# LitLeo/3m-asr-inference

Measured on AMD Instinct MI355X. Metric: encoder frames/sec, 18Lx32e Conformer-MoE, 206-frame utterance, higher is better.
Workload: dtype f32; 1 GPU; 18-layer 32-expert fp32 (v_mfma_f32_16x16x4_f32), batch=1x206 frames per GPU, all experts local (BASELINE.json configs[1]); layers=18, experts=32, frames=206, batch_per_gpu=1, parallelism=replicas x1, streams_per_gpu=4, hip_graph=True, kernels_per_forward=267, fold_pos_proj=True, routing=balanced, route_mode=staged, packed_rows=False, fork_embed=auto

## Files before the change

### 3m-asr-inference_amd/csrc/api.hip

```cpp
#include <string.h>

#include <vector>

#include "../../include/m3asr.h"
#include "common.h"
#include "kernels.h"

namespace m3 {

static thread_local char g_err[512] = "";

void set_error(const char* fmt, ...) {
  va_list ap;
  va_start(ap, fmt);
  vsnprintf(g_err, sizeof(g_err), fmt, ap);
  va_end(ap);
}
const char* last_error() { return g_err; }

struct MoeWorkspace {
  int32_t* mapping;
  int32_t* acc;
  int32_t* pos;
  float* slab;
// ... 152 lines not shown
  M3_REQUIRE(rows && mapping && out, "moe_combine_bf16: null pointer");
  return launch_moe_combine(rows, 1, mapping, nullptr, gate_value, nullptr, resid, alpha, ln_gamma, ln_beta, ln_eps, out,
                            S, idim, (hipStream_t)stream, out_bf16);
}
int m3_ep_send_map(const int32_t* gate_idx, const int32_t* mapping, const int32_t* acc_histogram, int S, int world, int e_loc,
                   int capacity, int32_t* map_send, void* wire, int row_bytes, m3_stream stream) {
  M3_REQUIRE(gate_idx && mapping && acc_histogram && map_send && wire, "ep_send_map: null pointer");
  return launch_ep_send_map(gate_idx, mapping, acc_histogram, S, world, e_loc, capacity, map_send, wire, row_bytes,
                            (hipStream_t)stream);
}
int m3_ep_recv_gate(const void* wire, int world, int e_loc, int capacity, int row_bytes, int32_t* gate_recv, m3_stream stream) {
  M3_REQUIRE(wire && gate_recv, "ep_recv_gate: null pointer");
  return launch_ep_recv_gate(wire, world, e_loc, capacity, row_bytes, gate_recv, (hipStream_t)stream);
}
int m3_moe_router(const float* embed, int ld_embed, int embed_dim, const float* x, int ldx, int idim, const float* w,
                  const float* bias, const float* ln_gamma, const float* ln_beta, float ln_eps, float* xn, int ld_xn,
                  float* logits, int ld_logits, int S, int num_expert, m3_stream stream) {
  M3_REQUIRE(S <= 1 || (ld_embed >= embed_dim && ldx >= idim), "moe_router: ld_embed=%d / ldx=%d shorter than the rows (%d / %d)",
             ld_embed, ldx, embed_dim, idim);
  M3_REQUIRE(S <= 1 || xn == nullptr || ld_xn >= idim, "moe_router: ld_xn=%d is shorter than a row of %d", ld_xn, idim);
  M3_REQUIRE(S <= 1 || ld_logits >= num_expert, "moe_router: ld_logits=%d is shorter than a row of %d", ld_logits, num_expert);
  M3_REQUIRE(aligned16(embed) && aligned16(x) && aligned16(xn), "moe_router: embed / x / xn must be 16-byte aligned");
  return launch_moe_router(embed, ld_embed, embed_dim, x, ldx, idim, w, bias, ln_gamma, ln_beta, ln_eps, xn, ld_xn, logits,
                           ld_logits, S, num_expert, nullptr, (hipStream_t)stream);
}
int m3_softmax_top1(const float* logits, int ld, const int32_t* len, int rows_per_batch, int S, int width,
                    int32_t* idx, float* value, m3_stream stream) {
  M3_REQUIRE(S <= 1 || ld >= width, "softmax_topk: ld=%d is shorter than a row of %d", ld, width);
  return launch_softmax_top1(logits, ld, len, rows_per_batch, S, width, idx, value, (hipStream_t)stream);
}
int m3_moe_gate_index(const float* logits, const int32_t* row_len, int rows_per_batch, int S, int num_expert, int32_t* gate_idx,
                      float* gate_value, int32_t* mapping, int32_t* acc_histogram, int32_t* pos, m3_stream stream) {
  M3_REQUIRE(logits && gate_idx && gate_value && mapping && acc_histogram, "moe_gate_index: null pointer");
  M3_REQUIRE(aligned16(logits), "moe_gate_index: logits must be 16-byte aligned");
  return launch_moe_gate_index(logits, num_expert, row_len, rows_per_batch, S, gate_idx, gate_value, mapping, acc_histogram, pos,
                               (hipStream_t)stream);
}
int m3_moe_route(const float* x, int ldx, int idim, const float* wx, const float* wsum, const float* bias, const float* eall,
                 int ld_e, float ln_eps, const int32_t* row_len, int rows_per_batch, int S, int num_expert, int32_t* gate_idx,
                 float* gate_value, int32_t* mapping, int32_t* acc_histogram, int32_t* pos, m3_stream stream) {
  M3_REQUIRE(x && wx && wsum && gate_idx && gate_value && mapping && acc_histogram, "moe_route: null pointer");
  M3_REQUIRE(idim > 0, "moe_route: idim=%d", idim);
  M3_REQUIRE(S <= 1 || ldx >= idim, "moe_route: ldx=%d is shorter than a row of %d", ldx, idim);
  M3_REQUIRE(eall == nullptr || S <= 1 || ld_e >= num_expert, "moe_route: ld_e=%d is shorter than a row of %d", ld_e, num_expert);
  M3_REQUIRE(aligned16(x) && aligned16(wx), "moe_route: x / wx must be 16-byte aligned");
  return launch_moe_route(x, ldx, idim, wx, wsum, bias, eall, ld_e, ln_eps, row_len, rows_per_batch, S, num_expert, gate_idx,
                          gate_value, mapping, acc_histogram, pos, (hipStream_t)stream);
}
size_t m3_moe_route_expert_workspace_size(int S, int num_expert, int idim, int hidden_units) {
  if (!expert_ffn_f32_self_routing(S, num_expert) || idim <= 0 || hidden_units <= 0 || hidden_units % kExpertSlice) return 0;
  return align_up(expert_ffn_slab_bytes(S, idim, hidden_units), 256);
}
int m3_moe_route_expert_ffn(const float* x, int ldx, const float* logits, const int32_t* row_len, int rows_per_batch,
                            const float* w1, const float* b1, const float* w2, int w2_sliced, const float* b2, int S,
                            int num_expert, int idim, int hidden_units, const float* norm_gamma, const float* norm_beta,
                            float norm_eps, int use_gate_value, const float* resid, float alpha, const float* ln_gamma,
                            const float* ln_beta, float ln_eps, int32_t* gate_idx, float* gate_value, int32_t* mapping,
                            int32_t* acc_histogram, int32_t* pos, float* y, void* workspace, size_t workspace_bytes,
                            m3_stream stream) {
  M3_REQUIRE(x && w1 && b1 && w2 && y, "moe_route_expert_ffn: null pointer");
  M3_REQUIRE((norm_gamma == nullptr) == (norm_beta == nullptr) && (ln_gamma == nullptr) == (ln_beta == nullptr),
             "moe_route_expert_ffn: a LayerNorm needs both gamma and beta");
  M3_REQUIRE(idim > 0 && hidden_units > 0, "moe_route_expert_ffn: bad sizes D=%d F=%d", idim, hidden_units);
  M3_REQUIRE(S <= 1 || ldx >= idim, "moe_route_expert_ffn: ldx=%d is shorter than a row of %d", ldx, idim);
  M3_REQUIRE(aligned16(x) && aligned16(logits), "moe_route_expert_ffn: x / logits must be 16-byte aligned");
  const size_t need = m3_moe_route_expert_workspace_size(S, num_expert, idim, hidden_units);
  M3_REQUIRE(need == 0 || (workspace != nullptr && workspace_bytes >= need), "moe_route_expert_ffn: workspace %zu bytes < required %zu",
             workspace_bytes, need);
  float* slab = (float*)workspace;
  int rc = launch_expert_route_ffn_f32(x, ldx, logits, row_len, rows_per_batch, S, num_expert, idim, hidden_units, w1, b1, w2, w2_sliced,
                                       b2, slab, gate_idx, gate_value, mapping, acc_histogram, pos, (hipStream_t)stream, norm_gamma,
                                       norm_beta, norm_eps);
  if (rc) return rc;
  return launch_moe_combine(slab, hidden_units / kExpertSlice, nullptr, gate_idx, use_gate_value ? gate_value : nullptr, nullptr, resid,
                            alpha, ln_gamma, ln_beta, ln_eps, y, S, idim, (hipStream_t)stream);
}

static int attention_operands(const void* qkv, int ldq, const void* p, int ldp, const void* out, int ldo, int B, int T, int H, int dk) {
  M3_REQUIRE(B * T <= 1 || (ldq >= 3 * H * dk && ldo >= H * dk), "attention: ldq=%d / ldo=%d shorter than the rows (%d / %d)", ldq, ldo, 3 * H * dk, H * dk);
  M3_REQUIRE(T <= 1 || ldp >= H * dk, "attention: ldp=%d is shorter than a row of %d", ldp, H * dk);
  M3_REQUIRE(aligned16(qkv) && aligned16(p) && aligned16(out), "attention: qkv / p / out must be 16-byte aligned");
  return 0;
}

static int linear_params(const m3_linear_desc* d, GemmParams* out) {
  M3_REQUIRE(d != nullptr, "linear: null descriptor");
  GemmParams p;
  p.A = d->a; p.lda = d->lda;
  p.A2 = d->a2; p.lda2 = d->lda2; p.K1 = d->k1;
  p.mode = d->a2 ? GEMM_A_CONCAT2 : GEMM_A_PLAIN;
  p.W = (const float*)d->w; p.bias = d->bias; p.Y = d->y; p.ldy = d->ldy;
  M3_REQUIRE(d->weight_dtype == M3_F32 || d->weight_dtype == M3_BF16, "linear: weight_dtype %d", d->weight_dtype);
  p.w_bf16 = d->weight_dtype == M3_BF16;
  p.M = d->M; p.N = d->N; p.K = d->K;
  p.ln_gamma = d->ln_gamma; p.ln_beta = d->ln_beta; p.ln_eps = d->ln_eps;
  p.ln_wsum = d->ln_wsum; p.ln_wbeta = d->ln_wbeta;
  p.row_len = d->len; p.rows_per_batch = d->rows_per_batch; p.mask_in = d->mask_in; p.mask_out = d->mask_out;
  p.act = d->act; p.alpha = d->alpha; p.resid = d->resid; p.ldr = d->ldr;
  M3_REQUIRE((d->a_dtype == M3_F32 || d->a_dtype == M3_BF16) && (d->y_dtype == M3_F32 || d->y_dtype == M3_BF16),
             "linear: a_dtype / y_dtype must be f32 or bf16");
  if (d->a_dtype == M3_BF16 || d->y_dtype == M3_BF16 || d->y_copy_bf16)
    M3_REQUIRE(p.w_bf16 && p.mode == GEMM_A_PLAIN && !p.ln_gamma, "linear: bf16 activations need bf16 weights, plain A, no affine LayerNorm");
  p.a_bf16 = d->a_dtype == M3_BF16; p.y_bf16 = d->y_dtype == M3_BF16;
  p.Yb = d->y_copy_bf16; p.ldyb = d->ld_copy; p.Yb_stats = d->y_copy_stats;
  p.ln_stats = d->ln_stats; p.ln_stat_parts = d->ln_stat_parts;
  {
    const int n_out = d->act == M3_ACT_GLU ? d->N / 2 : d->N;
    const int k1 = d->a2 ? d->k1 : d->K, a_mult = p.a_bf16 ? 8 : 4;
    const bool rows = d->M > 1;
    M3_REQUIRE(d->lda % a_mult == 0 && (!rows || d->lda >= k1), "linear: lda=%d must be a multiple of %d and >= %d", d->lda, a_mult, k1);
    if (d->a2) M3_REQUIRE(d->lda2 % 4 == 0 && (!rows || d->lda2 >= d->K - k1), "linear: lda2=%d must be a multiple of 4 and >= %d", d->lda2, d->K - k1);
    M3_REQUIRE(!rows || d->ldy >= n_out, "linear: ldy=%d is shorter than an output row of %d", d->ldy, n_out);
    if (p.y_bf16) M3_REQUIRE(d->ldy % 4 == 0, "linear: ldy=%d must be a multiple of 4 for a bf16 y", d->ldy);
    if (d->resid) M3_REQUIRE(!rows || d->ldr >= n_out, "linear: ldr=%d is shorter than an output row of %d", d->ldr, n_out);
    if (d->y_copy_bf16) M3_REQUIRE(d->ld_copy % 4 == 0 && (!rows || d->ld_copy >= n_out), "linear: ld_copy=%d must be a multiple of 4 and >= %d", d->ld_copy, n_out);
  }
  *out = p;
  return 0;
}
static int linear_pointers(const m3_linear_desc* d) {
  M3_REQUIRE(d->a && d->w && d->y, "linear: null a / w / y");
  M3_REQUIRE(aligned16(d->a) && aligned16(d->a2) && aligned16(d->y) && aligned16(d->resid) && aligned16(d->y_copy_bf16),
             "linear: a / a2 / y / resid / y_copy_bf16 must be 16-byte aligned");
  M3_REQUIRE((const void*)d->resid != (const void*)d->y || d->ldr == d->ldy, "linear: y == resid (in-place) needs ldr=%d == ldy=%d", d->ldr, d->ldy);
  return 0;
}
const char* m3_linear_kernel(const m3_linear_desc* d, int with_workspace) {
  GemmParams p;
  if (linear_params(d, &p)) return nullptr;
  return gemm_kernel_label(p, with_workspace && gemm_f32_splitk_plan(p, nullptr) >= 2);
}
int m3_linear(const m3_linear_desc* d, m3_stream stream) {
  GemmParams p;
  if (int rc = linear_params(d, &p)) return rc;
  if (int rc = linear_pointers(d)) return rc;
  return launch_gemm_f32(p, (hipStream_t)stream);
}
size_t m3_linear_workspace_size(const m3_linear_desc* d) {
  GemmParams p;
  size_t need = 0;
  if (linear_params(d, &p) == 0) gemm_f32_splitk_plan(p, &need);
  return need;
}
int m3_linear_ws(const m3_linear_desc* d, void* workspace, size_t workspace_bytes, m3_stream stream) {
  GemmParams p;
  if (int rc = linear_params(d, &p)) return rc;
  if (int rc = linear_pointers(d)) return rc;
  size_t need = 0;
  if (gemm_f32_splitk_plan(p, &need) >= 2 && workspace != nullptr && workspace_bytes >= need)
    return launch_gemm_f32_splitk(p, (float*)workspace, workspace_bytes, (hipStream_t)stream);
  return launch_gemm_f32(p, (hipStream_t)stream);
}

int m3_layer_norm(const float* x, const float* gamma, const float* beta, float eps, float* y, int rows, int dim,
                  m3_stream stream) {
  return launch_layernorm(x, gamma, beta, eps, y, rows, dim, (hipStream_t)stream);
}
int m3_relpos_attention(const float* qkv, int ldq, const float* p, int ldp, const float* pos_u, const float* pos_v,
                        const int32_t* len, int B, int T, int H, int dk, float scale, float* out, int ldo,
                        m3_stream stream) {
  if (int rc = attention_operands(qkv, ldq, p, ldp, out, ldo, B, T, H, dk)) return rc;
  return launch_relpos_attention(qkv, ldq, p, ldp, pos_u, pos_v, len, B, T, H, dk, scale, out, ldo,
                                 (hipStream_t)stream);
}
int m3_relpos_attention_bf16(const void* qkv, int ldq, const float* p, int ldp, const float* pos_u, const float* pos_v,
                             const int32_t* len, int B, int T, int H, int dk, float scale, int chunk, int left_chunks,
                             void* out, int ldo, m3_stream stream) {
  if (int rc = attention_operands(qkv, ldq, p, ldp, out, ldo, B, T, H, dk)) return rc;
  return launch_relpos_attention_bf16(qkv, ldq, p, ldp, pos_u, pos_v, len, B, T, H, dk, scale, out, ldo, (hipStream_t)stream,
                                      nullptr, chunk, left_chunks);
}
int m3_relpos_attention_chunk(const float* qkv, int ldq, const float* p, int ldp, const float* pos_u, const float* pos_v,
                              const int32_t* len, int B, int T, int H, int dk, float scale, int chunk, int left_chunks,
                              float* out, int ldo, m3_stream stream) {
  if (int rc = attention_operands(qkv, ldq, p, ldp, out, ldo, B, T, H, dk)) return rc;
  return launch_relpos_attention(qkv, ldq, p, ldp, pos_u, pos_v, len, B, T, H, dk, scale, out, ldo, (hipStream_t)stream, 0,
                                 nullptr, chunk, left_chunks);
}
int m3_dwconv_ln_silu(const float* z, const float* w_kc, const float* bias, const float* gamma, const float* beta,
                      float eps, int B, int T, int D, int K, float* out, m3_stream stream) {
  return launch_dwconv_ln_silu(z, w_kc, bias, gamma, beta, eps, B, T, D, K, out, (hipStream_t)stream);
}
int m3_subsample_conv1(const float* feat, const float* w9c, const float* bias, int B, int T, int idim, int C,
                       float* out, m3_stream stream) {
  return launch_conv1_relu(feat, w9c, bias, nullptr, nullptr, B, T, idim, C, out, (hipStream_t)stream);
}
int m3_subsample_conv1_cmvn(const float* feat, const float* w9c, const float* bias, const float* cmvn_mean,
                            const float* cmvn_istd, int B, int T, int idim, int C, float* out, m3_stream stream) {
  M3_REQUIRE((cmvn_mean == nullptr) == (cmvn_istd == nullptr), "subsample_conv1: cmvn mean and istd go together");
  return launch_conv1_relu(feat, w9c, bias, cmvn_mean, cmvn_istd, B, T, idim, C, out, (hipStream_t)stream);
}
int m3_conv2d_3x3s2_first(const float* feat, const float* w9c, const float* bias, int B, int T, int idim, int C, int act,
                          float* out, m3_stream stream) {
  M3_REQUIRE(act == M3_ACT_NONE || act == M3_ACT_RELU, "conv2d: act %d (none / relu)", act);
  return launch_conv1_relu(feat, w9c, bias, nullptr, nullptr, B, T, idim, C, out, (hipStream_t)stream, act == M3_ACT_RELU);
}
int m3_cmvn(const float* x, const int32_t* len, const float* mean, const float* istd, int B, int T, int D, float* y,
            m3_stream stream) {
  M3_REQUIRE(x && mean && istd && y, "cmvn: null pointer");
  return launch_cmvn(x, len, mean, istd, B, T, D, y, (hipStream_t)stream);
}
int m3_log_softmax_bias(const float* x, const float* bias, float* y, size_t rows, int n, m3_stream stream) {
  M3_REQUIRE(x && y && n > 0, "log_softmax_bias: bad arguments");
  return launch_log_softmax_bias(x, bias, y, rows, n, (hipStream_t)stream);
}
int m3_conv2d_3x3s2(const float* in, const float* w, const float* bias, int B, int T1, int F1, int C, int act, float* out,
                    m3_stream stream);
int m3_subsample_conv2(const float* in, const float* w, const float* bias, int B, int T1, int F1, int C, float* out,
                       m3_stream stream) {
  return m3_conv2d_3x3s2(in, w, bias, B, T1, F1, C, M3_ACT_RELU, out, stream);
}
int m3_conv2d_3x3s2(const float* in, const float* w, const float* bias, int B, int T1, int F1, int C, int act, float* out,
                    m3_stream stream) {
  M3_REQUIRE(T1 >= 3 && F1 >= 3, "subsample_conv2: input (%d,%d) smaller than the kernel", T1, F1);
  M3_REQUIRE(act == M3_ACT_NONE || act == M3_ACT_RELU || act == M3_ACT_SILU, "conv2d: act %d", act);
  GemmParams p;
  p.mode = GEMM_A_CONV3X3S2;
  p.A = in; p.lda = 4;
  p.conv_T1 = T1; p.conv_F1 = F1; p.conv_T2 = (T1 - 3) / 2 + 1; p.conv_F2 = (F1 - 3) / 2 + 1; p.conv_C = C;
  p.W = w; p.bias = bias; p.Y = out; p.ldy = C;
  p.M = B * p.conv_T2 * p.conv_F2; p.N = C; p.K = 9 * C;
  p.act = act;
  return launch_gemm_f32(p, (hipStream_t)stream);
}

int m3_att_masked_softmax(const float* scores, const int32_t* len, int B, int H, int T1, int T2, float scale,
                          float* out, m3_stream stream) {
  return launch_att_masked_softmax(scores, len, B, H, T1, T2, scale, out, (hipStream_t)stream);
}
int m3_ctc_greedy(const float* logits, const int32_t* len, int B, int T, int V, int blank, int32_t* frame_ids,
                  int32_t* tokens, int32_t* n_tokens, m3_stream stream) {
  return launch_ctc_greedy(logits, len, B, T, V, blank, frame_ids, tokens, n_tokens, (hipStream_t)stream);
}
int m3_ctc_topk(const float* logits, size_t rows, int V, int k, float* top_logp, int32_t* top_idx, m3_stream stream) {
  return launch_ctc_topk(logits, rows, V, k, top_logp, top_idx, (hipStream_t)stream);
}
int m3_ctc_prefix_beam_search(const float* top_logp, const int32_t* top_idx, int T, int k, int beam, int blank,
                              int32_t* hyp_tokens, int32_t* hyp_len, float* hyp_score, int32_t* n_hyps) {
  return ctc_prefix_beam_search_host(top_logp, top_idx, T, k, beam, blank, hyp_tokens, hyp_len, hyp_score, n_hyps);
}
size_t m3_ctc_beam_state_size(const m3_ctc_beam_desc* desc) { return ctc_beam_state_size(desc); }
int m3_ctc_beam_reset(const m3_ctc_beam_desc* desc, void* state, size_t state_bytes, m3_stream stream) {
  return launch_ctc_beam_reset(desc, state, state_bytes, (hipStream_t)stream);
}
int m3_ctc_beam_reset_slots(const m3_ctc_beam_desc* desc, void* state, size_t state_bytes, const int32_t* slots, int n, m3_stream stream) {
  M3_REQUIRE(n == 0 || slots != nullptr, "ctc_beam_reset_slots: null slot list");
  if (n == 0) return 0;
  return launch_ctc_beam_reset(desc, state, state_bytes, (hipStream_t)stream, slots, n);
}
int m3_ctc_beam_advance(const m3_ctc_beam_desc* desc, void* state, size_t state_bytes, const float* top_logp,
                        const int32_t* top_idx, int T_chunk, const int32_t* n_frames, m3_stream stream) {
  return launch_ctc_beam_advance(desc, state, state_bytes, top_logp, top_idx, T_chunk, n_frames, (hipStream_t)stream);
}
int m3_ctc_beam_nbest(const m3_ctc_beam_desc* desc, const void* state, size_t state_bytes, int32_t* hyp_tokens,
                      int32_t* hyp_len, float* hyp_score, int32_t* n_hyps, m3_stream stream) {
  return launch_ctc_beam_nbest(desc, state, state_bytes, hyp_tokens, hyp_len, hyp_score, n_hyps, (hipStream_t)stream);
}
size_t m3_ctc_greedy_stream_state_size(const m3_ctc_greedy_desc* desc) { return ctc_greedy_stream_state_size(desc); }
int m3_ctc_greedy_stream_reset(const m3_ctc_greedy_desc* desc, void* state, size_t state_bytes, m3_stream stream) {
  return launch_ctc_greedy_stream_reset(desc, state, state_bytes, (hipStream_t)stream);
}
int m3_ctc_greedy_stream_reset_slots(const m3_ctc_greedy_desc* desc, void* state, size_t state_bytes, const int32_t* slots, int n,
                                     m3_stream stream) {
  M3_REQUIRE(n == 0 || slots != nullptr, "ctc_greedy_stream_reset_slots: null slot list");
  if (n == 0) return 0;
  return launch_ctc_greedy_stream_reset(desc, state, state_bytes, (hipStream_t)stream, slots, n);
}
int m3_ctc_greedy_stream_advance(const m3_ctc_greedy_desc* desc, void* state, size_t state_bytes, const float* logits,
                                 int T_chunk, int V, const int32_t* n_frames, int32_t* frame_ids, m3_stream stream) {
  return launch_ctc_greedy_stream_advance(desc, state, state_bytes, logits, T_chunk, V, n_frames, frame_ids, (hipStream_t)stream);
}
int m3_ctc_greedy_stream_tokens(const m3_ctc_greedy_desc* desc, const void* state, size_t state_bytes, int32_t* tokens,
                                int32_t* n_tokens, m3_stream stream) {
  return launch_ctc_greedy_stream_tokens(desc, state, state_bytes, tokens, n_tokens, (hipStream_t)stream);
}
int m3_cat_split_cache(const void* in_cache, const void* input, int B, int cache_dim, int input_dim, void* output,
                       void* out_cache, m3_stream stream) {
  return launch_cat_split_cache(in_cache, input, B, cache_dim, input_dim, output, out_cache, (hipStream_t)stream);
}
int m3_att_stream_softmax(const float* scores, const int32_t* decode_frame_num, const int32_t* mask_idx, int B, int N,
                          int ld, int cache_len, float scale, float* out, m3_stream stream) {
  return launch_att_stream_softmax(scores, decode_frame_num, mask_idx, B, N, ld, cache_len, scale, out, (hipStream_t)stream);
}
int m3_rel_positional_encoding(const float* x, const float* pe, int pe_len, const int32_t* frame_num, int max_offset,
                               float scale, int B, int T, int D, float* y, float* pos_emb, int32_t* frame_num_out,
                               m3_stream stream) {
  return launch_rel_positional_encoding(x, pe, pe_len, frame_num, max_offset, scale, B, T, D, y, pos_emb, frame_num_out,
                                        (hipStream_t)stream);
}
int m3_masked_fill(const float* x, const int32_t* len, int B, int C, int T, float fill, float* y, m3_stream stream) {
  return launch_masked_fill(x, len, B, C, T, fill, y, (hipStream_t)stream);
}
int m3_glu(const float* x, int outer, int C, int inner, float* y, m3_stream stream) {
  return launch_glu(x, outer, C, inner, y, (hipStream_t)stream);
}
int m3_mask_conv2d_sample(const int32_t* len_in, int B, int left_padding, int stride, int32_t* len_out,
                          m3_stream stream) {
  return launch_mask_conv2d_sample(len_in, B, left_padding, stride, len_out, (hipStream_t)stream);
}
int m3_scale(const float* x, float scale, float* y, size_t n, m3_stream stream) {
  return launch_scale(x, scale, y, n, (hipStream_t)stream);
}
int m3_unary(const float* x, float* y, size_t n, int act, m3_stream stream) {
  return launch_unary(x, y, n, act, (hipStream_t)stream);
}
int m3_binary(const float* a, const float* b, float* y, const int64_t* shape, const int64_t* strides_a,
// ... 70 lines not shown
```

### 3m-asr-inference_amd/csrc/conv.hip

```cpp
#include "common.h"
#include "kernels.h"

namespace m3 {

struct DwCausal {
  int causal = 0;
  const float* left = nullptr;
  long left_b_stride = 0; int left_t_stride = 0;
  const int32_t* step = nullptr;
  long half = 0;
  const int32_t* chunk_len = nullptr;
  int max_chunks = 0;
};

template <int KT, bool CAUSAL, bool SLOTS = false>
__device__ __forceinline__ void dwconv_ln_silu_body(const float* __restrict__ z, const float* __restrict__ w_kc,
                                                    const float* __restrict__ bias, const float* __restrict__ gamma,
                                                    const float* __restrict__ beta, float eps, int T, int D, int K,
                                                    float* __restrict__ out, int out_bf16, const int32_t* __restrict__ pad_of,
                                                    const int32_t* __restrict__ row0, const int32_t* __restrict__ row_len,
                                                    int n_rows, const DwCausal& cs, const int row) {
  __shared__ float red[2][16];
  asm volatile("" ::"s"(z), "s"(w_kc), "s"(bias), "s"(gamma), "s"(beta), "s"(eps), "s"(T), "s"(D), "s"(K), "s"(out), "s"(out_bf16),
               "s"(pad_of), "s"(row0), "s"(row_len), "s"(n_rows));
// ... 53 lines not shown
        } else {
          on[kk] = (k0 + kk < K && tt >= 0 && tt < T) ? 1.f : 0.f;
        }
        zz[kk] = ldg4(src + c);
        ww[kk] = ldg4(w_kc + (size_t)k * D + c);
      }
#pragma unroll
      for (int kk = 0; kk < KT; ++kk)
#pragma unroll
        for (int j = 0; j < 4; ++j) v[j] = fmaf(zz[kk][j] * on[kk], ww[kk][j], v[j]);
    }
  }
  if (gamma != nullptr) {
    float s = live ? (v[0] + v[1]) + (v[2] + v[3]) : 0.f;
    s = wave_sum(s);
    if (lane == 0) red[0][wave] = s;
    __syncthreads();
    float tot = 0.f;
    for (int w = 0; w < nwaves; ++w) tot += red[0][w];
    const float mean = tot / (float)D;
    float q = 0.f;
    if (live) {
#pragma unroll
      for (int j = 0; j < 4; ++j) {
        const float d = v[j] - mean;
        q += d * d;
      }
    }
    q = wave_sum(q);
    if (lane == 0) red[1][wave] = q;
    __syncthreads();
    float qt = 0.f;
    for (int w = 0; w < nwaves; ++w) qt += red[1][w];
    const float rstd = rsqrtf(qt / (float)D + eps);
    if (live) {
      const f32x4 g = ldg4(gamma + c), be = ldg4(beta + c);
#pragma unroll
      for (int j = 0; j < 4; ++j) v[j] = (v[j] - mean) * rstd * g[j] + be[j];
    }
  }
  if (live) {
#pragma unroll
    for (int j = 0; j < 4; ++j) v[j] = silu(v[j]);
    if (out_bf16) {
      bf16x4 h;
#pragma unroll
      for (int j = 0; j < 4; ++j) h[j] = (bf16_t)v[j];
      *reinterpret_cast<bf16x4*>(reinterpret_cast<bf16_t*>(out) + (size_t)row * D + c) = h;
    } else {
      stg4(out + (size_t)row * D + c, v);
    }
  }
}

template <int KT, bool CAUSAL, bool SLOTS = false>
__global__ __launch_bounds__(1024) void dwconv_ln_silu_kernel(const float* __restrict__ z, const float* __restrict__ w_kc,
                                                              const float* __restrict__ bias,
                                                              const float* __restrict__ gamma,
                                                              const float* __restrict__ beta, float eps, int T,
                                                              int D, int K, float* __restrict__ out, int out_bf16,
                                                              const int32_t* __restrict__ pad_of,
                                                              const int32_t* __restrict__ row0,
                                                              const int32_t* __restrict__ row_len, int n_rows, DwCausal cs) {
  dwconv_ln_silu_body<KT, CAUSAL, SLOTS>(z, w_kc, bias, gamma, beta, eps, T, D, K, out, out_bf16, pad_of, row0, row_len, n_rows, cs, (int)blockIdx.x);
}
struct DwKernArgs {
  const float *z, *w_kc, *bias, *gamma, *beta; float eps; int T, D, K; float* out; int out_bf16;
  const int32_t *pad_of, *row0, *row_len; int n_rows; DwCausal cs;
};
template <int KT, bool CAUSAL>
__global__ __launch_bounds__(1024) void dwconv_ln_silu_dual_kernel(const DwKernArgs a, const DwKernArgs b) {
  if ((int)blockIdx.x < a.n_rows)
    dwconv_ln_silu_body<KT, CAUSAL>(a.z, a.w_kc, a.bias, a.gamma, a.beta, a.eps, a.T, a.D, a.K, a.out, a.out_bf16, a.pad_of, a.row0, a.row_len,
                                    a.n_rows, a.cs, (int)blockIdx.x);
  else
    dwconv_ln_silu_body<KT, CAUSAL>(b.z, b.w_kc, b.bias, b.gamma, b.beta, b.eps, b.T, b.D, b.K, b.out, b.out_bf16, b.pad_of, b.row0, b.row_len,
                                    b.n_rows, b.cs, (int)blockIdx.x - a.n_rows);
}

static int launch_dwconv_impl(const float* z, const float* w_kc, const float* bias, const float* gamma, const float* beta, float eps,
                              int B, int T, int D, int K, float* out, hipStream_t stream, int out_bf16, const int32_t* pad_of,
                              const int32_t* row0, const int32_t* row_len, const DwCausal& cs, bool slots = false) {
  M3_REQUIRE(!slots || (cs.causal && cs.step != nullptr && cs.max_chunks > 0), "dwconv (slot mode): needs the streaming causal form");
  M3_REQUIRE((D & 3) == 0 && D <= 4096, "dwconv: channels=%d must be a multiple of 4 (<=4096)", D);
  M3_REQUIRE(cs.causal || (K & 1) == 1, "dwconv: kernel size %d must be odd (non-causal)", K);
  M3_REQUIRE(!cs.causal || (cs.left != nullptr && K >= 2), "dwconv (causal): the frames left of frame 0 must be supplied (left_fill / cache)");
  const int rows = B * T;
  if (rows == 0) return 0;
  const int threads = (int)align_up(D / 4, 64);
  const int grid = rows + (cs.step != nullptr ? B * (K - 1) : 0);
#define M3_DW_CASE(KT_, C_)                                                                                                  \
  hipLaunchKernelGGL((dwconv_ln_silu_kernel<KT_, C_>), dim3(grid), dim3(threads), 0, stream, z, w_kc, bias, gamma, beta, eps, T, \
                     D, K, out, out_bf16, pad_of, row0, row_len, rows, cs)
#define M3_DW_SLOTS(KT_)                                                                                                        \
  hipLaunchKernelGGL((dwconv_ln_silu_kernel<KT_, true, true>), dim3(grid), dim3(threads), 0, stream, z, w_kc, bias, gamma, beta, eps, \
                     T, D, K, out, out_bf16, pad_of, row0, row_len, rows, cs)
  if (slots) { if (K <= 15) M3_DW_SLOTS(15); else M3_DW_SLOTS(8); }
  else if (K <= 15) { if (cs.causal) M3_DW_CASE(15, true); else M3_DW_CASE(15, false); }
  else { if (cs.causal) M3_DW_CASE(8, true); else M3_DW_CASE(8, false); }
#undef M3_DW_SLOTS
#undef M3_DW_CASE
  M3_LAUNCH_CHECK();
  return 0;
}

int launch_dwconv_ln_silu(const float* z, const float* w_kc, const float* bias, const float* gamma,
                          const float* beta, float eps, int B, int T, int D, int K, float* out, hipStream_t stream, int out_bf16,
                          const int32_t* pad_of, const int32_t* row0, const int32_t* row_len, const float* causal_left_fill) {
  DwCausal cs;
  if (causal_left_fill != nullptr) { cs.causal = 1; cs.left = causal_left_fill; }
  return launch_dwconv_impl(z, w_kc, bias, gamma, beta, eps, B, T, D, K, out, stream, out_bf16, pad_of, row0, row_len, cs);
}

int launch_dwconv_ln_silu_args(const DwArgs& a, hipStream_t stream) {
  return launch_dwconv_ln_silu(a.z, a.w_kc, a.bias, a.gamma, a.beta, a.eps, a.B, a.T, a.D, a.K, a.out, stream, a.out_bf16, a.pad_of, a.row0,
                               a.row_len, a.causal_left_fill);
}
bool dwconv_dual_fusable(const DwArgs& a, const DwArgs& b) {
  return a.D == b.D && a.K == b.K && (a.causal_left_fill != nullptr) == (b.causal_left_fill != nullptr) && a.B * a.T > 0 && b.B * b.T > 0 &&
         (a.D & 3) == 0 && a.D <= 4096 && (a.causal_left_fill != nullptr || (a.K & 1) == 1);
}
int launch_dwconv_ln_silu_dual(const DwArgs& a, const DwArgs& b, hipStream_t stream) {
  M3_REQUIRE(dwconv_dual_fusable(a, b), "dwconv dual: the two problems do not share an instantiation");
  auto pack = [](const DwArgs& q) {
    DwKernArgs k;
    k.z = q.z; k.w_kc = q.w_kc; k.bias = q.bias; k.gamma = q.gamma; k.beta = q.beta; k.eps = q.eps; k.T = q.T; k.D = q.D; k.K = q.K;
    k.out = q.out; k.out_bf16 = q.out_bf16; k.pad_of = q.pad_of; k.row0 = q.row0; k.row_len = q.row_len; k.n_rows = q.B * q.T;
    if (q.causal_left_fill != nullptr) { k.cs.causal = 1; k.cs.left = q.causal_left_fill; }
    return k;
  };
  const DwKernArgs ka = pack(a), kb = pack(b);
  const int threads = (int)align_up(a.D / 4, 64), grid = ka.n_rows + kb.n_rows;
  const bool causal = a.causal_left_fill != nullptr;
#define M3_DWD_CASE(KT_, C_) hipLaunchKernelGGL((dwconv_ln_silu_dual_kernel<KT_, C_>), dim3(grid), dim3(threads), 0, stream, ka, kb)
  if (a.K <= 15) { if (causal) M3_DWD_CASE(15, true); else M3_DWD_CASE(15, false); }
  else { if (causal) M3_DWD_CASE(8, true); else M3_DWD_CASE(8, false); }
#undef M3_DWD_CASE
  M3_LAUNCH_CHECK();
  return 0;
}

int launch_dwconv_ln_silu_stream(const float* z, const float* w_kc, const float* bias, const float* gamma, const float* beta,
                                 float eps, int B, int T, int D, int K, float* out, float* cache_pair, const int32_t* step,
                                 const int32_t* chunk_len, hipStream_t stream, int out_bf16, int slot_max_chunks) {
  M3_REQUIRE(cache_pair && step && chunk_len, "dwconv (stream): null state");
  DwCausal cs;
  cs.causal = 1; cs.left = cache_pair; cs.left_b_stride = (long)(K - 1) * D; cs.left_t_stride = D;
  cs.step = step; cs.half = (long)B * (K - 1) * D; cs.chunk_len = chunk_len;
  cs.max_chunks = slot_max_chunks > 0 ? slot_max_chunks : 0;
  return launch_dwconv_impl(z, w_kc, bias, gamma, beta, eps, B, T, D, K, out, stream, out_bf16, nullptr, nullptr, nullptr, cs,
                            slot_max_chunks >= 0);
}

__global__ __launch_bounds__(256) void conv1_relu_kernel(const float* __restrict__ feat, const float* __restrict__ w9c,
                                                         const float* __restrict__ bias,
                                                         const float* __restrict__ cmvn_mean,
                                                         const float* __restrict__ cmvn_istd, int T, int idim, int T1,
                                                         int F1, int C, float* __restrict__ out, int relu, int out_bf16,
                                                         const int32_t* __restrict__ feat_len, int32_t* __restrict__ lens_out, int B) {
  extern __shared__ float xs[];
  const int row = blockIdx.x;
  if (feat_len != nullptr && blockIdx.x == 0 && blockIdx.y == 0)
    for (int i = threadIdx.x; i < B; i += blockDim.x) lens_out[i] = ((feat_len[i] - 3) / 2 + 1 - 3) / 2 + 1;
  const int b = row / T1, t1 = row - b * T1;
  const float* src = feat + ((size_t)b * T + 2 * t1) * idim;
  for (int i = threadIdx.x; i < 3 * idim; i += blockDim.x) {
    float xv = src[i];
    if (cmvn_mean != nullptr) {
      const int f = i % idim;
      xv = (xv - cmvn_mean[f]) * cmvn_istd[f];
    }
    xs[i] = xv;
  }
  const int c = threadIdx.x * 4;
  const bool live = c < C;
  f32x4 w[9], bv = f32x4{0.f, 0.f, 0.f, 0.f};
  if (live) {
    bv = ldg4(bias + c);
#pragma unroll
    for (int k = 0; k < 9; ++k) w[k] = ldg4(w9c + (size_t)k * C + c);
  }
  __syncthreads();
  if (!live) return;
  const size_t obase = (size_t)row * F1 * C + c;
  const int fchunk = (F1 + gridDim.y - 1) / gridDim.y;
  const int f_lo = blockIdx.y * fchunk, f_hi = min(F1, f_lo + fchunk);
  for (int f1 = f_lo; f1 < f_hi; ++f1) {
    f32x4 acc = bv;
#pragma unroll
    for (int kh = 0; kh < 3; ++kh)
#pragma unroll
      for (int kw = 0; kw < 3; ++kw) {
        const float xv = xs[kh * idim + 2 * f1 + kw];
#pragma unroll
        for (int j = 0; j < 4; ++j) acc[j] = fmaf(xv, w[kh * 3 + kw][j], acc[j]);
      }
#pragma unroll
    for (int j = 0; j < 4; ++j) acc[j] = relu ? fmaxf(acc[j], 0.f) : acc[j];
    if (out_bf16) {
      bf16x4 h;
#pragma unroll
      for (int j = 0; j < 4; ++j) h[j] = (bf16_t)acc[j];
      *reinterpret_cast<bf16x4*>(reinterpret_cast<bf16_t*>(out) + obase + (size_t)f1 * C) = h;
    } else {
      stg4(out + obase + (size_t)f1 * C, acc);
    }
  }
}

int launch_conv1_relu(const float* feat, const float* w9c, const float* bias, const float* cmvn_mean,
                      const float* cmvn_istd, int B, int T, int idim, int C, float* out, hipStream_t stream, int relu, int out_bf16,
                      const int32_t* feat_len, int32_t* lens_out) {
  M3_REQUIRE(T >= 3 && idim >= 3, "subsampling: input (T=%d, idim=%d) shorter than the 3x3 kernel", T, idim);
  M3_REQUIRE((C & 3) == 0 && C <= 1024, "subsampling: channels=%d must be a multiple of 4 (<= 1024)", C);
  const int T1 = (T - 3) / 2 + 1, F1 = (idim - 3) / 2 + 1;
  if (B * T1 == 0) return 0;
  const int threads = (int)align_up(C / 4, 64);
  const int fsplit = B * T1 >= 2048 ? 1 : (B * T1 >= 512 ? 2 : 5);
  hipLaunchKernelGGL(conv1_relu_kernel, dim3(B * T1, fsplit), dim3(threads), 3 * idim * sizeof(float), stream,
                     feat, w9c, bias, cmvn_mean, cmvn_istd, T, idim, T1, F1, C, out, relu, out_bf16, feat_len, lens_out, B);
  M3_LAUNCH_CHECK();
  return 0;
}

__global__ void depthwise_conv1d_nct_kernel(const float* __restrict__ x, const float* __restrict__ w,
                                            const float* __restrict__ bias, int C, int T, int To, int K, int pad,
                                            float* __restrict__ y, size_t n) {
  for (size_t i = (size_t)blockIdx.x * blockDim.x + threadIdx.x; i < n; i += (size_t)gridDim.x * blockDim.x) {
    const int t = (int)(i % To);
    const size_t bc = i / To;
    const int c = (int)(bc % C);
    const float* xr = x + bc * T;
    float acc = bias ? bias[c] : 0.f;
    for (int k = 0; k < K; ++k) {
      const int tt = t + k - pad;
      if (tt >= 0 && tt < T) acc = fmaf(xr[tt], w[(size_t)c * K + k], acc);
    }
    y[i] = acc;
  }
}

int launch_depthwise_conv1d_nct(const float* x, const float* w, const float* bias, int B, int C, int T, int K,
                                int pad, float* y, hipStream_t stream) {
  const int To = T + 2 * pad - K + 1;
  M3_REQUIRE(pad >= 0 && To > 0, "depthwise_conv1d: T=%d K=%d pad=%d leaves no output", T, K, pad);
  const size_t n = (size_t)B * C * To;
  if (n == 0) return 0;
  hipLaunchKernelGGL(depthwise_conv1d_nct_kernel, dim3(grid1d(n, 4096)), dim3(256), 0,
                     stream, x, w, bias, C, T, To, K, pad, y, n);
  M3_LAUNCH_CHECK();
  return 0;
}

__global__ void pad2d_kernel(const float* __restrict__ x, int H, int W, int pre_h, int pre_w, int Ho, int Wo,
                             float* __restrict__ y, size_t n) {
  for (size_t i = (size_t)blockIdx.x * blockDim.x + threadIdx.x; i < n; i += (size_t)gridDim.x * blockDim.x) {
    const int wo = (int)(i % Wo), ho = (int)((i / Wo) % Ho);
    const size_t o = i / ((size_t)Wo * Ho);
    const int h = ho - pre_h, w_ = wo - pre_w;
    y[i] = (h >= 0 && h < H && w_ >= 0 && w_ < W) ? x[(o * H + h) * W + w_] : 0.f;
  }
}
int launch_pad2d(const float* x, size_t outer, int H, int W, int pre_h, int post_h, int pre_w, int post_w, float* y, hipStream_t stream) {
  M3_REQUIRE(pre_h >= 0 && post_h >= 0 && pre_w >= 0 && post_w >= 0, "pad2d: negative padding (cropping) is not implemented");
  const int Ho = H + pre_h + post_h, Wo = W + pre_w + post_w;
  const size_t n = outer * Ho * Wo;
  if (n == 0) return 0;
  hipLaunchKernelGGL(pad2d_kernel, dim3(grid1d(n, 4096)), dim3(256), 0, stream, x, H, W, pre_h, pre_w, Ho, Wo, y, n);
  M3_LAUNCH_CHECK();
  return 0;
}

}
```

### 3m-asr-inference_amd/csrc/engine.hip

```cpp
#include <assert.h>
#include <math.h>
#include <stdlib.h>
#include <string.h>

#include <functional>
#include <memory>
#include <string>
#include <unordered_map>
#include <vector>

#include "../../include/m3asr.h"
#include "common.h"
#include "kernels.h"

namespace m3 {
struct MoeWorkspace {
  int32_t* mapping; int32_t* acc; int32_t* pos; float* slab; size_t bytes;
};
MoeWorkspace carve_moe_workspace(void* base, int S, int E, int D, int F);
}

using namespace m3;

namespace {

struct Norm { const float* g = nullptr; const float* b = nullptr; };
struct Lin { const float* w = nullptr; const float* b = nullptr; const float* wsum = nullptr; const float* wbeta = nullptr; };

struct BlockW {
  Norm n_ffm, n_mha, n_conv, n_ff, n_final, n_cnn;
  Lin mac1, mac2, qkv, pos, out, pw1, pw2, ff1, ff2;
  const float* pos_u = nullptr; const float* pos_v = nullptr;
  const float* dw_w = nullptr; const float* dw_b = nullptr;
  const float* left_fill = nullptr;
  Lin router;
  Lin router_x;
  const float *ew1 = nullptr, *eb1 = nullptr, *ew2 = nullptr, *eb2 = nullptr;
  const float *es1 = nullptr, *es2 = nullptr;
  float h_scale = 0.f;
};

struct SubW { const float* c1w; const float* c1b; const float* c2w; const float* c2b; Lin out; };

enum class FuseKind { None, Gemm, Dwconv, Attention };

struct Stage {
  std::string name;
  std::function<int(hipStream_t)> run;
  m3_stage_info info;
  bool reads_embed = false;
  FuseKind fuse_kind = FuseKind::None;
  GemmParams gemm;
  DwArgs dw;
  AttArgs att;
};

m3_stage_info stage_info(const char* kernel, int launches, double bytes, double flops, bool per_row = true) {
  m3_stage_info i;
  i.kernel = kernel; i.launches = launches; i.per_row = per_row ? 1 : 0; i.alg_bytes = bytes; i.flops = flops;
  return i;
}

struct Buf { void* ptr; size_t bytes; };

struct BindKey {
  int B = 0, T = 0;
  const float* feat = nullptr; const int32_t* feat_len = nullptr; float* logits = nullptr;
  void* ws = nullptr; size_t ws_bytes = 0;
  int ep_cap = 0;
  void* sstate = nullptr; int s_hist = 0, s_maxf = 0;
  bool s_slots = false;
  bool operator==(const BindKey& o) const {
    return B == o.B && T == o.T && feat == o.feat && feat_len == o.feat_len && logits == o.logits && ws == o.ws &&
           ws_bytes == o.ws_bytes && ep_cap == o.ep_cap && sstate == o.sstate && s_hist == o.s_hist && s_maxf == o.s_maxf &&
           s_slots == o.s_slots;
  }
};

}

struct m3_engine {
  m3_engine_config cfg;
  std::unordered_map<std::string, m3_weight_entry> table;
  std::vector<std::string> names;
  SubW sub_e, sub_m;
  std::vector<BlockW> eblocks, mblocks;
  Norm e_after, m_after;
  Lin out_linear;
  const float* pe = nullptr;
  int64_t pe_rows = 0;
  const float* pos_all = nullptr;
  const float* cmvn_mean = nullptr; const float* cmvn_istd = nullptr;
  const float* output_bias = nullptr;
  const float* router_e_all = nullptr;

  struct Bound {
    BindKey key;
    int Tp = 0, S = 0;
    bool a16 = false;
    bool dma = false;
    bool packed = false;
    bool xn_skipped = false;
    int fork_first = -1, fork_mid = -1, join_at = -1;
    std::shared_ptr<float> pfold;
    std::vector<Stage> stages;
    std::unordered_map<std::string, Buf> buffers;
    int n_kernels = 0;
    hipGraphExec_t graph_exec = nullptr;
    bool graph_valid = false;
    uint64_t last_use = 0;
    bool matches(const BindKey& k) const { return !stages.empty() && key == k; }
  };
  Bound cur;
  std::vector<Bound> parked;
  uint64_t use_clock = 0;
  int n_captures = 0;
  int ep_capacity = 0;
  hipStream_t side = nullptr;
  hipEvent_t ev_fork = nullptr, ev_join = nullptr;
  std::unordered_map<int, std::weak_ptr<float>> pfold_by_tp;
};

namespace {

struct Switches {
  int gate_index_max_rows;
  bool self_route;
  bool hfuse;
  int router_min_rows;
  bool router_xq;
  bool router_skip_xn;
  bool fused8_adapt;
};
const Switches& switches() {
  static const Switches sw = [] {
    auto num = [](const char* name, int dflt) { const char* v = getenv(name); return v ? atoi(v) : dflt; };
    Switches w;
    w.gate_index_max_rows = num("M3_GATE_INDEX_MAX_ROWS", 512);
    w.self_route = num("M3_SELF_ROUTE", 1) != 0;
    w.hfuse = num("M3_HFUSE", 1) != 0;
    w.router_min_rows = num("M3_ROUTER_MIN_ROWS", 2048);
    w.router_xq = num("M3_ROUTER_XQ", 1) != 0;
    w.router_skip_xn = num("M3_ROUTER_SKIP_XN", 0) != 0;
    w.fused8_adapt = num("M3_FUSED8_ADAPT", 0) != 0;
    return w;
  }();
  return sw;
}

bool lookup(const m3_engine* e, const std::string& name, int64_t numel, const float** out, int dtype = M3_F32) {
  auto it = e->table.find(name);
  if (it == e->table.end()) {
    set_error("engine: weight '%s' missing from the plan", name.c_str());
    return false;
  }
  if (numel >= 0 && it->second.numel != numel) {
    set_error("engine: weight '%s' has %lld elements, expected %lld", name.c_str(), (long long)it->second.numel,
              (long long)numel);
    return false;
  }
  if (it->second.dtype != dtype) {
    set_error("engine: weight '%s' has dtype %d, the engine (weight_dtype=%d) expects %d", name.c_str(),
              (int)it->second.dtype, (int)e->cfg.weight_dtype, dtype);
    return false;
  }
  *out = (const float*)it->second.data;
  return true;
}

#define GET(dst, name, numel) \
  do { if (!lookup(e, (name), (numel), &(dst))) return false; } while (0)
#define GETW(dst, name, numel) \
  do { if (!lookup(e, (name), (numel), &(dst), e->cfg.weight_dtype == M3_F32 ? M3_F32 : M3_BF16)) return false; } while (0)
#define GETE(dst, name, numel) \
  do { if (!lookup(e, (name), (numel), &(dst), e->cfg.weight_dtype)) return false; } while (0)

bool load_norm(const m3_engine* e, const std::string& p, int d, Norm* n) {
  GET(n->g, p + "weight", d);
  GET(n->b, p + "bias", d);
  return true;
}
bool load_lin(const m3_engine* e, const std::string& p, int64_t n_out, int64_t n_in, bool bias, Lin* l) {
  GETW(l->w, p + "weight", n_out * n_in);
  if (bias) GET(l->b, p + "bias", n_out);
  return true;
}
bool load_lin_ln(const m3_engine* e, const std::string& p, int64_t n_out, int64_t n_in, bool wbeta, Lin* l,
                 bool fp32_only = false) {
  if (fp32_only) {
    GET(l->w, p + "ln.weight", n_out * n_in);
  } else {
    GETW(l->w, p + "ln.weight", n_out * n_in);
  }
  GET(l->b, p + "ln.bias", n_out);
  GET(l->wsum, p + "ln.wsum", n_out);
  if (wbeta) GET(l->wbeta, p + "ln.wbeta", n_out);
  return true;
}

bool load_block(const m3_engine* e, const std::string& p, int D, int F, int K, bool cnn_ln, bool moe, int De, BlockW* b, bool causal) {
  const m3_engine_config& c = e->cfg;
  if (!load_norm(e, p + "norm_final.", D, &b->n_final)) return false;
  if (moe && !load_norm(e, p + "norm_ff.", D, &b->n_ff)) return false;
  if (!load_lin_ln(e, p + "feed_forward_macaron.w_1.", F, D, false, &b->mac1) ||
      !load_lin(e, p + "feed_forward_macaron.w_2.", D, F, true, &b->mac2) ||
      !load_lin_ln(e, p + "self_attn.qkv.", 3 * D, D, false, &b->qkv) ||
      !load_lin(e, p + "self_attn.linear_out.", D, D, true, &b->out) ||
      !load_lin_ln(e, p + "conv_module.pointwise_conv1.", 2 * D, D, true, &b->pw1) ||
      !load_lin(e, p + "conv_module.pointwise_conv2.", D, D, true, &b->pw2))
    return false;
  GET(b->pos_u, p + "self_attn.pos_bias_u", D);
  GET(b->pos_v, p + "self_attn.pos_bias_v", D);
  GET(b->dw_w, p + "conv_module.depthwise_conv.weight_kc", (int64_t)K * D);
  GET(b->dw_b, p + "conv_module.depthwise_conv.bias", D);
  if (cnn_ln && !load_norm(e, p + "conv_module.norm.", D, &b->n_cnn)) return false;
  if (causal) GET(b->left_fill, p + "conv_module.left_fill", D);
  if (!moe) {
    if (!load_lin_ln(e, p + "feed_forward.w_1.", F, D, false, &b->ff1) ||
        !load_lin(e, p + "feed_forward.w_2.", D, F, true, &b->ff2))
      return false;
  } else {
    const int world = c.ep_world_size > 0 ? c.ep_world_size : 1;
    const int64_t Etot = (int64_t)c.num_experts * world;
    GET(b->router.w, p + "feed_forward.router_weights_t", Etot * (D + De));
    if (c.router_with_bias) GET(b->router.b, p + "feed_forward.router_bias", Etot);
    if (c.fuse_route && !load_lin_ln(e, p + "feed_forward.router_x.", Etot, D, false, &b->router_x, true)) return false;
    const int64_t E = c.num_experts;
    GETE(b->ew1, p + "feed_forward.experts.w_1.weight", E * F * D);
    if (c.weight_dtype == M3_FP8) {
      GET(b->es1, p + "feed_forward.experts.w_1.scale", E * F);
      GET(b->es2, p + "feed_forward.experts.w_2.scale", E * D);
      if (c.fp8_activations) {
        const float* hs = nullptr;
        GET(hs, p + "feed_forward.experts.h_scale", 1);
        if (hipMemcpy(&b->h_scale, hs, sizeof(float), hipMemcpyDeviceToHost) != hipSuccess || !(b->h_scale > 0.f)) {
          set_error("engine: '%sfeed_forward.experts.h_scale' must hold one positive number", p.c_str());
          return false;
        }
      }
    }
    GET(b->eb1, p + "feed_forward.experts.w_1.bias", E * F);
    GETE(b->ew2, p + "feed_forward.experts.w_2.weight_sliced", E * D * F);
    GET(b->eb2, p + "feed_forward.experts.w_2.bias", E * D);
  }
  return true;
}

bool load_sub(const m3_engine* e, const std::string& p, int D, int idim, SubW* s) {
  const int F2 = ((idim - 1) / 2 - 1) / 2;
  GET(s->c1w, p + "conv.0.weight_9c", 9 * (int64_t)D);
  GET(s->c1b, p + "conv.0.bias", D);
  GETW(s->c2w, p + "conv.2.weight_ohwi", 9 * (int64_t)D * D);
  GET(s->c2b, p + "conv.2.bias", D);
  return load_lin(e, p + "out.0.", D, (int64_t)D * F2, true, &s->out);
}
#undef GET
#undef GETW
#undef GETE

inline int sub_len(int t) { return ((t - 3) / 2 + 1 - 3) / 2 + 1; }

struct Carver {
  char* base; size_t off = 0;
  explicit Carver(void* b) : base((char*)b) {}
  template <typename T> T* take(size_t n) {
    T* p = (T*)(base ? base + off : nullptr);
    off += align_up(n * sizeof(T), 256);
    return p;
  }
};

struct Plan {
  int32_t* lens;
  float *c1, *c2, *x, *emb, *h1, *qkv, *pbuf, *ctx, *glu, *dw, *xn, *rl, *eall;
  void* xb;
  int32_t* moe_fs;
  unsigned char* xq; float* xq_scale;
  float* xstats;
  int32_t* gate_idx; float* gate_val;
  void* moe_ws; size_t moe_ws_bytes;
  float* splitk; size_t splitk_bytes;
  float* taps;
  float* pfold;
  int32_t *row0, *pad_of; float* xpad; void* xbpad; float* lpk;
  int32_t *ep_acc, *ep_mapping, *ep_pos, *ep_map_send, *ep_gate_recv, *ep_overflow; float *wire_a, *wire_b; int ep_cap, ep_rows;
  bool fork;
  bool hfuse;
  float *e_c1, *e_c2, *e_x, *e_h1, *e_qkv, *e_ctx, *e_glu, *e_dw, *e_xpad, *e_splitk, *e_xstats; void *e_xb, *e_xbpad;
  size_t bytes;
};

bool use_fork_embed(const m3_engine_config& c, int B, int S) { return c.fork_embed > 0 && !c.debug_taps; }
bool use_packed_rows(const m3_engine_config& c, int B) {
  if (c.packed_rows < 0 || (c.packed_rows == 0 && B <= 1)) return false;
  return !c.debug_taps && c.fuse_route == 0 && B <= 1024;
}

bool use_hfuse(const m3_engine_config& c, int B, int S) {
  return switches().hfuse && !c.debug_taps && c.weight_dtype == M3_F32 && c.embed_blocks > 0 && c.num_blocks > 0 && S <= 128 && c.fork_embed <= 0 &&
         !use_packed_rows(c, B);
}

Plan make_plan(const m3_engine_config& c, void* base, int B, int T, int ep_capacity = 0) {
  Plan p;
  Carver cv(base);
  const int Tp = sub_len(T), S = B * Tp;
  const int T1 = (T - 3) / 2 + 1, F1 = (c.input_dim - 3) / 2 + 1, F2 = (F1 - 3) / 2 + 1;
  const int D = c.attention_dim > c.embed_dim ? c.attention_dim : c.embed_dim;
  const int F = c.hidden_units > c.embed_linear_units ? c.hidden_units : c.embed_linear_units;
  const int world = c.ep_world_size > 0 ? c.ep_world_size : 1;
  const int Etot = c.num_experts * world;
  p.lens = cv.take<int32_t>(B);
  p.c1 = cv.take<float>((size_t)B * T1 * F1 * D);
  p.c2 = cv.take<float>((size_t)S * F2 * D);
  p.x = cv.take<float>((size_t)S * D);
  p.emb = cv.take<float>((size_t)S * D);
  p.xb = cv.take<uint16_t>((size_t)S * D);
  p.xstats = cv.take<float>((size_t)S * 2 * kXbStatParts);
  p.h1 = cv.take<float>((size_t)S * F);
  p.qkv = cv.take<float>((size_t)S * 3 * D);
  p.pbuf = cv.take<float>((size_t)Tp * D * (c.num_blocks + c.embed_blocks));
  p.ctx = cv.take<float>((size_t)S * D);
  p.glu = cv.take<float>((size_t)S * D);
  p.dw = cv.take<float>((size_t)S * D);
  p.xn = cv.take<float>((size_t)S * D);
  p.xq = nullptr; p.xq_scale = nullptr; p.moe_fs = nullptr;
  if (c.weight_dtype == M3_FP8) p.moe_fs = cv.take<int32_t>(64);
  if (c.weight_dtype == M3_FP8 && D == 512) {
    p.xq = cv.take<unsigned char>((size_t)S * D);
    p.xq_scale = cv.take<float>((size_t)S);
  }
  p.rl = cv.take<float>((size_t)S * Etot);
  p.eall = cv.take<float>((size_t)S * Etot * c.num_blocks);
  p.gate_idx = cv.take<int32_t>((size_t)c.num_blocks * S);
  p.gate_val = cv.take<float>((size_t)c.num_blocks * S);
  const bool ep = world > 1 || c.ep_stages > 0;
  p.ep_cap = ep ? (ep_capacity > 0 ? ep_capacity : S) : 0;
  p.ep_rows = ep ? world * (p.ep_cap + 1) : 0;
  p.moe_ws_bytes = carve_moe_workspace(nullptr, ep ? p.ep_rows : S, c.num_experts, c.attention_dim, c.hidden_units).bytes;
  p.moe_ws = cv.take<char>(p.moe_ws_bytes * (size_t)(c.debug_taps ? c.num_blocks : 1));
  p.ep_acc = p.ep_mapping = p.ep_pos = p.ep_map_send = p.ep_gate_recv = p.ep_overflow = nullptr; p.wire_a = p.wire_b = nullptr;
  if (ep) {
    p.ep_overflow = cv.take<int32_t>(64);
    p.ep_acc = cv.take<int32_t>((size_t)Etot + 1);
    p.ep_mapping = cv.take<int32_t>(S);
    p.ep_pos = cv.take<int32_t>(S);
    p.ep_map_send = cv.take<int32_t>(S);
    p.ep_gate_recv = cv.take<int32_t>(p.ep_rows);
    p.wire_a = cv.take<float>((size_t)p.ep_rows * c.attention_dim);
    p.wire_b = cv.take<float>((size_t)p.ep_rows * c.attention_dim);
  }
  {
    size_t n1 = 0, n2 = 0;
    if (c.weight_dtype == M3_F32) {
      GemmParams g;
      g.mode = GEMM_A_CONV3X3S2; g.lda = 4; g.conv_C = D; g.M = S * F2; g.N = D; g.K = 9 * D; g.ldy = D;
      gemm_f32_splitk_plan(g, &n1);
      GemmParams l;
      l.lda = F2 * D; l.M = S; l.N = D; l.K = F2 * D; l.ldy = D;
      gemm_f32_splitk_plan(l, &n2);
    }
    p.splitk_bytes = n1 > n2 ? n1 : n2;
    p.splitk = p.splitk_bytes ? cv.take<float>(p.splitk_bytes / sizeof(float)) : nullptr;
  }
  p.taps = c.debug_taps ? cv.take<float>((size_t)(c.num_blocks + c.embed_blocks) * S * D) : nullptr;
  p.pfold = nullptr;
  p.row0 = p.pad_of = nullptr; p.xpad = p.lpk = nullptr; p.xbpad = nullptr;
  if (use_packed_rows(c, B)) {
    p.row0 = cv.take<int32_t>(B + 1);
    p.pad_of = cv.take<int32_t>(S);
    p.xpad = cv.take<float>((size_t)S * D);
    p.xbpad = cv.take<uint16_t>((size_t)S * D);
    p.lpk = cv.take<float>((size_t)S * c.output_dim);
  }
  p.fork = use_fork_embed(c, B, S);
  p.hfuse = !p.fork && use_hfuse(c, B, S);
  p.e_c1 = p.c1; p.e_c2 = p.c2; p.e_x = p.x; p.e_h1 = p.h1; p.e_qkv = p.qkv; p.e_ctx = p.ctx; p.e_glu = p.glu; p.e_dw = p.dw;
  p.e_xb = p.xb; p.e_xpad = p.xpad; p.e_xbpad = p.xbpad; p.e_splitk = p.splitk; p.e_xstats = p.xstats;
  if (p.fork || p.hfuse) {
    p.e_c1 = cv.take<float>((size_t)B * T1 * F1 * D);
    p.e_c2 = cv.take<float>((size_t)S * F2 * D);
    p.e_x = cv.take<float>((size_t)S * D);
    p.e_xb = cv.take<uint16_t>((size_t)S * D);
    p.e_xstats = cv.take<float>((size_t)S * 2 * kXbStatParts);
    p.e_h1 = cv.take<float>((size_t)S * F);
    p.e_qkv = cv.take<float>((size_t)S * 3 * D);
    p.e_ctx = cv.take<float>((size_t)S * D);
    p.e_glu = cv.take<float>((size_t)S * D);
    p.e_dw = cv.take<float>((size_t)S * D);
    if (p.splitk_bytes) p.e_splitk = cv.take<float>(p.splitk_bytes / sizeof(float));
    if (use_packed_rows(c, B)) {
      p.e_xpad = cv.take<float>((size_t)S * D);
      p.e_xbpad = cv.take<uint16_t>((size_t)S * D);
    }
  }
  p.bytes = cv.off;
  return p;
}

struct StreamState {
  int32_t* step = nullptr;
  std::vector<float*> kv, conv;
  int32_t *slot_pos = nullptr, *slot_status = nullptr, *slot_frames = nullptr;
  size_t bytes = 0;
};
StreamState carve_stream_state(const m3_engine_config& c, void* base, int B, int hist) {
  Carver cv(base);
  StreamState st;
  st.step = cv.take<int32_t>(64);
  const int nb = c.embed_blocks + c.num_blocks, D = c.attention_dim, K = c.cnn_module_kernel;
  for (int i = 0; i < nb; ++i) st.kv.push_back(cv.take<float>((size_t)B * hist * 2 * D));
  for (int i = 0; i < nb; ++i) st.conv.push_back(cv.take<float>((size_t)2 * B * (K - 1) * D));
  st.slot_pos = cv.take<int32_t>((size_t)3 * B);
  st.slot_status = st.slot_pos ? st.slot_pos + B : nullptr;
  st.slot_frames = st.slot_pos ? st.slot_pos + 2 * B : nullptr;
  st.bytes = cv.off;
  return st;
}

Plan embed_view(const Plan& pl) {
  Plan q = pl;
  q.c1 = pl.e_c1; q.c2 = pl.e_c2; q.x = pl.e_x; q.h1 = pl.e_h1; q.qkv = pl.e_qkv; q.ctx = pl.e_ctx; q.glu = pl.e_glu; q.dw = pl.e_dw;
  q.xb = pl.e_xb; q.xpad = pl.e_xpad; q.xbpad = pl.e_xbpad; q.splitk = pl.e_splitk; q.xstats = pl.e_xstats;
  return q;
}

enum class RouterForm {
  Gemm,
  Kernel,
  Fused,
  Split,
};
enum class GateForm {
  RouterTail,
  GateIndex,
  Top1Index,
  InExpert,
  InRoute,
};
struct MoeRoute {
  RouterForm router = RouterForm::Gemm;
  GateForm gate = GateForm::Top1Index;
  bool ep = false;
  bool router_top1 = false;
  bool use_xq = false;
  bool skip_xn = false;
  bool fs_dev = false;
  bool needs_e_all = false;
  bool norm_in_expert() const { return router == RouterForm::Fused || router == RouterForm::Split; }
};

static ExpertWeights expert_weights(const m3_engine_config& c, const BlockW& w) {
  if (c.weight_dtype == M3_F32) return ExpertWeights::F32;
  if (c.weight_dtype == M3_BF16) return ExpertWeights::BF16;
  return w.h_scale > 0.f ? ExpertWeights::FP8A8 : ExpertWeights::FP8;
}

MoeRoute choose_moe_route(const m3_engine_config& c, int S, const BlockW& w, const Plan& pl) {
  const Switches& sw = switches();
  const int world = c.ep_world_size > 0 ? c.ep_world_size : 1;
  const int E = c.num_experts, Etot = E * world, D = c.attention_dim, De = c.embed_dim, F = c.hidden_units;
  const bool one_wg_experts = Etot == 8 || Etot == 16 || Etot == 32 || Etot == 64;
  const bool self_routing = sw.self_route && c.weight_dtype == M3_F32 && expert_ffn_f32_self_routing(S, Etot) &&
                            plan_expert_ffn(ExpertWeights::F32, S, E, D, F).kernel == ExpertKernel::SlabF32;
  MoeRoute r;
  r.ep = world > 1 || c.ep_stages > 0;
  if (c.fuse_route == 2 && world == 1 && S < 1024 && one_wg_experts) {
    r.router = RouterForm::Split;
    r.gate = self_routing ? GateForm::InExpert : GateForm::GateIndex;
  } else if (c.fuse_route == 1 && world == 1 && S <= 256 && (E == 16 || E == 32 || E == 64)) {
    r.router = RouterForm::Fused;
    r.gate = GateForm::InRoute;
  } else {
    r.router = moe_router_supports(De, D, Etot) && S >= sw.router_min_rows ? RouterForm::Kernel : RouterForm::Gemm;
    r.router_top1 = r.router == RouterForm::Kernel && moe_router_fuses_top1(Etot) && S > sw.gate_index_max_rows;
    if (self_routing && c.fuse_route == 0 && !r.ep) r.gate = GateForm::InExpert;
    else if (S <= sw.gate_index_max_rows && one_wg_experts) r.gate = GateForm::GateIndex;
    else r.gate = r.router_top1 ? GateForm::RouterTail : GateForm::Top1Index;
  }
  const bool fused8 = !r.ep && plan_expert_ffn(expert_weights(c, w), S, E, D, F).kernel == ExpertKernel::FusedFp8;
  r.use_xq = r.router == RouterForm::Kernel && sw.router_xq && fused8 && pl.xq != nullptr;
  r.skip_xn = r.use_xq && sw.router_skip_xn && !c.debug_taps;
  r.fs_dev = sw.fused8_adapt && fused8 && pl.moe_fs != nullptr && !c.debug_taps;
  r.needs_e_all = r.norm_in_expert();
  return r;
}

struct StageBuilder {
  const m3_engine& eng;
  Plan pl;
  m3_engine::Bound& bd;
  StreamState st;
  bool lens_in_conv1 = false;
  const float *tail_ln_g = nullptr, *tail_ln_b = nullptr; float tail_ln_eps = 0.f; float* tail_ln_out = nullptr;
  float* splitk_ws = nullptr; size_t splitk_bytes = 0;
};

}

static void add_stage(StageBuilder& sb, const std::string& name, int kernels, std::function<int(hipStream_t)> fn,
                      m3_stage_info info = stage_info("", 0, 0.0, 0.0)) {
  info.launches = kernels;
  sb.bd.stages.push_back(Stage{name, std::move(fn), info});
  sb.bd.n_kernels += kernels;
}

static m3_stage_info gemm_info(const GemmParams& p, bool splitk) {
  const bool glu = p.act == ACT_GLU;
  const double M = p.M, N = p.N, K = p.K, Nout = glu ? N / 2 : N;
  const double wsz = p.w_bf16 ? 2 : 4, asz = p.a_bf16 ? 2 : 4, ysz = p.y_bf16 ? 2 : 4;
  double a_bytes = M * K * asz;
  if (p.mode == GEMM_A_CONV3X3S2)
    a_bytes = (double)(p.M / (p.conv_T2 * p.conv_F2)) * p.conv_T1 * p.conv_F1 * p.conv_C * asz;
  double bytes = N * K * wsz + a_bytes + M * Nout * ysz;
  if (p.resid) bytes += M * Nout * 4;
  if (p.Yb) bytes += M * Nout * 2;
  if (p.ln_out) bytes += M * (K - p.K1) * 4;
  return stage_info(gemm_kernel_label(p, splitk), 1, bytes, 2.0 * M * N * K, p.mode != GEMM_A_CONV3X3S2);
}

static void add_gemm(StageBuilder& sb, const std::string& name, GemmParams p, bool fp32_weights = false) {
  p.w_bf16 = (!fp32_weights && sb.eng.cfg.weight_dtype != M3_F32) ? 1 : 0;
  size_t need = 0;
  if (gemm_f32_splitk_plan(p, &need) >= 2 && sb.splitk_ws != nullptr && need <= sb.splitk_bytes) {
    float* ws = sb.splitk_ws; const size_t wsb = sb.splitk_bytes;
    add_stage(sb, name, 2, [p, ws, wsb](hipStream_t s) { return launch_gemm_f32_splitk(p, ws, wsb, s); }, gemm_info(p, true));
    return;
  }
  add_stage(sb, name, 1, [p](hipStream_t s) { return launch_gemm_f32(p, s); }, gemm_info(p, false));
  sb.bd.stages.back().fuse_kind = FuseKind::Gemm;
  sb.bd.stages.back().gemm = p;
}

static bool stages_fusable(const Stage& a, const Stage& b) {
  if (a.fuse_kind == FuseKind::None || a.fuse_kind != b.fuse_kind) return false;
  if (a.fuse_kind == FuseKind::Gemm) return gemm_f32_dual_fusable(a.gemm, b.gemm);
  if (a.fuse_kind == FuseKind::Dwconv) return dwconv_dual_fusable(a.dw, b.dw);
  if (a.fuse_kind == FuseKind::Attention) return relpos_attention_dual_fusable(a.att, b.att);
  return false;
}
static Stage fused_stage(const Stage& a, const Stage& b) {
  Stage d;
  d.name = a.name + "+" + b.name;
  const char* label = "";
  if (a.fuse_kind == FuseKind::Gemm) {
    const GemmParams pa = a.gemm, pb = b.gemm;
    d.run = [pa, pb](hipStream_t s) { return launch_gemm_f32_dual(pa, pb, s); };
    label = "gemm_f32_dual_kernel";
  } else if (a.fuse_kind == FuseKind::Dwconv) {
    const DwArgs pa = a.dw, pb = b.dw;
    d.run = [pa, pb](hipStream_t s) { return launch_dwconv_ln_silu_dual(pa, pb, s); };
    label = "dwconv_ln_silu_dual_kernel";
  } else {
    const AttArgs pa = a.att, pb = b.att;
    d.run = [pa, pb](hipStream_t s) { return launch_relpos_attention_dual(pa, pb, s); };
    label = "relpos_attention_dual_kernel";
  }
  d.info = stage_info(label, 1, a.info.alg_bytes + b.info.alg_bytes, a.info.flops + b.info.flops);
  return d;
}
static void fuse_independent_pairs(StageBuilder& sb, int first, int mid, int join) {
  if (first < 0 || mid <= first + 1 || join <= mid) return;
  std::vector<Stage>& st = sb.bd.stages;
  std::vector<Stage> out(st.begin(), st.begin() + first);
  std::vector<Stage> pending;
  int i = first, saved = 0;
  for (int m = mid; m < join; ++m) {
    assert(!st[m].reads_embed);
    int partner = -1;
    if (st[m].fuse_kind != FuseKind::None)
      for (int k = std::max(i, first + 1); k < mid; ++k)
        if (stages_fusable(st[k], st[m])) { partner = k; break; }
    if (partner < 0) { pending.push_back(st[m]); continue; }
    for (; i < partner; ++i) out.push_back(st[i]);
    for (Stage& q : pending) out.push_back(q);
    pending.clear();
    out.push_back(fused_stage(st[partner], st[m]));
    i = partner + 1;
    ++saved;
  }
  for (; i < mid; ++i) out.push_back(st[i]);
  for (Stage& q : pending) out.push_back(q);
  for (int k = join; k < (int)st.size(); ++k) out.push_back(st[k]);
  st.swap(out);
  sb.bd.n_kernels -= saved;
}

static int embed_join(const std::vector<Stage>& st, int from) {
  for (int i = from; i < (int)st.size(); ++i)
    if (st[i].reads_embed) return i;
  return -1;
}

static void build_subsample(StageBuilder& sb, const std::string& pfx, const SubW& w, int D, const Plan& pl, float* xout) {
  const m3_engine_config& c = sb.eng.cfg;
  const int B = sb.bd.key.B, T = sb.bd.key.T;
  const int T1 = (T - 3) / 2 + 1, F1 = (c.input_dim - 3) / 2 + 1, F2 = (F1 - 3) / 2 + 1, T2 = (T1 - 3) / 2 + 1;
  const float* feat = sb.bd.key.feat;
  float* c1 = pl.c1; float* c2 = pl.c2;
  const int idim = c.input_dim;
  const float* cm = sb.eng.cmvn_mean; const float* ci = sb.eng.cmvn_istd;
  const bool a16 = sb.bd.a16;
  const int32_t* flen = sb.lens_in_conv1 ? sb.bd.key.feat_len : nullptr;
  int32_t* lens_out = pl.lens;
  sb.lens_in_conv1 = false;
  add_stage(sb, pfx + "conv1", 1, [=](hipStream_t s) { return launch_conv1_relu(feat, w.c1w, w.c1b, cm, ci, B, T, idim, D, c1, s, 1, a16, flen, lens_out); },
            stage_info("conv1_relu_kernel", 1, (double)B * T * idim * 4 + (double)B * T1 * F1 * D * (a16 ? 2 : 4), 18.0 * B * T1 * F1 * D, false));
  GemmParams g;
  g.a_bf16 = a16; g.y_bf16 = a16;
  g.mode = GEMM_A_CONV3X3S2; g.A = c1; g.lda = 4;
  g.conv_T1 = T1; g.conv_F1 = F1; g.conv_T2 = T2; g.conv_F2 = F2; g.conv_C = D;
  g.W = w.c2w; g.bias = w.c2b; g.Y = c2; g.ldy = D; g.M = B * T2 * F2; g.N = D; g.K = 9 * D; g.act = ACT_RELU;
  if (sb.bd.packed) g.conv_len = pl.lens;
  add_gemm(sb, pfx + "conv2", g);
  const bool packed = sb.bd.packed;
  GemmParams l;
  l.A = c2; l.lda = F2 * D; l.W = w.out.w; l.bias = w.out.b; l.Y = packed ? pl.xpad : xout; l.ldy = D;
  l.M = B * T2; l.N = D; l.K = F2 * D; l.alpha = sqrtf((float)D);
  l.a_bf16 = a16;
  if (a16) { l.Yb = packed ? pl.xbpad : pl.xb; l.ldyb = D; }
  add_gemm(sb, pfx + "linear", l);
  if (packed) {
    const float* xpad = pl.xpad; const void* xbpad = pl.xbpad; void* xb = pl.xb; const int32_t* pad_of = pl.pad_of;
    const int S = B * T2;
    add_stage(sb, pfx + "pack", a16 ? 2 : 1, [=](hipStream_t s) {
      if (int rc = launch_local_gather(xpad, pad_of, S, D * 4, xout, s)) return rc;
      return a16 ? launch_local_gather(xbpad, pad_of, S, D * 2, xb, s) : 0;
    }, stage_info("row_permute_kernel", 1, (double)S * D * (a16 ? 12 : 8) + 4.0 * S, 0.0));
  }
  if (sb.bd.dma) {
    const void* xbv = pl.xb; float* xs = pl.xstats;
    const int S = B * T2;
    add_stage(sb, pfx + "row_stats", 1, [=](hipStream_t s) { return launch_row_stats_bf16(xbv, S, D, xs, s); },
              stage_info("row_stats_bf16_kernel", 1, (double)S * D * 2 + 32.0 * S, 3.0 * S * D));
  }
}

struct MoeLayer {
  std::string pfx;
  const BlockW* w;
  int S, Tp, D, F, De, E, Etot, world;
  float eps;
  float *x, *xn, *rl;
  int32_t* gidx; float* gval;
  const float* gv;
  const int32_t *lens, *live_len; int live_rpb;
  const int32_t* pdev;
  const float* eall; int ld_eall;
  void* xb_out; float* xstats_out;
  void* ws; MoeWorkspace mw;
};

static void add_moe_router(StageBuilder& sb, const MoeLayer& m, const MoeRoute& r, const Plan& pl) {
  const BlockW& w = *m.w;
  const int S = m.S, D = m.D, De = m.De, E = m.E, Etot = m.Etot;
  if (r.router == RouterForm::Fused) {
    add_stage(sb, m.pfx + "moe_route", 1, [m](hipStream_t s) {
      const BlockW& w = *m.w;
      return launch_moe_route(m.x, m.D, m.D, w.router_x.w, w.router_x.wsum, w.router_x.b, m.eall, m.ld_eall, m.eps, m.lens, m.Tp,
                              m.S, m.E, m.gidx, m.gval, m.mw.mapping, m.mw.acc, m.mw.pos, s);
    }, stage_info("moe_route_kernel", 1, (double)E * D * 4 + (double)S * (D + E) * 4 + 16.0 * S, 2.0 * S * E * D));
  } else if (r.router == RouterForm::Kernel) {
    void* xq = r.use_xq ? pl.xq : nullptr; float* xqs = r.use_xq ? pl.xq_scale : nullptr;
    float* xn_out = r.skip_xn ? nullptr : m.xn;
    if (r.skip_xn) sb.bd.xn_skipped = true;
    int32_t* gidx = r.router_top1 ? m.gidx : nullptr; float* gval = r.router_top1 ? m.gval : nullptr;
    const float* emb = pl.emb;
    add_stage(sb, m.pfx + "moe_router", 1, [=](hipStream_t s) {
      const BlockW& w = *m.w;
      return launch_moe_router(emb, m.De, m.De, m.x, m.D, m.D, w.router.w, w.router.b, w.n_ff.g, w.n_ff.b, m.eps, xn_out, m.D, m.rl,
                               m.Etot, m.S, m.Etot, m.pdev, s, gidx, gval, m.live_len, m.live_rpb, xq, xqs);
    }, stage_info("moe_router_kernel", 1, (double)Etot * (De + D) * 4 + (double)S * (De + 2 * D + Etot) * 4, 2.0 * S * Etot * (De + D)));
  } else {
    GemmParams g;
    g.Y = m.rl; g.ldy = Etot; g.M = S; g.N = Etot; g.m_dev = m.pdev;
    if (r.router == RouterForm::Split) {
      g.A = m.x; g.lda = D; g.W = w.router_x.w; g.bias = w.router_x.b; g.ln_wsum = w.router_x.wsum; g.ln_eps = m.eps; g.K = D;
      g.resid = m.eall; g.ldr = m.ld_eall;
    } else {
      g.mode = GEMM_A_CONCAT2; g.A = pl.emb; g.lda = De; g.K1 = De; g.A2 = m.x; g.lda2 = D; g.K = De + D;
      g.W = w.router.w; g.bias = w.router.b;
      g.ln_gamma = w.n_ff.g; g.ln_beta = w.n_ff.b; g.ln_eps = m.eps; g.ln_on_a2 = 1; g.ln_out = m.xn; g.ld_ln_out = D;
    }
    add_gemm(sb, m.pfx + "moe_router", g, true);
  }
  sb.bd.stages.back().reads_embed = true;
}

static void add_moe_gate_index(StageBuilder& sb, const MoeLayer& m, int32_t* map, int32_t* acc, int32_t* pos) {
  add_stage(sb, m.pfx + "moe_gate_index", 1, [=](hipStream_t s) {
    return launch_moe_gate_index(m.rl, m.Etot, m.live_len, m.live_rpb, m.S, m.gidx, m.gval, map, acc, pos, s);
  }, stage_info("moe_index_kernel", 1, (double)m.S * (m.Etot * 4 + 16) + 4.0 * (m.Etot + 1), 0.0));
}

static void add_moe_top1(StageBuilder& sb, const MoeLayer& m) {
  add_stage(sb, m.pfx + "moe_top1", 1, [m](hipStream_t s) {
    return launch_softmax_top1(m.rl, m.Etot, m.live_len, m.live_rpb, m.S, m.Etot, m.gidx, m.gval, s);
  }, stage_info("softmax_top1_kernel", 1, (double)m.S * (m.Etot * 4 + 8), 0.0));
}

static void add_moe_local_index(StageBuilder& sb, const MoeLayer& m) {
  add_stage(sb, m.pfx + "moe_local.index", 1, [m](hipStream_t s) {
    return launch_moe_index(m.gidx, m.S, m.E, m.mw.mapping, m.mw.acc, m.mw.pos, s);
  }, stage_info("moe_index_kernel", 1, 12.0 * m.S + 4.0 * (m.E + 1), 0.0));
}

static ExpertFfnArgs expert_args(const BlockW& w, const float* x, const MoeWorkspace& mw, int D) {
  ExpertFfnArgs a{};
  a.x = x; a.ldx = D; a.pos = mw.pos; a.acc_hist = mw.acc; a.w1 = w.ew1; a.w2 = w.ew2; a.s1 = w.es1; a.s2 = w.es2; a.b1 = w.eb1;
  a.w2_sliced = 1; a.h_scale = w.h_scale; a.slab = mw.slab;
  return a;
}

static void add_moe_local_expert(StageBuilder& sb, const MoeLayer& m, const MoeRoute& r, const ExpertFfnPlan& f, const Plan& pl) {
  const bool norm = r.norm_in_expert();
  const float* xin = norm ? m.x : m.xn;
  const bool self_route = r.gate == GateForm::InExpert;
  const void* xq = r.use_xq ? pl.xq : nullptr; const float* xqs = r.use_xq ? pl.xq_scale : nullptr;
  int32_t* fs = r.fs_dev ? pl.moe_fs : nullptr;
  add_stage(sb, m.pfx + "moe_local.expert", f.launches, [=](hipStream_t s) {
    const BlockW& w = *m.w;
    const float* ln_g = norm ? w.n_ff.g : nullptr; const float* ln_b = norm ? w.n_ff.b : nullptr; const float ln_eps = norm ? m.eps : 0.f;
    if (self_route)
      return launch_expert_route_ffn_f32(xin, m.D, m.rl, m.live_len, m.live_rpb, m.S, m.E, m.D, m.F, w.ew1, w.eb1, w.ew2, 1, w.eb2,
                                         m.mw.slab, m.gidx, m.gval, m.mw.mapping, m.mw.acc, m.mw.pos, s, ln_g, ln_b, ln_eps);
    ExpertFfnArgs a = expert_args(w, xin, m.mw, m.D);
    a.ln_gamma = ln_g; a.ln_beta = ln_b; a.ln_eps = ln_eps; a.xq = xq; a.xq_scale = xqs; a.fs_dev = fs;
    return launch_expert_ffn(f, m.S, m.E, m.D, m.F, a, s);
  }, stage_info(f.label, 1, -1.0, 4.0 * m.D * m.F * m.S));
}

static void add_moe_local_combine(StageBuilder& sb, const MoeLayer& m, const MoeRoute& r, const ExpertFfnPlan& f, const Plan& pl) {
  const bool self_route = r.gate == GateForm::InExpert;
  const int32_t* cmap = self_route ? nullptr : m.mw.mapping;
  const float* cb2 = self_route ? nullptr : m.w->eb2;
  const int32_t* fs = r.fs_dev ? pl.moe_fs : nullptr;
  const double S = m.S, D = m.D;
  add_stage(sb, m.pfx + "moe_local.combine", 1, [=](hipStream_t s) {
    const BlockW& w = *m.w;
    return launch_moe_combine(f.rows(m.mw.slab), fs ? kExpertFusedFp8MaxSplit : f.slices, cmap, m.gidx, m.gv, cb2, m.x, 0.5f, w.n_final.g, w.n_final.b, m.eps, m.x,
                              m.S, m.D, s, m.xb_out, m.xstats_out, fs);
  }, stage_info("moe_combine_kernel", 1, S * D * 4 * (f.slices + 2) + (m.xb_out ? 2.0 * S * D : 0.0), S * D * (f.slices + 10)));
}

static void add_moe_ep(StageBuilder& sb, const MoeLayer& m, const MoeRoute& r, const Plan& pl) {
  const int S = m.S, E = m.E, Etot = m.Etot, D = m.D, F = m.F, world = m.world;
  const int cap = pl.ep_cap, R = pl.ep_rows;
  int32_t *g_acc = pl.ep_acc, *g_map = pl.ep_mapping, *g_pos = pl.ep_pos, *map_send = pl.ep_map_send, *gate_recv = pl.ep_gate_recv;
  int32_t* ep_overflow = pl.ep_overflow;
  float *wire_a = pl.wire_a, *wire_b = pl.wire_b;
  const MoeWorkspace rw = carve_moe_workspace(m.ws, R, E, D, F);
  if (r.gate == GateForm::GateIndex) add_moe_gate_index(sb, m, g_map, g_acc, g_pos);
  if (r.gate == GateForm::Top1Index) add_moe_top1(sb, m);
  const bool one_launch = r.gate == GateForm::GateIndex;
  const int32_t* gidx = m.gidx; const float* xn = m.xn;
  add_stage(sb, m.pfx + "moe_ep.send", one_launch ? 1 : 2, [=](hipStream_t s) {
    if (!one_launch)
      if (int rc = launch_moe_index(gidx, S, Etot, g_map, g_acc, g_pos, s)) return rc;
    return launch_ep_send_rows(gidx, g_map, g_acc, S, world, E, cap, map_send, xn, wire_a, D * 4, s, ep_overflow);
  }, stage_info("ep_send_rows_kernel", 1, (double)S * D * 8 + 24.0 * S, 0.0));
  auto exchange = [=, &sb](const char* name) {
    if (world == 1) add_stage(sb, m.pfx + name, 0, [=](hipStream_t s) {
      M3_CHECK_HIP(hipMemcpyAsync(wire_b, wire_a, (size_t)R * D * 4, hipMemcpyDeviceToDevice, s));
      return 0;
    });
  };
  exchange("moe_ep.exchange1");
// ... 176 lines not shown
    if (r.ep) {
      add_moe_ep(sb, m, r, pl);
    } else {
      if (r.gate == GateForm::GateIndex) add_moe_gate_index(sb, m, m.mw.mapping, m.mw.acc, m.mw.pos);
      if (r.gate == GateForm::Top1Index) add_moe_top1(sb, m);
      if (r.gate == GateForm::Top1Index || r.gate == GateForm::RouterTail) add_moe_local_index(sb, m);
      const ExpertFfnPlan f = plan_expert_ffn(expert_weights(c, w), S, m.E, D, F, r.norm_in_expert() ? EXPERT_NORM_IN_KERNEL : 0);
      add_moe_local_expert(sb, m, r, f, pl);
      add_moe_local_combine(sb, m, r, f, pl);
    }
    const std::string b = pfx.substr(0, pfx.size() - 1);
    sb.bd.buffers[b + ".gate_idx"] = Buf{m.gidx, (size_t)S * 4};
    sb.bd.buffers[b + ".gate_value"] = Buf{m.gval, (size_t)S * 4};
    sb.bd.buffers[b + ".mapping"] = Buf{m.mw.mapping, (size_t)S * 4};
    sb.bd.buffers[b + ".acc_histogram"] = Buf{m.mw.acc, (size_t)(m.E + 1) * 4};
  }
  if (c.debug_taps) {
    float* tap = pl.taps + (size_t)tap_index * S * D;
    add_stage(sb, pfx + "tap", 0, [=](hipStream_t s) {
      M3_CHECK_HIP(hipMemcpyAsync(tap, x, (size_t)S * D * sizeof(float), hipMemcpyDeviceToDevice, s));
      return 0;
    });
    sb.bd.buffers[pfx.substr(0, pfx.size() - 1) + ".out"] = Buf{tap, (size_t)S * D * 4};
  }
}

extern "C" {

int m3_engine_output_frames(int T) { return T >= 7 ? sub_len(T) : 0; }

m3_engine* m3_engine_create(const m3_engine_config* config, const m3_weight_entry* table, int n_entries) {
  if (!config || !table || n_entries <= 0) {
    set_error("engine_create: null config / weight table");
    return nullptr;
  }
  m3_engine* e = new m3_engine;
  e->cfg = *config;
  const m3_engine_config& c = e->cfg;
  auto fail = [&](const char* msg) -> m3_engine* {
    if (msg) set_error("%s", msg);
    delete e;
    return nullptr;
  };
  if (c.attention_dim % c.attention_heads || c.embed_dim % c.embed_heads) return fail("engine_create: dim % heads != 0");
  if (c.attention_dim % 16 || c.embed_dim % 16 || c.hidden_units % 64 || c.embed_linear_units % 16)
    return fail("engine_create: dims must be multiples of 16 (hidden_units of 64)");
  if (c.embed_dim != c.attention_dim) return fail("engine_create: embed_dim != attention_dim is not supported");
  if (c.weight_dtype != M3_F32 && c.weight_dtype != M3_BF16 && c.weight_dtype != M3_FP8)
    return fail("engine_create: weight_dtype must be f32, bf16 or fp8");
  if (c.weight_dtype == M3_FP8 && (c.attention_dim % 64 || c.hidden_units % 64))
    return fail("engine_create: fp8 experts need attention_dim and hidden_units that are multiples of 64");
  if (c.fp8_activations && c.weight_dtype != M3_FP8) return fail("engine_create: fp8_activations needs weight_dtype fp8");
  if (c.ep_stages > 0 && c.fuse_route) return fail("engine_create: ep_stages needs the staged route (fuse_route = 0)");
  if (c.ep_world_size > 1 && (c.ep_rank < 0 || c.ep_rank >= c.ep_world_size)) return fail("engine_create: ep_rank outside [0, ep_world_size)");
  if (c.weight_dtype != M3_F32) {
    if (c.fuse_route) return fail("engine_create: fuse_route is fp32-only");
    if (c.attention_dim % 32 || c.hidden_units % 64 || c.embed_linear_units % 32)
      return fail("engine_create: bf16 weights need dims that are multiples of 32");
  }
  e->names.reserve(n_entries);
  for (int i = 0; i < n_entries; ++i) {
    if (!table[i].name || !table[i].data) return fail("engine_create: null weight entry");
    e->names.emplace_back(table[i].name);
    m3_weight_entry w = table[i];
    w.name = nullptr;
    e->table[e->names.back()] = w;
  }
  const int D = c.attention_dim, De = c.embed_dim, K = c.cnn_module_kernel;
  if (!load_sub(e, "embed.subsampling.", De, c.input_dim, &e->sub_e) || !load_sub(e, "subsampling.", D, c.input_dim, &e->sub_m))
    return fail(nullptr);
  if (!load_norm(e, "embed.after_norm.", De, &e->e_after) ||
      !load_lin_ln(e, "out_linear.", c.output_dim, D, false, &e->out_linear))
    return fail(nullptr);
  {
    auto m = e->table.find("cmvn.mean"), v = e->table.find("cmvn.istd"), ob = e->table.find("output_bias");
    if ((m == e->table.end()) != (v == e->table.end())) return fail("engine_create: cmvn.mean and cmvn.istd go together");
    if (m != e->table.end()) {
      if (m->second.numel != c.input_dim || v->second.numel != c.input_dim) return fail("engine_create: cmvn vectors must have input_dim entries");
      e->cmvn_mean = (const float*)m->second.data;
      e->cmvn_istd = (const float*)v->second.data;
    }
    if (ob != e->table.end()) {
      if (ob->second.numel != c.output_dim) return fail("engine_create: output_bias must have output_dim entries");
      e->output_bias = (const float*)ob->second.data;
    }
  }
  {
    auto it = e->table.find("pe");
    if (it == e->table.end() || it->second.numel % D) return fail("engine_create: positional table 'pe' missing");
    e->pe = (const float*)it->second.data;
    e->pe_rows = it->second.numel / D;
  }
  if (!lookup(e, "pos_all.weight", (int64_t)(c.embed_blocks + c.num_blocks) * D * D, &e->pos_all,
              c.weight_dtype == M3_F32 ? M3_F32 : M3_BF16))
    return fail(nullptr);
  if (c.fuse_route && !lookup(e, "router_e_all.weight", (int64_t)c.num_blocks * c.num_experts * De, &e->router_e_all))
    return fail(nullptr);
  e->eblocks.resize(c.embed_blocks);
  for (int i = 0; i < c.embed_blocks; ++i)
    if (!load_block(e, "embed.blocks." + std::to_string(i) + ".", De, c.embed_linear_units, K, c.embed_cnn_layer_norm,
                    false, De, &e->eblocks[i], c.embed_causal > 0))
      return fail(nullptr);
  e->mblocks.resize(c.num_blocks);
  for (int i = 0; i < c.num_blocks; ++i)
    if (!load_block(e, "blocks." + std::to_string(i) + ".", D, c.hidden_units, K, c.cnn_layer_norm, true, De,
                    &e->mblocks[i], c.causal > 0))
      return fail(nullptr);
  return e;
}

void m3_engine_destroy(m3_engine* engine) {
  if (!engine) return;
  if (engine->ev_fork) (void)hipEventDestroy(engine->ev_fork);
  if (engine->ev_join) (void)hipEventDestroy(engine->ev_join);
  if (engine->side) (void)hipStreamDestroy(engine->side);
  if (engine->cur.graph_exec) (void)hipGraphExecDestroy(engine->cur.graph_exec);
  for (auto& b : engine->parked)
    if (b.graph_exec) (void)hipGraphExecDestroy(b.graph_exec);
  delete engine;
}

size_t m3_engine_workspace_size(const m3_engine* engine, int B, int T) {
  if (!engine || B <= 0 || T < 7) return 0;
  return make_plan(engine->cfg, nullptr, B, T, engine->ep_capacity).bytes;
}

static int init_engine_kernels() {
  int (*const inits[])() = {init_expert_ffn_kernels, init_expert_ffn_bf16_kernels, init_expert_ffn_w8_kernels, init_gemm_bf16_tiled_kernels,
                            init_expert_ffn_f32_tiled_kernels, init_expert_ffn_fused_fp8_kernels, init_gemm_f32_tiled_kernels,
                            init_gemm_bf16_dma_kernels, init_expert_gemm_g256_kernels, init_moe_router_kernels,
                            init_relpos_attention_bf16_kernels, init_gemm_f32_splitk_kernels};
  for (auto init : inits)
    if (int rc = init()) return rc;
  return 0;
}

static int build_binding(m3_engine* e, const BindKey& k, m3_engine::Bound& bd) {
  M3_REQUIRE(k.feat && k.feat_len && k.logits && k.ws, "engine_prepare: null argument");
  const int B = k.B, T = k.T;
  M3_REQUIRE(B > 0 && T >= 7, "engine_prepare: need B > 0 and T >= 7 frames (got B=%d T=%d)", B, T);
  const m3_engine_config& c = e->cfg;
  const int Tp = sub_len(T);
  M3_REQUIRE(Tp < e->pe_rows, "engine_prepare: T'=%d exceeds the positional table (%lld rows)", Tp,
             (long long)e->pe_rows);
  if (int rc = init_engine_kernels()) return rc;
  const bool streaming = k.sstate != nullptr;
  StageBuilder sb{*e, make_plan(c, k.ws, B, T, k.ep_cap), bd,
                  streaming ? carve_stream_state(c, k.sstate, B, k.s_hist) : StreamState()};
  Plan& pl = sb.pl;
  M3_REQUIRE(k.ws_bytes >= pl.bytes, "engine_prepare: workspace %zu bytes < required %zu", k.ws_bytes, pl.bytes);
  const int32_t* feat_len = k.feat_len; float* logits = k.logits;
  bd.key = k; bd.Tp = Tp; bd.S = B * Tp;
  sb.splitk_ws = pl.splitk; sb.splitk_bytes = pl.splitk_bytes;
  {
    GemmParams t;
    t.M = B * Tp; t.N = c.attention_dim; t.K = c.attention_dim; t.w_bf16 = 1;
    bd.a16 = c.weight_dtype != M3_F32 && c.bf16_activations >= 0 && !c.debug_taps && c.embed_dim == c.attention_dim &&
             (c.embed_linear_units % 128) == 0 && (c.hidden_units % 128) == 0 && gemm_bf16w_uses_tiled(t);
  }
  {
    GemmParams t;
    t.M = B * Tp; t.N = c.attention_dim; t.K = c.attention_dim; t.lda = c.attention_dim; t.w_bf16 = 1; t.a_bf16 = 1;
    bd.dma = bd.a16 && c.attention_dim == 128 * kXbStatParts && gemm_bf16w_uses_dma(t);
  }
  bd.packed = use_packed_rows(c, B);
  if (streaming) {
    bd.a16 = bd.dma = bd.packed = false;
  }
  const int S = bd.S, D = c.attention_dim, De = c.embed_dim;

  if (pl.ep_overflow != nullptr) {
    int32_t* ovf = pl.ep_overflow;
    add_stage(sb, "ep.reset", 0, [=](hipStream_t s) {
      M3_CHECK_HIP(hipMemsetAsync(ovf, 0, sizeof(int32_t), s));
      return 0;
    });
    bd.buffers["ep.overflow"] = Buf{ovf, sizeof(int32_t)};
  }
  {
    int32_t* lens = pl.lens;
    if (bd.packed) {
      int32_t* row0 = pl.row0; int32_t* pad_of = pl.pad_of;
      add_stage(sb, "pack_plan", 1, [=](hipStream_t s) { return launch_pack_plan(lens, B, Tp, row0, pad_of, s, feat_len); },
                stage_info("pack_plan_kernel", 1, 12.0 * B + 4.0 * B * Tp, 0.0, false));
    } else if (pl.fork || (!c.fold_pos_proj && !streaming)) {
      add_stage(sb, "lens", 1, [=](hipStream_t s) { return launch_subsample_lens(feat_len, B, lens, s); },
                stage_info("subsample_lens_kernel", 1, 8.0 * B, 0.0, false));
    } else {
      sb.lens_in_conv1 = true;
    }
  }
  {
    const int nb = c.num_blocks + c.embed_blocks;
    GemmParams pp;
    const int Tpos = streaming ? k.s_maxf : Tp;
    pp.A = e->pe; pp.lda = D; pp.W = e->pos_all; pp.Y = pl.pbuf; pp.ldy = nb * D; pp.M = Tpos; pp.N = nb * D; pp.K = D;
    if (c.fold_pos_proj || streaming) {
      auto known = e->pfold_by_tp.find(Tpos);
      std::shared_ptr<float> pf = known != e->pfold_by_tp.end() ? known->second.lock() : nullptr;
      if (!pf) {
        float* dev = nullptr;
        M3_CHECK_HIP(hipMalloc((void**)&dev, (size_t)Tpos * nb * D * sizeof(float)));
        pf = std::shared_ptr<float>(dev, [](float* q) { (void)hipFree(q); });
        pp.Y = dev;
        pp.w_bf16 = c.weight_dtype != M3_F32;
        if (int rc = launch_gemm_f32(pp, nullptr)) return rc;
        M3_CHECK_HIP(hipStreamSynchronize(nullptr));
        for (auto it = e->pfold_by_tp.begin(); it != e->pfold_by_tp.end();)
          it = it->second.expired() ? e->pfold_by_tp.erase(it) : std::next(it);
        e->pfold_by_tp[Tpos] = pf;
      }
      bd.pfold = pf;
      pl.pbuf = pf.get();
    } else {
      add_gemm(sb, "pos_all", pp);
    }
  }
  const Plan ple = embed_view(pl);
  const int embed_start = (int)bd.stages.size();
  sb.splitk_ws = ple.splitk;
  build_subsample(sb, "embed.subsample.", e->sub_e, De, ple, ple.x);
  for (int i = 0; i < c.embed_blocks; ++i) {
    if (i + 1 == c.embed_blocks) {
      sb.tail_ln_g = e->e_after.g; sb.tail_ln_b = e->e_after.b; sb.tail_ln_eps = 1e-12f; sb.tail_ln_out = pl.emb;
    }
    build_block(sb, "embed.blocks." + std::to_string(i) + ".", e->eblocks[i], De, c.embed_linear_units, c.embed_heads,
                c.cnn_module_kernel, c.embed_cnn_layer_norm, false, i, i, ple, c.embed_causal > 0);
  }
  sb.splitk_ws = pl.splitk;
  if (c.embed_blocks == 0) {
    float* x = ple.x; float* emb = pl.emb;
    const float* g = e->e_after.g; const float* b = e->e_after.b;
    add_stage(sb, "embed.after_norm", 1, [=](hipStream_t s) { return launch_layernorm(x, g, b, 1e-12f, emb, S, De, s); },
              stage_info("layernorm_kernel", 1, 8.0 * S * De, 8.0 * S * De));
  }
  if (choose_moe_route(c, S, e->mblocks.empty() ? BlockW() : e->mblocks[0], pl).needs_e_all) {
    GemmParams g;
    g.A = pl.emb; g.lda = De; g.W = e->router_e_all; g.Y = pl.eall; g.ldy = c.num_blocks * c.num_experts;
    g.M = S; g.N = c.num_blocks * c.num_experts; g.K = De;
    add_gemm(sb, "router_e_all", g, true);
    bd.stages.back().reads_embed = true;
  }
  const int main_start = (int)bd.stages.size();
  build_subsample(sb, "subsample.", e->sub_m, D, pl, pl.x);
  for (int i = 0; i < c.num_blocks; ++i)
    build_block(sb, "blocks." + std::to_string(i) + ".", e->mblocks[i], D, c.hidden_units, c.attention_heads,
                c.cnn_module_kernel, c.cnn_layer_norm, true, i, c.embed_blocks + i, pl, c.causal > 0);
  {
    GemmParams g;
    g.A = pl.x; g.lda = D; g.W = e->out_linear.w; g.bias = e->out_linear.b; g.Y = logits; g.ldy = c.output_dim;
    g.M = S; g.N = c.output_dim; g.K = D;
    g.ln_wsum = e->out_linear.wsum; g.ln_eps = 1e-12f;
    if (bd.a16) { g.A = (const float*)pl.xb; g.a_bf16 = 1; }
    if (bd.dma) { g.ln_stats = pl.xstats; g.ln_stat_parts = kXbStatParts; }
    float* lout = logits;
    if (bd.packed) {
      lout = pl.lpk;
      g.Y = lout;
      g.m_dev = pl.row0 + B;
    }
    add_gemm(sb, "logits", g);
    const float* ob = e->output_bias;
    const int V = c.output_dim;
    if (c.log_softmax_out) {
      add_stage(sb, "log_softmax", 1, [=](hipStream_t s) { return launch_log_softmax_bias(lout, ob, lout, (size_t)S, V, s); },
                stage_info("log_softmax_bias_kernel", 1, 8.0 * S * V, 4.0 * S * V));
    }
    if (bd.packed) {
      const int32_t* row0 = pl.row0;
      add_stage(sb, "unpack", 1, [=](hipStream_t s) { return launch_unpack_rows(lout, row0, B, Tp, V, logits, s); },
                stage_info("unpack_rows_kernel", 1, 8.0 * S * V, 0.0, false));
    }
  }
  const int join = embed_join(bd.stages, main_start);
  if (pl.fork && join >= 0 && c.num_blocks >= 1) {
    bd.fork_first = embed_start; bd.fork_mid = main_start; bd.join_at = join;
  }
  if (pl.hfuse && !streaming && join > 0) fuse_independent_pairs(sb, embed_start, main_start, join);
  if (streaming) {
    const StreamState& st = sb.st;
    int32_t* step = st.step;
    if (k.s_slots) {
      int32_t *pos = st.slot_pos, *status = st.slot_status, *frames = st.slot_frames;
      const int32_t* lens = pl.lens; const int max_chunks = k.s_maxf / Tp;
      add_stage(sb, "stream.advance", 1, [=](hipStream_t s) { return launch_advance_slots(pos, status, frames, lens, B, Tp, max_chunks, s); },
                stage_info("advance_slots_kernel", 1, 20.0 * B, 0.0, false));
    } else
    add_stage(sb, "stream.advance", 1, [=](hipStream_t s) { return launch_advance_counter(step, 1, s); },
              stage_info("advance_counter_kernel", 1, 8.0, 0.0, false));
  }
  bd.buffers["x"] = Buf{pl.x, (size_t)S * D * 4};
  if (!bd.xn_skipped) bd.buffers["xn"] = Buf{pl.xn, (size_t)S * D * 4};
  if (pl.xq != nullptr) {
    bd.buffers["xq"] = Buf{pl.xq, (size_t)S * D};
    bd.buffers["xq_scale"] = Buf{pl.xq_scale, (size_t)S * 4};
  }
  bd.buffers["embed"] = Buf{pl.emb, (size_t)S * De * 4};
  if (bd.a16) bd.buffers["xb"] = Buf{pl.xb, (size_t)S * D * 2};
  bd.buffers["lens"] = Buf{pl.lens, (size_t)B * 4};
  if (bd.packed) bd.buffers["row0"] = Buf{pl.row0, (size_t)(B + 1) * 4};
  if (pl.ep_rows) bd.buffers["ep.gate_recv"] = Buf{pl.ep_gate_recv, (size_t)pl.ep_rows * 4};
  bd.buffers["router_logits"] = Buf{pl.rl, (size_t)S * c.num_experts * (c.ep_world_size > 0 ? c.ep_world_size : 1) * 4};

  return 0;
}

static int find_parked(const m3_engine* e, const BindKey& k) {
  for (size_t i = 0; i < e->parked.size(); ++i)
    if (e->parked[i].matches(k)) return (int)i;
  return -1;
}

static int shape_cache_capacity(const m3_engine* e) { return e->cfg.shape_cache > 0 ? e->cfg.shape_cache : (e->cfg.shape_cache < 0 ? 0 : 7); }

static int park_victim(const m3_engine* e) {
  if (e->parked.empty() || (int)e->parked.size() < shape_cache_capacity(e)) return -1;
  size_t lru = 0;
  for (size_t i = 1; i < e->parked.size(); ++i)
    if (e->parked[i].last_use < e->parked[lru].last_use) lru = i;
  return (int)lru;
}

static void park_current(m3_engine* e) {
  if (e->cur.stages.empty()) return;
  if (shape_cache_capacity(e) > 0) {
    const int victim = park_victim(e);
    if (victim >= 0) {
      if (e->parked[victim].graph_exec) (void)hipGraphExecDestroy(e->parked[victim].graph_exec);
      e->parked.erase(e->parked.begin() + victim);
    }
    e->parked.push_back(std::move(e->cur));
  } else if (e->cur.graph_exec) {
    (void)hipGraphExecDestroy(e->cur.graph_exec);
  }
  e->cur = m3_engine::Bound();
}

static int bind(m3_engine* e, const BindKey& k) {
  if (!e->cur.matches(k)) {
    int hit = find_parked(e, k);
    if (hit >= 0 && !e->cur.stages.empty() && hit == park_victim(e)) hit = -1;
    m3_engine::Bound fresh;
    if (hit < 0)
      if (int rc = build_binding(e, k, fresh)) return rc;
    park_current(e);
    if (hit >= 0) {
      hit = find_parked(e, k);
      fresh = std::move(e->parked[hit]);
      e->parked.erase(e->parked.begin() + hit);
    }
    e->cur = std::move(fresh);
  }
  e->cur.last_use = ++e->use_clock;
  return 0;
}

static BindKey forward_key(const m3_engine* e, const float* feat, const int32_t* feat_len, int B, int T, float* logits,
                           void* workspace, size_t workspace_bytes) {
  BindKey k;
  k.B = B; k.T = T; k.feat = feat; k.feat_len = feat_len; k.logits = logits; k.ws = workspace; k.ws_bytes = workspace_bytes;
  k.ep_cap = e->ep_capacity;
  return k;
}

int m3_engine_prepare(m3_engine* e, const float* feat, const int32_t* feat_len, int B, int T, float* logits,
                      void* workspace, size_t workspace_bytes) {
  M3_REQUIRE(e != nullptr, "engine_prepare: null argument");
  if (int rc = bind(e, forward_key(e, feat, feat_len, B, T, logits, workspace, workspace_bytes))) return rc;
  return (int)e->cur.stages.size();
}

int m3_engine_set_ep_capacity(m3_engine* engine, int rows_per_chunk) {
  M3_REQUIRE(engine != nullptr && rows_per_chunk >= 0, "engine_set_ep_capacity: bad argument");
  engine->ep_capacity = rows_per_chunk;
  return 0;
}

int m3_engine_num_stages(const m3_engine* engine) { return engine ? (int)engine->cur.stages.size() : 0; }
const char* m3_engine_stage_name(const m3_engine* engine, int index) {
  if (!engine || index < 0 || index >= (int)engine->cur.stages.size()) return nullptr;
  return engine->cur.stages[index].name.c_str();
}
// ... 193 lines not shown
```

### 3m-asr-inference_amd/csrc/gemm_f32_splitk.hip

```cpp
#include "common.h"
#include "kernels.h"

namespace m3 {

namespace {
constexpr int SBM = 64, SBN = 64, SBK = 64;
constexpr int S_LD = SBK + 4;
constexpr int SC_LD = SBN + 4;
constexpr int kSplitLdsBytes = 2 * (SBM + SBN) * S_LD * 4;
}

template <bool CONV>
__global__ __launch_bounds__(256, 2) void gemm_f32_splitk_kernel(const GemmParams p, float* __restrict__ part,
                                                                 int ksteps_per_split) {
  constexpr int MT = SBM / 32, NT = SBN / 32;
  constexpr int CA = SBK / 4, RA = 256 / CA, JA = SBM / RA, JB = SBN / RA;
  extern __shared__ __attribute__((aligned(16))) unsigned char splitk_lds[];
  float* As = reinterpret_cast<float*>(splitk_lds);
  float* Bs = As + 2 * SBM * S_LD;
  float* Cs = reinterpret_cast<float*>(splitk_lds);

  const int tid = threadIdx.x, lane = tid & 63, wave = tid >> 6;
  const int col = lane & 15, kq = lane >> 4;
  const int wm = wave >> 1, wn = wave & 1;
  const int n_tile = blockIdx.x % p.n_tiles, m_tile = blockIdx.x / p.n_tiles, split = blockIdx.y;
  const int m0 = m_tile * SBM, n0 = n_tile * SBN;
  const int nsteps_total = p.K / SBK;
  const int s_lo = split * ksteps_per_split, s_hi = min(s_lo + ksteps_per_split, nsteps_total);

  const int ac = tid % CA, ar0 = tid / CA;
  const float* aptr[JA];
#pragma unroll
  for (int j = 0; j < JA; ++j) {
    const int m = min(m0 + ar0 + RA * j, p.M - 1);
    if (CONV) {
      const int f2 = m % p.conv_F2;
      const int t2 = (m / p.conv_F2) % p.conv_T2;
      const int b = m / (p.conv_F2 * p.conv_T2);
      aptr[j] = p.A + ((size_t)(b * p.conv_T1 + 2 * t2) * p.conv_F1 + 2 * f2) * p.conv_C + 4 * ac;
    } else {
      aptr[j] = p.A + (size_t)m * p.lda + 4 * ac;
    }
  }
  const float* bptr[JB];
#pragma unroll
  for (int j = 0; j < JB; ++j) bptr[j] = p.W + (size_t)min(n0 + ar0 + RA * j, p.N - 1) * p.K + 4 * ac;
  auto a_offset = [&](int k) -> int {
    if (CONV) {
      const int seg = k / p.conv_C, c = k - seg * p.conv_C;
      const int kh = seg / 3, kw = seg - kh * 3;
      return (kh * p.conv_F1 + kw) * p.conv_C + c;
    }
    return k;
  };

  f32x4 acc[MT][NT];
#pragma unroll
  for (int mt = 0; mt < MT; ++mt)
#pragma unroll
    for (int nt = 0; nt < NT; ++nt) acc[mt][nt] = f32x4{0.f, 0.f, 0.f, 0.f};

  f32x4 areg[JA], breg[JB];
  auto load_tiles = [&](int s) {
    const int ko = a_offset(s * SBK);
#pragma unroll
    for (int j = 0; j < JA; ++j) areg[j] = ldg4(aptr[j] + ko);
#pragma unroll
    for (int j = 0; j < JB; ++j) breg[j] = ldg4_w(bptr[j] + s * SBK);
  };
  auto store_tiles = [&](int buf) {
    float* a_dst = As + buf * (SBM * S_LD) + ar0 * S_LD + 4 * ac;
    float* b_dst = Bs + buf * (SBN * S_LD) + ar0 * S_LD + 4 * ac;
#pragma unroll
    for (int j = 0; j < JA; ++j) *reinterpret_cast<f32x4*>(a_dst + RA * j * S_LD) = areg[j];
#pragma unroll
    for (int j = 0; j < JB; ++j) *reinterpret_cast<f32x4*>(b_dst + RA * j * S_LD) = breg[j];
  };

  load_tiles(s_lo);
  store_tiles(0);
  __syncthreads();
  for (int s = s_lo; s < s_hi; ++s) {
    const int i = s - s_lo;
    load_tiles(min(s + 1, s_hi - 1));
    __builtin_amdgcn_sched_barrier(0);
    const float* a_lds = As + (i & 1) * (SBM * S_LD) + ((SBM / 2) * wm + col) * S_LD + 4 * kq;
    const float* b_lds = Bs + (i & 1) * (SBN * S_LD) + ((SBN / 2) * wn + col) * S_LD + 4 * kq;
#pragma unroll
    for (int ks = 0; ks < SBK / 16; ++ks) {
      f32x4 b[NT];
#pragma unroll
      for (int nt = 0; nt < NT; ++nt) b[nt] = *reinterpret_cast<const f32x4*>(b_lds + 16 * nt * S_LD + 16 * ks);
#pragma unroll
      for (int mt = 0; mt < MT; ++mt) {
        const f32x4 a = *reinterpret_cast<const f32x4*>(a_lds + 16 * mt * S_LD + 16 * ks);
#pragma unroll
        for (int nt = 0; nt < NT; ++nt)
#pragma unroll
          for (int j = 0; j < 4; ++j) acc[mt][nt] = mfma16(a[j], b[nt][j], acc[mt][nt]);
      }
    }
    __builtin_amdgcn_sched_barrier(0);
    store_tiles((i + 1) & 1);
    __syncthreads();
  }

#pragma unroll
  for (int mt = 0; mt < MT; ++mt)
#pragma unroll
    for (int nt = 0; nt < NT; ++nt)
#pragma unroll
      for (int r = 0; r < 4; ++r)
        Cs[((SBM / 2) * wm + 16 * mt + 4 * kq + r) * SC_LD + (SBN / 2) * wn + 16 * nt + col] = acc[mt][nt][r];
  __syncthreads();
  const int c4 = 4 * (lane & 15), n = n0 + c4;
  for (int it = 0; it < SBM / 16; ++it) {
    const int row = (4 * it + wave) * 4 + (lane >> 4);
    const int m = m0 + row;
    if (m < p.M && n < p.N) stg4(part + ((size_t)split * p.M + m) * p.N + n, *reinterpret_cast<const f32x4*>(Cs + row * SC_LD + c4));
  }
}

__global__ __launch_bounds__(256) void splitk_reduce_kernel(const float* __restrict__ part, int splits, int M, int N,
                                                            const float* __restrict__ bias, int act, float alpha,
                                                            float* __restrict__ y, int ldy) {
  const size_t quads = (size_t)M * (N / 4);
  for (size_t q = (size_t)blockIdx.x * 256 + threadIdx.x; q < quads; q += (size_t)gridDim.x * 256) {
    const int m = (int)(q / (N / 4)), n = 4 * (int)(q % (N / 4));
    f32x4 v = bias ? ldg4(bias + n) : f32x4{0.f, 0.f, 0.f, 0.f};
    for (int s0 = 0; s0 < splits; s0 += 4) {
      f32x4 t[4];
#pragma unroll
      for (int j = 0; j < 4; ++j)
        t[j] = (s0 + j < splits) ? ldg4(part + ((size_t)(s0 + j) * M + m) * N + n) : f32x4{0.f, 0.f, 0.f, 0.f};
#pragma unroll
      for (int j = 0; j < 4; ++j) v += t[j];
    }
#pragma unroll
    for (int e = 0; e < 4; ++e) {
      float t = v[e];
      if (act == ACT_RELU) t = fmaxf(t, 0.f);
      if (act == ACT_SILU) t = silu(t);
      v[e] = t * alpha;
    }
    stg4(y + (size_t)m * ldy + n, v);
  }
}

int init_gemm_f32_splitk_kernels() {
  static PerDeviceOnce once;
  if (once.done()) return 0;
  M3_CHECK_HIP(hipFuncSetAttribute((const void*)gemm_f32_splitk_kernel<true>, hipFuncAttributeMaxDynamicSharedMemorySize, kSplitLdsBytes));
  M3_CHECK_HIP(hipFuncSetAttribute((const void*)gemm_f32_splitk_kernel<false>, hipFuncAttributeMaxDynamicSharedMemorySize, kSplitLdsBytes));
  once.mark();
  return 0;
}

int gemm_f32_splitk_plan(const GemmParams& p, size_t* ws_bytes) {
  if (ws_bytes) *ws_bytes = 0;
  if (p.w_bf16 || p.K < 4096 || (p.K & 63) || (p.N & 3) || (p.lda & 3) || (p.ldy & 3)) return 0;
  if (p.mode == GEMM_A_CONCAT2 || p.ln_wsum || p.ln_gamma || p.mask_in || p.mask_out || p.resid || p.act == ACT_GLU) return 0;
  if (p.mode == GEMM_A_CONV3X3S2 && (p.conv_C & 63)) return 0;
  const long tiles = (long)cdiv(p.M, SBM) * cdiv(p.N, SBN);
  if (tiles > 160) return 0;
  const int nsteps = p.K / SBK;
  int splits = (int)(512 / tiles);
  if (splits > nsteps / 4) splits = nsteps / 4;
  if (splits < 2) return 0;
  const int per = cdiv(nsteps, splits);
  splits = cdiv(nsteps, per);
  if (ws_bytes) *ws_bytes = (size_t)splits * p.M * p.N * sizeof(float);
  return splits;
}

int launch_gemm_f32_splitk(const GemmParams& pin, float* ws, size_t ws_bytes, hipStream_t stream) {
  GemmParams p = pin;
  size_t need = 0;
  const int splits = gemm_f32_splitk_plan(p, &need);
  M3_REQUIRE(splits >= 2 && ws != nullptr && ws_bytes >= need, "gemm split-K: not applicable / workspace %zu < %zu", ws_bytes, need);
  if (int rc = init_gemm_f32_splitk_kernels()) return rc;
  p.m_tiles = cdiv(p.M, SBM);
  p.n_tiles = cdiv(p.N, SBN);
  const int per = cdiv(p.K / SBK, splits);
  dim3 grid(p.m_tiles * p.n_tiles, splits);
  if (p.mode == GEMM_A_CONV3X3S2)
    hipLaunchKernelGGL((gemm_f32_splitk_kernel<true>), grid, dim3(256), kSplitLdsBytes, stream, p, ws, per);
  else
    hipLaunchKernelGGL((gemm_f32_splitk_kernel<false>), grid, dim3(256), kSplitLdsBytes, stream, p, ws, per);
  const size_t quads = (size_t)p.M * (p.N / 4);
  hipLaunchKernelGGL(splitk_reduce_kernel, dim3(grid1d(quads, 1024)), dim3(256), 0, stream, ws, splits, p.M, p.N, p.bias, p.act,
                     p.alpha, p.Y, p.ldy);
  M3_LAUNCH_CHECK();
  return 0;
}

}
```

### 3m-asr-inference_amd/csrc/kernels.h

```cpp
#pragma once
#include <hip/hip_runtime.h>
#include <stdint.h>

#include "../../include/m3asr.h"

namespace m3 {

enum { ACT_NONE = 0, ACT_RELU = 1, ACT_SILU = 2, ACT_GLU = 3 };
enum { GEMM_A_PLAIN = 0, GEMM_A_CONCAT2 = 1, GEMM_A_CONV3X3S2 = 2 };

struct GemmParams {
  const float* A = nullptr; int lda = 0;
  const float* A2 = nullptr; int lda2 = 0; int K1 = 0;
  const float* W = nullptr;
  int w_bf16 = 0;
  const float* bias = nullptr;
  float* Y = nullptr; int ldy = 0;
  int M = 0, N = 0, K = 0;
  int mode = GEMM_A_PLAIN;
  const float* ln_gamma = nullptr; const float* ln_beta = nullptr; float ln_eps = 0.f;
  const float* ln_wsum = nullptr; const float* ln_wbeta = nullptr;
  int ln_on_a2 = 0;
  float* ln_out = nullptr; int ld_ln_out = 0;
  const int32_t* row_len = nullptr; int rows_per_batch = 0;
  int mask_in = 0, mask_out = 0;
  int conv_T1 = 0, conv_F1 = 0, conv_T2 = 0, conv_F2 = 0, conv_C = 0;
  int act = ACT_NONE;
  float alpha = 1.f;
  const float* resid = nullptr; int ldr = 0;
  const int32_t* grp_acc = nullptr; int grp_E = 0; const int32_t* grp_pos = nullptr; int w_sliced = 0;
  const float* w_scale = nullptr;
  int a_bf16 = 0, y_bf16 = 0; void* Yb = nullptr; int ldyb = 0;
  float* Yb_stats = nullptr; const float* ln_stats = nullptr; int ln_stat_parts = 0;
  const int32_t* m_dev = nullptr;
  const int32_t* y_rows = nullptr;
  const int32_t* conv_len = nullptr;
  int n_tiles = 0, m_tiles = 0, xcd_swizzle = 0;
};
int launch_gemm_f32(const GemmParams& p, hipStream_t stream);
bool gemm_f32_dual_fusable(const GemmParams& a, const GemmParams& b);
int launch_gemm_f32_dual(const GemmParams& a, const GemmParams& b, hipStream_t stream);
int launch_gemm_bf16w(const GemmParams& p, hipStream_t stream);
const char* gemm_kernel_label(const GemmParams& p, bool splitk);
bool gemm_bf16w_uses_tiled(const GemmParams& p);
int gemm_f32_splitk_plan(const GemmParams& p, size_t* ws_bytes);
int launch_gemm_f32_splitk(const GemmParams& p, float* ws, size_t ws_bytes, hipStream_t stream);
int init_gemm_f32_splitk_kernels();
int init_gemm_bf16_tiled_kernels();
constexpr int kXbStatParts = 4;
bool gemm_bf16_dma_supports(const GemmParams& p);
int gemm_bf16_dma_col_tiles(const GemmParams& p);
bool gemm_bf16w_uses_dma(const GemmParams& p);
int launch_gemm_bf16_dma(const GemmParams& p, hipStream_t stream);
int init_gemm_bf16_dma_kernels();
int launch_row_stats_bf16(const void* xb, int rows, int D, float* stats, hipStream_t stream);
int init_gemm_f32_tiled_kernels();

int launch_moe_index(const int32_t* gate_idx, int S, int E, int32_t* mapping, int32_t* acc_hist,
                     int32_t* pos, hipStream_t stream);
int launch_moe_gate_index(const float* logits, int width, const int32_t* row_len, int rows_per_batch, int S,
                          int32_t* gate_idx, float* gate_value, int32_t* mapping, int32_t* acc_hist, int32_t* pos,
                          hipStream_t stream);
int launch_moe_route(const float* x, int ldx, int D, const float* wx, const float* wsum, const float* bias,
                     const float* eall, int ld_e, float ln_eps, const int32_t* row_len, int rows_per_batch, int S, int E,
                     int32_t* gate_idx, float* gate_value, int32_t* mapping, int32_t* acc_hist, int32_t* pos,
                     hipStream_t stream);
bool moe_router_supports(int De, int D, int N);
bool moe_router_fuses_top1(int N);
int init_moe_router_kernels();
int launch_moe_router(const float* emb, int lde, int De, const float* x, int ldx, int D, const float* W, const float* bias,
                      const float* gamma, const float* beta, float eps, float* xn, int ldxn, float* Y, int ldy, int M, int N,
                      const int32_t* m_dev, hipStream_t stream, int32_t* gate_idx = nullptr, float* gate_val = nullptr,
                      const int32_t* row_len = nullptr, int rows_per_batch = 0, void* xq = nullptr, float* xq_scale = nullptr);
int launch_local_scatter(const void* x, const int32_t* mapping, int S, int row_bytes, void* out, hipStream_t stream);
int launch_local_gather(const void* buf, const int32_t* mapping, int S, int row_bytes, void* out, hipStream_t stream);

int launch_ep_send_map(const int32_t* gate_idx, const int32_t* mapping, const int32_t* acc_hist, int S, int world, int e_loc,
                       int capacity, int32_t* map_send, void* wire, int row_bytes, hipStream_t stream, int32_t* overflow = nullptr);
int launch_ep_send_rows(const int32_t* gate_idx, const int32_t* mapping, const int32_t* acc_hist, int S, int world, int e_loc,
                        int capacity, int32_t* map_send, const void* x, void* wire, int row_bytes, hipStream_t stream, int32_t* overflow = nullptr);
int launch_ep_recv_gate(const void* wire, int world, int e_loc, int capacity, int row_bytes, int32_t* gate_recv,
                        hipStream_t stream);

#ifndef M3_EXPERT_SLICE
#define M3_EXPERT_SLICE 64
#endif
constexpr int kExpertSliceW16 = 64;
constexpr int kExpertSlice = M3_EXPERT_SLICE;
size_t expert_ffn_slab_bytes(int S, int D, int F);
enum class ExpertWeights { F32, BF16, FP8, FP8A8 };
enum class ExpertKernel { SlabF32, TiledF32, SlabBf16, TiledBf16, G256Bf16, SlabW8, TiledW8, FusedFp8 };
struct ExpertFfnPlan {
  ExpertWeights weights; ExpertKernel kernel;
  const char* label;
  int launches, slices;
  int fsplit;
  size_t h_off, rows_off, xb_off;
  float* rows(float* slab) const { return (float*)((char*)slab + rows_off); }
};
enum { EXPERT_NORM_IN_KERNEL = 1,
       EXPERT_SCATTER_ROWS = 2 };
ExpertFfnPlan plan_expert_ffn(ExpertWeights w, int S, int E, int D, int F, unsigned flags = 0);
struct ExpertFfnArgs { const float* x; int ldx; const int32_t *pos, *acc_hist; const void *w1, *w2; const float *s1, *s2, *b1, *b2;
                       int w2_sliced; float h_scale; float* slab; const float *ln_gamma, *ln_beta; float ln_eps;
                       const void* xq; const float* xq_scale; int32_t* fs_dev; float* y_scatter; };
int launch_expert_ffn(const ExpertFfnPlan& plan, int S, int E, int D, int F, const ExpertFfnArgs& a, hipStream_t stream);
int init_expert_ffn_kernels();
int launch_expert_ffn_f32_slab(const float* x, int ldx, const int32_t* pos, const int32_t* acc_hist, int S, int E,
                               int D, int F, const float* w1, const float* b1, const float* w2, int w2_sliced, float* slab,
                               const float* ln_gamma, const float* ln_beta, float ln_eps, hipStream_t stream);
int init_expert_ffn_f32_tiled_kernels();
int launch_expert_tiled_f32(const float* x, int ldx, const int32_t* pos, const int32_t* acc_hist, int S, int E,
                            int D, int F, const float* w1, const float* b1, const float* w2, int w2_sliced,
                            float* hbuf, float* ybuf, hipStream_t stream);
int init_expert_ffn_bf16_kernels();
int launch_expert_ffn_bf16w_slab(const float* x, int ldx, const int32_t* pos, const int32_t* acc_hist, int S, int E,
                                 int D, int F, const void* w1, const float* b1, const void* w2, int w2_sliced, float* slab,
                                 hipStream_t stream);
int init_expert_ffn_w8_kernels();
int launch_expert_ffn_w8_slab(const float* x, int ldx, const int32_t* pos, const int32_t* acc_hist, int S, int E, int D, int F,
                              const void* w1, const float* s1, const float* b1, const void* w2, const float* s2, int w2_sliced,
                              float* slab, hipStream_t stream);
constexpr int kExpertFusedFp8MaxSplit = 4;
int expert_ffn_fused_fp8_fsplit(int S, int E, int D, int F);
int init_expert_ffn_fused_fp8_kernels();
int launch_expert_ffn_fused_fp8(const float* x, int ldx, const int32_t* pos, const int32_t* acc_hist, int S, int E, int D, int F,
                                const void* w1, const float* s1, const float* b1, const void* w2, const float* s2, int w2_sliced,
                                float h_scale, int fsplit, float* ybuf, hipStream_t stream, const void* xq = nullptr,
                                const float* xq_scale = nullptr, int32_t* fs_dev = nullptr);
int launch_quantize_rows_e4m3(const float* x, int ldx, int S, int D, void* xq, float* scale, hipStream_t stream);
int launch_expert_tiled_w16(bool w_fp8, const float* x, int ldx, const int32_t* pos, const int32_t* acc_hist, int S, int E,
                            int D, int F, const void* w1, const float* s1, const float* b1, const void* w2, const float* s2,
                            int w2_sliced, void* hbuf, float* ybuf, hipStream_t stream, const float* b2 = nullptr,
                            float* y_scatter = nullptr);
bool expert_ffn_f32_self_routing(int S, int E);
int launch_expert_route_ffn_f32(const float* x, int ldx, const float* logits, const int32_t* row_len, int rows_per_batch, int S, int E,
                                int D, int F, const float* w1, const float* b1, const float* w2, int w2_sliced, const float* b2,
                                float* slab, int32_t* gate_idx, float* gate_value, int32_t* mapping, int32_t* acc_hist, int32_t* pos,
                                hipStream_t stream, const float* ln_gamma = nullptr, const float* ln_beta = nullptr, float ln_eps = 0.f);
bool expert_gemm_g256_takes(int S, int E, int D, int F);
int init_expert_gemm_g256_kernels();
int launch_rows_to_bf16(const float* x, int ldx, int S, int D, void* xb, hipStream_t stream);
int launch_expert_ffn_bf16_g256(const void* xb, int ldxb, const int32_t* pos, const int32_t* acc_hist, int S, int E, int D, int F,
                                const void* w1, const float* b1, const void* w2, int w2_sliced, void* hbuf, float* ybuf,
                                hipStream_t stream);
int launch_moe_combine(const float* slab, int n_slices, const int32_t* mapping, const int32_t* gate_idx,
                       const float* gate_value, const float* b2, const float* resid, float alpha,
                       const float* ln_gamma, const float* ln_beta, float ln_eps, float* out, int S, int D,
                       hipStream_t stream, void* out_bf16 = nullptr, float* out_stats = nullptr,
                       const int32_t* n_slices_dev = nullptr);

int launch_layernorm(const float* x, const float* gamma, const float* beta, float eps, float* y, int rows, int D,
                     hipStream_t stream, void* y_bf16 = nullptr, float* y_stats = nullptr, const float* gamma2 = nullptr,
                     const float* beta2 = nullptr, float eps2 = 0.f, float* y2 = nullptr);
int launch_softmax_top1(const float* logits, int ld, const int32_t* row_len, int rows_per_batch, int S, int E,
                        int32_t* idx, float* value, hipStream_t stream);
int launch_att_masked_softmax(const float* scores, const int32_t* len, int B, int H, int T1, int T2, float scale,
                              float* out, hipStream_t stream);
int launch_masked_fill(const float* x, const int32_t* len, int B, int C, int T, float fill, float* y,
                       hipStream_t stream);
int launch_glu(const float* x, int outer, int C, int inner, float* y, hipStream_t stream);
int launch_scale(const float* x, float scale, float* y, size_t n, hipStream_t stream);
int launch_mask_conv2d_sample(const int32_t* len_in, int B, int left_padding, int stride, int32_t* len_out,
                              hipStream_t stream);
int launch_subsample_lens(const int32_t* len_in, int B, int32_t* len_out, hipStream_t stream);
int launch_add(const float* a, const float* b, float* y, size_t n, hipStream_t stream);
int launch_binary_bcast(const float* a, const float* b, float* y, const int64_t* shape, const int64_t* sa,
                        const int64_t* sb, int nd, int op, hipStream_t stream);
int launch_unary(const float* x, float* y, size_t n, int act, hipStream_t stream);
int launch_permute(const float* x, float* y, const int64_t* out_shape, const int64_t* in_strides, int nd,
                   hipStream_t stream);
int launch_concat_last(const float* a, int da, const float* b, int db, float* y, size_t rows, hipStream_t stream);
int launch_softmax_lastdim(const float* x, float* y, size_t rows, int n, hipStream_t stream);
int launch_bmm(const float* a, const float* b, float* c, int batch, int M, int N, int K, int64_t sa, int64_t sb,
               int trans_b, hipStream_t stream);

int launch_relpos_attention(const float* qkv, int ldq, const float* pmat, int ldp, const float* pos_u,
                            const float* pos_v, const int32_t* row_len, int B, int T, int H, int dk, float scale,
                            float* out, int ldo, hipStream_t stream, int out_bf16 = 0, const int32_t* row0 = nullptr,
                            int chunk = 0, int left_chunks = -1);
struct AttArgs {
  const float* qkv = nullptr; int ldq = 0; const float* pmat = nullptr; int ldp = 0; const float *pos_u = nullptr, *pos_v = nullptr;
  const int32_t* row_len = nullptr; int B = 0, T = 0, H = 0, dk = 0; float scale = 1.f; float* out = nullptr; int ldo = 0, out_bf16 = 0;
  const int32_t* row0 = nullptr; int chunk = 0, left_chunks = 0;
};
int launch_relpos_attention_args(const AttArgs& a, hipStream_t stream);
bool relpos_attention_dual_fusable(const AttArgs& a, const AttArgs& b);
int launch_relpos_attention_dual(const AttArgs& a, const AttArgs& b, hipStream_t stream);
int launch_relpos_attention_stream(const float* qkv, int ldq, float* hist, int cap, const float* pmat, int ldp, const float* pos_u,
                                   const float* pos_v, const int32_t* chunk_len, const int32_t* step, int B, int C, int H, int dk,
                                   float scale, float* out, int ldo, int left_chunks, hipStream_t stream,
                                   int slot_max_chunks = -1);

bool relpos_attention_bf16_supports(int T, int dk);
int init_relpos_attention_bf16_kernels();
int launch_relpos_attention_bf16(const void* qkv, int ldq, const float* pmat, int ldp, const float* pos_u, const float* pos_v,
                                 const int32_t* row_len, int B, int T, int H, int dk, float scale, void* out, int ldo,
                                 hipStream_t stream, const int32_t* row0 = nullptr, int chunk = 0, int left_chunks = -1);

int launch_dwconv_ln_silu(const float* z, const float* w_kc, const float* bias, const float* gamma,
                          const float* beta, float eps, int B, int T, int D, int K, float* out, hipStream_t stream,
                          int out_bf16 = 0, const int32_t* pad_of = nullptr, const int32_t* row0 = nullptr,
                          const int32_t* row_len = nullptr, const float* causal_left_fill = nullptr);
int launch_pad2d(const float* x, size_t outer, int H, int W, int pre_h, int post_h, int pre_w, int post_w, float* y, hipStream_t stream);
int launch_advance_counter(int32_t* counter, int by, hipStream_t stream);
int launch_fill_rows(const float* row, int D, float* out, size_t rows, hipStream_t stream);
int launch_advance_slots(int32_t* pos, int32_t* status, int32_t* frames, const int32_t* chunk_len, int B, int C, int max_chunks,
                         hipStream_t stream);
constexpr int kMaxStreamBlocks = 64;
struct SlotResetArgs {
  int32_t *pos = nullptr, *status = nullptr, *frames = nullptr;
  const int32_t* slots = nullptr; int n = 0;
  int B = 0, K = 0, D = 0, n_blocks = 0;
  float* conv[kMaxStreamBlocks];
  const float* fill[kMaxStreamBlocks];
};
int launch_reset_slots(const SlotResetArgs& a, hipStream_t stream);
int launch_slot_positions(const int32_t* status, const int32_t* frames, int B, int32_t* out, hipStream_t stream);
struct DwArgs {
  const float *z = nullptr, *w_kc = nullptr, *bias = nullptr, *gamma = nullptr, *beta = nullptr; float eps = 1e-5f;
  int B = 0, T = 0, D = 0, K = 0; float* out = nullptr; int out_bf16 = 0;
  const int32_t *pad_of = nullptr, *row0 = nullptr, *row_len = nullptr; const float* causal_left_fill = nullptr;
};
int launch_dwconv_ln_silu_args(const DwArgs& a, hipStream_t stream);
bool dwconv_dual_fusable(const DwArgs& a, const DwArgs& b);
int launch_dwconv_ln_silu_dual(const DwArgs& a, const DwArgs& b, hipStream_t stream);
int launch_dwconv_ln_silu_stream(const float* z, const float* w_kc, const float* bias, const float* gamma, const float* beta,
                                 float eps, int B, int T, int D, int K, float* out, float* cache_pair, const int32_t* step,
                                 const int32_t* chunk_len, hipStream_t stream, int out_bf16 = 0,
                                 int slot_max_chunks = -1);
int launch_pack_plan(int32_t* len, int B, int T, int32_t* row0, int32_t* pad_of, hipStream_t stream,
                     const int32_t* feat_len = nullptr);
int launch_unpack_rows(const float* in, const int32_t* row0, int B, int T, int n, float* out, hipStream_t stream);
int launch_conv1_relu(const float* feat, const float* w9c, const float* bias, const float* cmvn_mean,
                      const float* cmvn_istd, int B, int T, int idim, int C, float* out, hipStream_t stream, int relu = 1,
                      int out_bf16 = 0, const int32_t* feat_len = nullptr, int32_t* lens_out = nullptr);
int launch_cmvn(const float* x, const int32_t* len, const float* mean, const float* istd, int B, int T, int D,
                float* y, hipStream_t stream);
int launch_log_softmax_bias(const float* x, const float* bias, float* y, size_t rows, int n, hipStream_t stream);
int launch_ctc_greedy(const float* logits, const int32_t* len, int B, int T, int V, int blank, int32_t* frame_ids,
                      int32_t* tokens, int32_t* n_tokens, hipStream_t stream);
int launch_ctc_topk(const float* logits, size_t rows, int V, int k, float* top_logp, int32_t* top_idx, hipStream_t stream);
int ctc_prefix_beam_search_host(const float* top_logp, const int32_t* top_idx, int T, int k, int beam, int blank,
                                int32_t* hyp_tokens, int32_t* hyp_len, float* hyp_score, int32_t* n_hyps);
int launch_ctc_argmax(const float* logits, size_t rows, int V, int32_t* ids, hipStream_t stream);
size_t ctc_beam_state_size(const m3_ctc_beam_desc* d);
int launch_ctc_beam_reset(const m3_ctc_beam_desc* d, void* state, size_t bytes, hipStream_t stream,
                          const int32_t* slots = nullptr, int n = 0);
int launch_ctc_beam_advance(const m3_ctc_beam_desc* d, void* state, size_t bytes, const float* top_logp, const int32_t* top_idx,
                            int T_chunk, const int32_t* n_frames, hipStream_t stream);
int launch_ctc_beam_nbest(const m3_ctc_beam_desc* d, const void* state, size_t bytes, int32_t* hyp_tokens, int32_t* hyp_len,
                          float* hyp_score, int32_t* n_hyps, hipStream_t stream);
size_t ctc_greedy_stream_state_size(const m3_ctc_greedy_desc* d);
int launch_ctc_greedy_stream_reset(const m3_ctc_greedy_desc* d, void* state, size_t bytes, hipStream_t stream,
                                   const int32_t* slots = nullptr, int n = 0);
int launch_ctc_greedy_stream_advance(const m3_ctc_greedy_desc* d, void* state, size_t bytes, const float* logits, int T_chunk,
                                     int V, const int32_t* n_frames, int32_t* frame_ids, hipStream_t stream);
int launch_ctc_greedy_stream_tokens(const m3_ctc_greedy_desc* d, const void* state, size_t bytes, int32_t* tokens,
                                    int32_t* n_tokens, hipStream_t stream);
int launch_cat_split_cache(const void* in_cache, const void* input, int B, int cache_dim, int input_dim, void* output,
                           void* out_cache, hipStream_t stream);
int launch_att_stream_softmax(const float* scores, const int32_t* decode_frame_num, const int32_t* mask_idx, int B, int N,
                              int ld, int cache_len, float scale, float* out, hipStream_t stream);
int launch_rel_positional_encoding(const float* x, const float* pe, int pe_len, const int32_t* frame_num, int max_offset,
                                   float scale, int B, int T, int D, float* y, float* pos_emb, int32_t* frame_num_out,
                                   hipStream_t stream);
int launch_depthwise_conv1d_nct(const float* x, const float* w, const float* bias, int B, int C, int T, int K,
                                int pad, float* y, hipStream_t stream);

size_t fbank_tables_bytes();
int fbank_tables_build(int num_mel_bins, double sample_rate, double low_freq, double high_freq, void* host_image);
int launch_fbank(const void* tables, const void* pcm, int pcm_is_int16, int ld_pcm, const int32_t* n_samples, int B, int T,
                 int num_mel_bins, float* feat, int ld_feat, int32_t* feat_len, hipStream_t stream);

}
```

### 3m-asr-inference_amd/m3asr/_lib.py

```python
import ctypes as C
import os

_HERE = os.path.dirname(os.path.abspath(__file__))
LIB_PATH = os.environ.get("M3ASR_LIB") or os.path.join(_HERE, "libm3asr_hip.so")


class M3Error(RuntimeError):
    pass


class Tensor(C.Structure):
    _fields_ = [("data", C.c_void_p), ("dtype", C.c_int32), ("ndim", C.c_int32), ("shape", C.c_int64 * 8)]


class Field(C.Structure):
    _fields_ = [("name", C.c_char_p), ("data", C.c_void_p), ("type", C.c_int32), ("length", C.c_int32)]


class LinearDesc(C.Structure):
    _fields_ = [("a", C.c_void_p), ("lda", C.c_int32),
                ("a2", C.c_void_p), ("lda2", C.c_int32), ("k1", C.c_int32),
                ("w", C.c_void_p), ("bias", C.c_void_p),
                ("y", C.c_void_p), ("ldy", C.c_int32),
                ("M", C.c_int32), ("N", C.c_int32), ("K", C.c_int32),
                ("ln_gamma", C.c_void_p), ("ln_beta", C.c_void_p), ("ln_eps", C.c_float),
                ("ln_wsum", C.c_void_p), ("ln_wbeta", C.c_void_p),
                ("len", C.c_void_p), ("rows_per_batch", C.c_int32), ("mask_in", C.c_int32), ("mask_out", C.c_int32),
                ("act", C.c_int32), ("alpha", C.c_float),
                ("resid", C.c_void_p), ("ldr", C.c_int32), ("weight_dtype", C.c_int32),
                ("a_dtype", C.c_int32), ("y_dtype", C.c_int32), ("y_copy_bf16", C.c_void_p), ("ld_copy", C.c_int32),
                ("y_copy_stats", C.c_void_p), ("ln_stats", C.c_void_p), ("ln_stat_parts", C.c_int32)]


class EngineConfig(C.Structure):
    _fields_ = [(n, C.c_int32) for n in (
        "input_dim", "output_dim", "attention_dim", "attention_heads", "num_blocks",
        "embed_dim", "embed_heads", "embed_linear_units", "embed_blocks",
        "num_experts", "hidden_units", "cnn_module_kernel", "cnn_layer_norm", "embed_cnn_layer_norm",
        "router_with_bias", "keep_expert_output", "ep_world_size", "ep_rank", "fold_pos_proj", "debug_taps", "log_softmax_out", "fuse_route",
        "shape_cache", "bf16_activations", "weight_dtype", "packed_rows", "fp8_activations", "ep_stages", "fork_embed", "static_chunk_size", "num_left_chunks", "causal", "embed_causal")]


class StreamDesc(C.Structure):
    _fields_ = [("B", C.c_int32), ("history_frames", C.c_int32), ("max_frames", C.c_int32)]


class CtcBeamDesc(C.Structure):
    _fields_ = [("B", C.c_int32), ("beam", C.c_int32), ("k", C.c_int32), ("max_frames", C.c_int32), ("blank", C.c_int32)]


class CtcGreedyDesc(C.Structure):
    _fields_ = [("B", C.c_int32), ("max_frames", C.c_int32), ("blank", C.c_int32)]


class WeightEntry(C.Structure):
    _fields_ = [("name", C.c_char_p), ("data", C.c_void_p), ("numel", C.c_int64), ("dtype", C.c_int32)]


FIELD_FLOAT32, FIELD_INT32 = 1, 5
F32, F16, I8, I32, BF16, FP8 = 0, 1, 2, 3, 4, 5
ACT_NONE, ACT_RELU, ACT_SILU, ACT_GLU, ACT_SIGMOID, ACT_LOG = 0, 1, 2, 3, 4, 5
OP_SUM, OP_PROD = 0, 1

_vp, _i, _f, _sz, _i64, _cp = C.c_void_p, C.c_int, C.c_float, C.c_size_t, C.c_int64, C.c_char_p
_P = C.POINTER

class StageInfo(C.Structure):
    _fields_ = [("kernel", C.c_char_p), ("launches", C.c_int32), ("per_row", C.c_int32),
                ("alg_bytes", C.c_double), ("flops", C.c_double)]


SIGNATURES = {
    "m3_abi_version": (_i, []),
    "m3_last_error": (_cp, []),
    "m3_registry_lookup": (_i, [_cp, _cp]),
    "m3_registry_count": (_i, []),
    "m3_registry_name": (_cp, [_i]),
    "m3_plugin_create": (_vp, [_cp, _cp, _P(Field), _i]),
    "m3_plugin_clone": (_vp, [_vp]),
    "m3_plugin_destroy": (None, [_vp]),
    "m3_plugin_type": (_cp, [_vp]),
    "m3_plugin_num_outputs": (_i, [_vp]),
    "m3_plugin_output_dims": (_i, [_vp, _P(Tensor), _i, _P(Tensor), _i]),
    "m3_plugin_workspace_size": (_sz, [_vp, _P(Tensor), _i, _P(Tensor), _i]),
    "m3_plugin_enqueue": (_i, [_vp, _P(Tensor), _i, _P(Tensor), _i, _vp, _sz, _vp]),
    "m3_plugin_serialization_size": (_sz, [_vp]),
    "m3_plugin_serialize": (_i, [_vp, _vp, _sz]),
    "m3_plugin_deserialize": (_vp, [_cp, _cp, _vp, _sz]),
    "m3_moe_scatter_mapping": (_i, [_vp, _i, _i, _vp, _vp, _vp, _vp]),
    "m3_moe_local_scatter": (_i, [_vp, _vp, _i, _i, _vp, _vp]),
    "m3_moe_local_gather": (_i, [_vp, _vp, _i, _i, _vp, _vp]),
    "m3_moe_expert_slice": (_i, []),
    "m3_moe_expert_workspace_size": (_sz, [_i, _i, _i, _i]),
    "m3_moe_expert_ffn": (_i, [_vp, _vp, _vp, _vp, _vp, _vp, _i, _i, _i, _i, _vp, _vp, _f, _vp, _vp, _f, _vp,
                               _vp, _sz, _vp]),
    "m3_moe_expert_ffn_bf16": (_i, [_vp, _vp, _vp, _vp, _vp, _vp, _i, _i, _i, _i, _vp, _vp, _f, _vp, _vp, _f, _vp,
                                    _vp, _sz, _vp]),
    "m3_moe_expert_ffn_fp8": (_i, [_vp, _vp, _vp, _vp, _vp, _vp, _vp, _vp, _i, _i, _i, _i, _vp, _vp, _f, _vp, _vp, _f, _vp,
                                   _vp, _sz, _vp]),
    "m3_moe_expert_ffn_fp8a8": (_i, [_vp, _vp, _vp, _vp, _vp, _vp, _vp, _vp, _f, _i, _i, _i, _i, _vp, _vp, _f, _vp, _vp, _f, _vp,
                                     _vp, _sz, _vp]),
    "m3_moe_expert_ffn_fp8a8_active": (_i, [_i, _i, _i, _i]),
    "m3_moe_expert_ffn_kernel": (C.c_char_p, [_i, _i, _i, _i, _i, _i, _vp, _vp]),
    "m3_moe_expert_ffn_fp8a8_xq": (_i, [_vp, _vp, _vp, _vp, _vp, _vp, _vp, _vp, _vp, _vp, _f, _i, _i, _i, _i, _vp, _vp, _f, _vp, _vp,
                                        _f, _vp, _vp, _sz, _vp]),
    "m3_quantize_rows_e4m3": (_i, [_vp, _i, _i, _i, _vp, _vp, _vp]),
    "m3_moe_combine": (_i, [_vp, _vp, _vp, _vp, _f, _vp, _vp, _f, _vp, _i, _i, _vp]),
    "m3_moe_combine_bf16": (_i, [_vp, _vp, _vp, _vp, _f, _vp, _vp, _f, _vp, _vp, _i, _i, _vp]),
    "m3_softmax_top1": (_i, [_vp, _i, _vp, _i, _i, _i, _vp, _vp, _vp]),
    "m3_moe_router": (_i, [_vp, _i, _i, _vp, _i, _i, _vp, _vp, _vp, _vp, _f, _vp, _i, _vp, _i, _i, _i, _vp]),
    "m3_moe_gate_index": (_i, [_vp, _vp, _i, _i, _i, _vp, _vp, _vp, _vp, _vp, _vp]),
    "m3_moe_route": (_i, [_vp, _i, _i, _vp, _vp, _vp, _vp, _i, _f, _vp, _i, _i, _i, _vp, _vp, _vp, _vp, _vp, _vp]),
    "m3_moe_route_expert_workspace_size": (_sz, [_i, _i, _i, _i]),
    "m3_moe_route_expert_ffn": (_i, [_vp, _i, _vp, _vp, _i, _vp, _vp, _vp, _i, _vp, _i, _i, _i, _i, _vp, _vp, _f, _i, _vp, _f,
                                     _vp, _vp, _f, _vp, _vp, _vp, _vp, _vp, _vp, _vp, _sz, _vp]),
    "m3_linear": (_i, [_P(LinearDesc), _vp]),
    "m3_linear_workspace_size": (_sz, [_P(LinearDesc)]),
    "m3_linear_kernel": (C.c_char_p, [_P(LinearDesc), _i]),
    "m3_linear_ws": (_i, [_P(LinearDesc), _vp, _sz, _vp]),
    "m3_conv2d_3x3s2_first": (_i, [_vp, _vp, _vp, _i, _i, _i, _i, _i, _vp, _vp]),
    "m3_conv2d_3x3s2": (_i, [_vp, _vp, _vp, _i, _i, _i, _i, _i, _vp, _vp]),
    "m3_layer_norm": (_i, [_vp, _vp, _vp, _f, _vp, _i, _i, _vp]),
    "m3_relpos_attention": (_i, [_vp, _i, _vp, _i, _vp, _vp, _vp, _i, _i, _i, _i, _f, _vp, _i, _vp]),
    "m3_relpos_attention_bf16": (_i, [_vp, _i, _vp, _i, _vp, _vp, _vp, _i, _i, _i, _i, _f, _i, _i, _vp, _i, _vp]),
    "m3_relpos_attention_chunk": (_i, [_vp, _i, _vp, _i, _vp, _vp, _vp, _i, _i, _i, _i, _f, _i, _i, _vp, _i, _vp]),
    "m3_dwconv_ln_silu": (_i, [_vp, _vp, _vp, _vp, _vp, _f, _i, _i, _i, _i, _vp, _vp]),
    "m3_subsample_conv1": (_i, [_vp, _vp, _vp, _i, _i, _i, _i, _vp, _vp]),
    "m3_subsample_conv1_cmvn": (_i, [_vp, _vp, _vp, _vp, _vp, _i, _i, _i, _i, _vp, _vp]),
    "m3_cmvn": (_i, [_vp, _vp, _vp, _vp, _i, _i, _i, _vp, _vp]),
    "m3_log_softmax_bias": (_i, [_vp, _vp, _vp, _sz, _i, _vp]),
    "m3_subsample_conv2": (_i, [_vp, _vp, _vp, _i, _i, _i, _i, _vp, _vp]),
    "m3_ctc_greedy": (_i, [_vp, _vp, _i, _i, _i, _i, _vp, _vp, _vp, _vp]),
    "m3_ctc_topk": (_i, [_vp, _sz, _i, _i, _vp, _vp, _vp]),
    "m3_ctc_prefix_beam_search": (_i, [_vp, _vp, _i, _i, _i, _i, _vp, _vp, _vp, _vp]),
    "m3_ctc_beam_state_size": (_sz, [_P(CtcBeamDesc)]),
    "m3_ctc_beam_reset": (_i, [_P(CtcBeamDesc), _vp, _sz, _vp]),
    "m3_ctc_beam_reset_slots": (_i, [_P(CtcBeamDesc), _vp, _sz, _vp, _i, _vp]),
    "m3_ctc_beam_advance": (_i, [_P(CtcBeamDesc), _vp, _sz, _vp, _vp, _i, _vp, _vp]),
    "m3_ctc_beam_nbest": (_i, [_P(CtcBeamDesc), _vp, _sz, _vp, _vp, _vp, _vp, _vp]),
    "m3_ctc_greedy_stream_state_size": (_sz, [_P(CtcGreedyDesc)]),
    "m3_ctc_greedy_stream_reset": (_i, [_P(CtcGreedyDesc), _vp, _sz, _vp]),
    "m3_ctc_greedy_stream_reset_slots": (_i, [_P(CtcGreedyDesc), _vp, _sz, _vp, _i, _vp]),
    "m3_ctc_greedy_stream_advance": (_i, [_P(CtcGreedyDesc), _vp, _sz, _vp, _i, _i, _vp, _vp, _vp]),
    "m3_ctc_greedy_stream_tokens": (_i, [_P(CtcGreedyDesc), _vp, _sz, _vp, _vp, _vp]),
    "m3_cat_split_cache": (_i, [_vp, _vp, _i, _i, _i, _vp, _vp, _vp]),
    "m3_att_stream_softmax": (_i, [_vp, _vp, _vp, _i, _i, _i, _i, _f, _vp, _vp]),
    "m3_rel_positional_encoding": (_i, [_vp, _vp, _i, _vp, _i, _f, _i, _i, _i, _vp, _vp, _vp, _vp]),
    "m3_att_masked_softmax": (_i, [_vp, _vp, _i, _i, _i, _i, _f, _vp, _vp]),
    "m3_masked_fill": (_i, [_vp, _vp, _i, _i, _i, _f, _vp, _vp]),
    "m3_glu": (_i, [_vp, _i, _i, _i, _vp, _vp]),
    "m3_mask_conv2d_sample": (_i, [_vp, _i, _i, _i, _vp, _vp]),
    "m3_scale": (_i, [_vp, _f, _vp, _sz, _vp]),
    "m3_unary": (_i, [_vp, _vp, _sz, _i, _vp]),
    "m3_binary": (_i, [_vp, _vp, _vp, _P(_i64), _P(_i64), _P(_i64), _i, _i, _vp]),
    "m3_permute": (_i, [_vp, _vp, _P(_i64), _P(_i64), _i, _vp]),
    "m3_concat_last": (_i, [_vp, _i, _vp, _i, _vp, _sz, _vp]),
    "m3_softmax": (_i, [_vp, _vp, _sz, _i, _vp]),
    "m3_batched_matmul": (_i, [_vp, _vp, _vp, _i, _i, _i, _i, _i64, _i64, _i, _vp]),
    "m3_pad2d": (_i, [_vp, _sz, _i, _i, _i, _i, _i, _i, _vp, _vp]),
    "m3_depthwise_conv1d": (_i, [_vp, _vp, _vp, _i, _i, _i, _i, _i, _vp, _vp]),
    "m3_engine_create": (_vp, [_P(EngineConfig), _P(WeightEntry), _i]),
    "m3_engine_destroy": (None, [_vp]),
    "m3_engine_output_frames": (_i, [_i]),
    "m3_engine_workspace_size": (_sz, [_vp, _i, _i]),
    "m3_engine_forward": (_i, [_vp, _vp, _vp, _i, _i, _vp, _vp, _sz, _i, _vp]),
    "m3_engine_prepare": (_i, [_vp, _vp, _vp, _i, _i, _vp, _vp, _sz]),
    "m3_engine_chunk_input_frames": (_i, [_vp]),
    "m3_engine_stream_state_size": (_sz, [_vp, _P(StreamDesc)]),
    "m3_engine_stream_reset": (_i, [_vp, _P(StreamDesc), _vp, _sz, _vp]),
    "m3_engine_forward_chunk": (_i, [_vp, _P(StreamDesc), _vp, _sz, _vp, _vp, _vp, _vp, _sz, _i, _i, _vp]),
    "m3_engine_stream_reset_slots": (_i, [_vp, _P(StreamDesc), _vp, _sz, _vp, _i, _vp]),
    "m3_engine_forward_chunk_slots": (_i, [_vp, _P(StreamDesc), _vp, _sz, _vp, _vp, _vp, _vp, _sz, _i, _vp]),
    "m3_engine_stream_positions": (_i, [_vp, _P(StreamDesc), _vp, _sz, _vp, _vp]),
    "m3_engine_set_ep_capacity": (_i, [_vp, _i]),
    "m3_engine_num_captures": (_i, [_vp]),
    "m3_engine_num_stages": (_i, [_vp]),
    "m3_engine_stage_name": (_cp, [_vp, _i]),
    "m3_engine_run": (_i, [_vp, _i, _i, _vp]),
    "m3_engine_buffer": (_i, [_vp, _cp, _P(_vp), _P(_sz)]),
    "m3_engine_num_kernels": (_i, [_vp]),
    "m3_engine_stage_info": (_i, [_vp, _i, _vp]),
    "m3_ep_send_map": (_i, [_vp, _vp, _vp, _i, _i, _i, _i, _vp, _vp, _i, _vp]),
    "m3_ep_recv_gate": (_i, [_vp, _i, _i, _i, _i, _vp, _vp]),
    "m3_fbank_tables_bytes": (_sz, [_i]),
    "m3_fbank_tables_host": (_i, [_i, _f, _f, _f, _vp]),
    "m3_fbank_tables_init": (_i, [_i, _f, _f, _f, _vp, _vp]),
    "m3_fbank_num_frames": (_i, [_i]),
    "m3_fbank": (_i, [_vp, _vp, _i, _i, _vp, _i, _i, _i, _vp, _i, _vp, _vp]),
}

_lib = None


def load():
    global _lib
    if _lib is not None:
        return _lib
    if not os.path.exists(LIB_PATH):
        raise M3Error("libm3asr_hip.so not found at %s -- build it with `make -C 3m-asr-inference_amd` "
                      "(or __graft_entry__.build()); there is no CPU fallback" % LIB_PATH)
    lib = C.CDLL(LIB_PATH, mode=C.RTLD_GLOBAL)
    for name, (res, args) in SIGNATURES.items():
        fn = getattr(lib, name)
        fn.restype = res
        fn.argtypes = args
    _lib = lib
    return lib


def last_error():
    return load().m3_last_error().decode()


def check(status, what):
    if status != 0:
        raise M3Error("%s failed (status %d): %s" % (what, status, last_error()))
```

### include/m3asr.h

```cpp
#ifndef M3ASR_H_
#define M3ASR_H_
#include <stddef.h>
#include <stdint.h>

#ifdef __cplusplus
extern "C" {
#endif

#define M3ASR_ABI_VERSION 10

typedef void* m3_stream;

enum m3_dtype { M3_F32 = 0, M3_F16 = 1, M3_I8 = 2, M3_I32 = 3, M3_BF16 = 4, M3_FP8 = 5  };

enum m3_act { M3_ACT_NONE = 0, M3_ACT_RELU = 1, M3_ACT_SILU = 2, M3_ACT_GLU = 3, M3_ACT_SIGMOID = 4, M3_ACT_LOG = 5 };
enum m3_binop { M3_OP_SUM = 0, M3_OP_PROD = 1 };

int m3_abi_version(void);
const char* m3_last_error(void);
int m3_registry_lookup(const char* plugin_name, const char* plugin_version);
int m3_registry_count(void);
const char* m3_registry_name(int index);

typedef struct m3_tensor {
  void* data;
  int32_t dtype;
  int32_t ndim;
  int64_t shape[8];
} m3_tensor;

enum m3_field_type { M3_FIELD_FLOAT32 = 1, M3_FIELD_INT32 = 5 };
typedef struct m3_field {
  const char* name;
  const void* data;
  int32_t type;
  int32_t length;
} m3_field;

typedef struct m3_plugin m3_plugin;

m3_plugin* m3_plugin_create(const char* plugin_name, const char* plugin_version, const m3_field* fields,
                            int n_fields);
m3_plugin* m3_plugin_clone(const m3_plugin* plugin);
void m3_plugin_destroy(m3_plugin* plugin);
const char* m3_plugin_type(const m3_plugin* plugin);
int m3_plugin_num_outputs(const m3_plugin* plugin);
int m3_plugin_output_dims(const m3_plugin* plugin, const m3_tensor* inputs, int n_in, m3_tensor* outputs,
                          int n_out);
size_t m3_plugin_workspace_size(const m3_plugin* plugin, const m3_tensor* inputs, int n_in,
                                const m3_tensor* outputs, int n_out);
int m3_plugin_enqueue(m3_plugin* plugin, const m3_tensor* inputs, int n_in, m3_tensor* outputs, int n_out,
                      void* workspace, size_t workspace_bytes, m3_stream stream);
size_t m3_plugin_serialization_size(const m3_plugin* plugin);
int m3_plugin_serialize(const m3_plugin* plugin, void* buffer, size_t bytes);
m3_plugin* m3_plugin_deserialize(const char* plugin_name, const char* plugin_version, const void* buffer,
                                 size_t bytes);

int m3_moe_scatter_mapping(const int32_t* gate_idx, int S, int num_expert, int32_t* mapping,
                           int32_t* acc_histogram, int32_t* pos, m3_stream stream);
int m3_moe_local_scatter(const void* x, const int32_t* mapping, int S, int row_bytes, void* out,
                         m3_stream stream);
int m3_moe_local_gather(const void* buf, const int32_t* mapping, int S, int row_bytes, void* out,
                        m3_stream stream);
int m3_moe_expert_slice(void);
size_t m3_moe_expert_workspace_size(int S, int num_expert, int idim, int hidden_units);
int m3_moe_expert_ffn(const float* x, const int32_t* gate_idx, const float* w1, const float* b1,
                      const float* w2, const float* b2, int S, int num_expert, int idim, int hidden_units,
                      const float* gate_value, const float* resid, float alpha, const float* ln_gamma,
                      const float* ln_beta, float ln_eps, float* y, void* workspace, size_t workspace_bytes,
                      m3_stream stream);
int m3_moe_expert_ffn_bf16(const float* x, const int32_t* gate_idx, const void* w1, const float* b1,
                           const void* w2, const float* b2, int S, int num_expert, int idim, int hidden_units,
                           const float* gate_value, const float* resid, float alpha, const float* ln_gamma,
                           const float* ln_beta, float ln_eps, float* y, void* workspace, size_t workspace_bytes,
                           m3_stream stream);
int m3_moe_expert_ffn_fp8(const float* x, const int32_t* gate_idx, const void* w1, const float* w1_scale,
                          const float* b1, const void* w2, const float* w2_scale, const float* b2, int S, int num_expert,
                          int idim, int hidden_units, const float* gate_value, const float* resid, float alpha,
                          const float* ln_gamma, const float* ln_beta, float ln_eps, float* y, void* workspace,
                          size_t workspace_bytes, m3_stream stream);
int m3_moe_expert_ffn_fp8a8(const float* x, const int32_t* gate_idx, const void* w1, const float* w1_scale,
                            const float* b1, const void* w2, const float* w2_scale, const float* b2, float h_scale, int S,
                            int num_expert, int idim, int hidden_units, const float* gate_value, const float* resid,
                            float alpha, const float* ln_gamma, const float* ln_beta, float ln_eps, float* y,
                            void* workspace, size_t workspace_bytes, m3_stream stream);
int m3_moe_expert_ffn_fp8a8_active(int S, int num_expert, int idim, int hidden_units);
const char* m3_moe_expert_ffn_kernel(int weight_dtype, int fp8_activations, int S, int num_expert, int idim, int hidden_units,
                                     int32_t* launches, int32_t* slices);
int m3_moe_expert_ffn_fp8a8_xq(const float* x, const void* xq, const float* xq_scale, const int32_t* gate_idx, const void* w1,
                               const float* w1_scale, const float* b1, const void* w2, const float* w2_scale, const float* b2,
                               float h_scale, int S, int num_expert, int idim, int hidden_units, const float* gate_value,
                               const float* resid, float alpha, const float* ln_gamma, const float* ln_beta, float ln_eps,
                               float* y, void* workspace, size_t workspace_bytes, m3_stream stream);
int m3_quantize_rows_e4m3(const float* x, int ldx, int S, int idim, void* xq, float* scale, m3_stream stream);
int m3_moe_combine(const float* rows, const int32_t* mapping, const float* gate_value, const float* resid,
                   float alpha, const float* ln_gamma, const float* ln_beta, float ln_eps, float* out, int S,
                   int idim, m3_stream stream);
int m3_moe_combine_bf16(const float* rows, const int32_t* mapping, const float* gate_value, const float* resid,
                        float alpha, const float* ln_gamma, const float* ln_beta, float ln_eps, float* out,
                        void* out_bf16, int S, int idim, m3_stream stream);
int m3_ep_send_map(const int32_t* gate_idx, const int32_t* mapping, const int32_t* acc_histogram, int S, int world, int e_loc,
                   int capacity, int32_t* map_send, void* wire, int row_bytes, m3_stream stream);
int m3_ep_recv_gate(const void* wire, int world, int e_loc, int capacity, int row_bytes, int32_t* gate_recv, m3_stream stream);
int m3_moe_router(const float* embed, int ld_embed, int embed_dim, const float* x, int ldx, int idim, const float* w,
                  const float* bias, const float* ln_gamma, const float* ln_beta, float ln_eps, float* xn, int ld_xn,
                  float* logits, int ld_logits, int S, int num_expert, m3_stream stream);
int m3_softmax_top1(const float* logits, int ld, const int32_t* len, int rows_per_batch, int S, int width,
                    int32_t* idx, float* value, m3_stream stream);
int m3_moe_gate_index(const float* logits, const int32_t* row_len, int rows_per_batch, int S, int num_expert,
                      int32_t* gate_idx, float* gate_value, int32_t* mapping, int32_t* acc_histogram, int32_t* pos,
                      m3_stream stream);
int m3_moe_route(const float* x, int ldx, int idim, const float* wx, const float* wsum, const float* bias, const float* eall,
                 int ld_e, float ln_eps, const int32_t* row_len, int rows_per_batch, int S, int num_expert, int32_t* gate_idx,
                 float* gate_value, int32_t* mapping, int32_t* acc_histogram, int32_t* pos, m3_stream stream);
size_t m3_moe_route_expert_workspace_size(int S, int num_expert, int idim, int hidden_units);
int m3_moe_route_expert_ffn(const float* x, int ldx, const float* logits, const int32_t* row_len, int rows_per_batch,
                            const float* w1, const float* b1, const float* w2, int w2_sliced, const float* b2, int S,
                            int num_expert, int idim, int hidden_units, const float* norm_gamma, const float* norm_beta,
                            float norm_eps, int use_gate_value, const float* resid, float alpha, const float* ln_gamma,
                            const float* ln_beta, float ln_eps, int32_t* gate_idx, float* gate_value, int32_t* mapping,
                            int32_t* acc_histogram, int32_t* pos, float* y, void* workspace, size_t workspace_bytes,
                            m3_stream stream);

typedef struct m3_linear_desc {
  const float* a; int32_t lda;
  const float* a2; int32_t lda2; int32_t k1;
  const void* w;
  const float* bias;
  float* y; int32_t ldy;
  int32_t M, N, K;
  const float* ln_gamma; const float* ln_beta; float ln_eps;
  const float* ln_wsum; const float* ln_wbeta;
  const int32_t* len; int32_t rows_per_batch; int32_t mask_in; int32_t mask_out;
  int32_t act; float alpha;
  const float* resid; int32_t ldr;
  int32_t weight_dtype;
  int32_t a_dtype, y_dtype;
  void* y_copy_bf16; int32_t ld_copy;
  float* y_copy_stats;
  const float* ln_stats; int32_t ln_stat_parts;
} m3_linear_desc;
int m3_linear(const m3_linear_desc* desc, m3_stream stream);
size_t m3_linear_workspace_size(const m3_linear_desc* desc);
const char* m3_linear_kernel(const m3_linear_desc* desc, int with_workspace);
int m3_linear_ws(const m3_linear_desc* desc, void* workspace, size_t workspace_bytes, m3_stream stream);

int m3_layer_norm(const float* x, const float* gamma, const float* beta, float eps, float* y, int rows, int dim,
                  m3_stream stream);
int m3_relpos_attention(const float* qkv, int ldq, const float* p, int ldp, const float* pos_u,
                        const float* pos_v, const int32_t* len, int B, int T, int H, int dk, float scale,
                        float* out, int ldo, m3_stream stream);
int m3_relpos_attention_bf16(const void* qkv, int ldq, const float* p, int ldp, const float* pos_u, const float* pos_v,
                             const int32_t* len, int B, int T, int H, int dk, float scale, int chunk, int left_chunks,
                             void* out, int ldo, m3_stream stream);
int m3_relpos_attention_chunk(const float* qkv, int ldq, const float* p, int ldp, const float* pos_u, const float* pos_v,
                              const int32_t* len, int B, int T, int H, int dk, float scale, int chunk, int left_chunks,
                              float* out, int ldo, m3_stream stream);
int m3_dwconv_ln_silu(const float* z, const float* w_kc, const float* bias, const float* gamma,
                      const float* beta, float eps, int B, int T, int D, int K, float* out, m3_stream stream);
int m3_subsample_conv1(const float* feat, const float* w9c, const float* bias, int B, int T, int idim, int C,
                       float* out, m3_stream stream);
int m3_subsample_conv1_cmvn(const float* feat, const float* w9c, const float* bias, const float* cmvn_mean,
                            const float* cmvn_istd, int B, int T, int idim, int C, float* out, m3_stream stream);
int m3_conv2d_3x3s2_first(const float* feat, const float* w9c, const float* bias, int B, int T, int idim, int C, int act,
                          float* out, m3_stream stream);
int m3_conv2d_3x3s2(const float* in, const float* w, const float* bias, int B, int T1, int F1, int C, int act, float* out,
                    m3_stream stream);
int m3_subsample_conv2(const float* in, const float* w, const float* bias, int B, int T1, int F1, int C,
                       float* out, m3_stream stream);

int m3_cmvn(const float* x, const int32_t* len, const float* mean, const float* istd, int B, int T, int D, float* y,
            m3_stream stream);
int m3_log_softmax_bias(const float* x, const float* bias, float* y, size_t rows, int n, m3_stream stream);

int m3_ctc_greedy(const float* logits, const int32_t* len, int B, int T, int V, int blank, int32_t* frame_ids,
                  int32_t* tokens, int32_t* n_tokens, m3_stream stream);
int m3_ctc_topk(const float* logits, size_t rows, int V, int k, float* top_logp, int32_t* top_idx, m3_stream stream);
int m3_ctc_prefix_beam_search(const float* top_logp, const int32_t* top_idx, int T, int k, int beam, int blank,
                              int32_t* hyp_tokens, int32_t* hyp_len, float* hyp_score, int32_t* n_hyps);
typedef struct m3_ctc_beam_desc {
  int32_t B;
  int32_t beam;
  int32_t k;
  int32_t max_frames;
  int32_t blank;
} m3_ctc_beam_desc;
size_t m3_ctc_beam_state_size(const m3_ctc_beam_desc* desc);
int m3_ctc_beam_reset(const m3_ctc_beam_desc* desc, void* state, size_t state_bytes, m3_stream stream);
int m3_ctc_beam_reset_slots(const m3_ctc_beam_desc* desc, void* state, size_t state_bytes, const int32_t* slots, int n,
                            m3_stream stream);
int m3_ctc_beam_advance(const m3_ctc_beam_desc* desc, void* state, size_t state_bytes, const float* top_logp,
                        const int32_t* top_idx, int T_chunk, const int32_t* n_frames, m3_stream stream);
int m3_ctc_beam_nbest(const m3_ctc_beam_desc* desc, const void* state, size_t state_bytes, int32_t* hyp_tokens,
                      int32_t* hyp_len, float* hyp_score, int32_t* n_hyps, m3_stream stream);
typedef struct m3_ctc_greedy_desc {
  int32_t B;
  int32_t max_frames;
  int32_t blank;
} m3_ctc_greedy_desc;
size_t m3_ctc_greedy_stream_state_size(const m3_ctc_greedy_desc* desc);
int m3_ctc_greedy_stream_reset(const m3_ctc_greedy_desc* desc, void* state, size_t state_bytes, m3_stream stream);
int m3_ctc_greedy_stream_reset_slots(const m3_ctc_greedy_desc* desc, void* state, size_t state_bytes, const int32_t* slots,
                                     int n, m3_stream stream);
int m3_ctc_greedy_stream_advance(const m3_ctc_greedy_desc* desc, void* state, size_t state_bytes, const float* logits,
                                 int T_chunk, int V, const int32_t* n_frames, int32_t* frame_ids, m3_stream stream);
int m3_ctc_greedy_stream_tokens(const m3_ctc_greedy_desc* desc, const void* state, size_t state_bytes, int32_t* tokens,
                                int32_t* n_tokens, m3_stream stream);

int m3_cat_split_cache(const void* in_cache, const void* input, int B, int cache_dim, int input_dim, void* output,
                       void* out_cache, m3_stream stream);
int m3_att_stream_softmax(const float* scores, const int32_t* decode_frame_num, const int32_t* mask_idx, int B, int N,
                          int ld, int cache_len, float scale, float* out, m3_stream stream);
int m3_rel_positional_encoding(const float* x, const float* pe, int pe_len, const int32_t* frame_num, int max_offset,
                               float scale, int B, int T, int D, float* y, float* pos_emb, int32_t* frame_num_out,
                               m3_stream stream);

int m3_att_masked_softmax(const float* scores, const int32_t* len, int B, int H, int T1, int T2, float scale,
                          float* out, m3_stream stream);
int m3_masked_fill(const float* x, const int32_t* len, int B, int C, int T, float fill, float* y,
                   m3_stream stream);
int m3_glu(const float* x, int outer, int C, int inner, float* y, m3_stream stream);
int m3_mask_conv2d_sample(const int32_t* len_in, int B, int left_padding, int stride, int32_t* len_out,
                          m3_stream stream);
int m3_scale(const float* x, float scale, float* y, size_t n, m3_stream stream);

int m3_unary(const float* x, float* y, size_t n, int act, m3_stream stream);
int m3_binary(const float* a, const float* b, float* y, const int64_t* shape, const int64_t* strides_a,
              const int64_t* strides_b, int ndim, int op, m3_stream stream);
int m3_permute(const float* x, float* y, const int64_t* out_shape, const int64_t* in_strides, int ndim,
               m3_stream stream);
int m3_concat_last(const float* a, int da, const float* b, int db, float* y, size_t rows, m3_stream stream);
int m3_softmax(const float* x, float* y, size_t rows, int n, m3_stream stream);
int m3_batched_matmul(const float* a, const float* b, float* c, int batch, int M, int N, int K,
                      int64_t stride_a, int64_t stride_b, int transpose_b, m3_stream stream);
int m3_pad2d(const float* x, size_t outer, int H, int W, int pre_h, int post_h, int pre_w, int post_w, float* y,
             m3_stream stream);
int m3_depthwise_conv1d(const float* x, const float* w, const float* bias, int B, int C, int T, int K, int pad,
                        float* y, m3_stream stream);

typedef struct m3_engine m3_engine;

typedef struct m3_engine_config {
  int32_t input_dim, output_dim;
  int32_t attention_dim, attention_heads, num_blocks;
  int32_t embed_dim, embed_heads, embed_linear_units, embed_blocks;
  int32_t num_experts, hidden_units;
  int32_t cnn_module_kernel;
  int32_t cnn_layer_norm;
  int32_t embed_cnn_layer_norm;
  int32_t router_with_bias, keep_expert_output;
  int32_t ep_world_size, ep_rank;
  int32_t fold_pos_proj;
  int32_t debug_taps;
  int32_t log_softmax_out;
  int32_t fuse_route;
  int32_t shape_cache;
  int32_t bf16_activations;
  int32_t weight_dtype;
  int32_t packed_rows;
  int32_t fp8_activations;
  int32_t ep_stages;
  int32_t fork_embed;
  int32_t static_chunk_size;
  int32_t num_left_chunks;
  int32_t causal;
  int32_t embed_causal;
} m3_engine_config;

typedef struct m3_weight_entry {
  const char* name;
  const void* data;
  int64_t numel;
  int32_t dtype;
} m3_weight_entry;

m3_engine* m3_engine_create(const m3_engine_config* config, const m3_weight_entry* table, int n_entries);
void m3_engine_destroy(m3_engine* engine);
int m3_engine_output_frames(int T);
size_t m3_engine_workspace_size(const m3_engine* engine, int B, int T);
int m3_engine_forward(m3_engine* engine, const float* feat, const int32_t* feat_len, int B, int T, float* logits,
                      void* workspace, size_t workspace_bytes, int use_graph, m3_stream stream);
int m3_engine_prepare(m3_engine* engine, const float* feat, const int32_t* feat_len, int B, int T, float* logits,
                      void* workspace, size_t workspace_bytes);

typedef struct m3_stream_desc {
  int32_t B;
  int32_t history_frames;
  int32_t max_frames;
} m3_stream_desc;
int m3_engine_chunk_input_frames(const m3_engine* engine);
size_t m3_engine_stream_state_size(const m3_engine* engine, const m3_stream_desc* desc);
int m3_engine_stream_reset(m3_engine* engine, const m3_stream_desc* desc, void* state, size_t state_bytes, m3_stream stream);
int m3_engine_forward_chunk(m3_engine* engine, const m3_stream_desc* desc, void* state, size_t state_bytes,
                            const float* feat_chunk, const int32_t* chunk_feat_len, float* logits, void* workspace,
                            size_t workspace_bytes, int chunk_index, int use_graph, m3_stream stream);
int m3_engine_stream_reset_slots(m3_engine* engine, const m3_stream_desc* desc, void* state, size_t state_bytes,
                                 const int32_t* slots, int n, m3_stream stream);
int m3_engine_forward_chunk_slots(m3_engine* engine, const m3_stream_desc* desc, void* state, size_t state_bytes,
// ... 32 lines not shown
```

Before: 148,700 frames/s.

## Fuse split-K reduction into GEMM tail via arrival counters and dual-launch embed branches

Split-K GEMMs now use per-tile arrival counters so the last-arriving split reduces the partials and applies the epilogue in-kernel. This removes the separate reduce kernel launch. Split-K GEMMs (e.g. conv2 of the subsampling) from the main and embed branches can be fused into one dual kernel, and conv1 of both branches into a dual conv1 kernel. Together these cut kernel count and launch overhead in the graph. The cost is counter memory that must be zeroed, plus atomics and extra partial traffic, and the counters must self-reset correctly across graph replays.

```diff
diff --git a/3m-asr-inference_amd/csrc/api.hip b/3m-asr-inference_amd/csrc/api.hip
--- a/3m-asr-inference_amd/csrc/api.hip
+++ b/3m-asr-inference_amd/csrc/api.hip
@@ -328,6 +328,57 @@
   return launch_gemm_f32(p, (hipStream_t)stream);
 }
 
+static_assert(kSplitkCounters == M3_SPLITK_COUNTERS, "include/m3asr.h promises this many arrival counters");
+size_t m3_linear_splitk_workspace_size(const m3_linear_desc* d, int splits) {
+  GemmParams p;
+  size_t need = 0;
+  if (linear_params(d, &p) == 0) gemm_f32_splitk_splits(p, splits, &need);
+  return need;
+}
+int m3_linear_splitk(const m3_linear_desc* d, int splits, void* workspace, size_t workspace_bytes, int32_t* counters, m3_stream stream) {
+  GemmParams p;
+  if (int rc = linear_params(d, &p)) return rc;
+  if (int rc = linear_pointers(d)) return rc;
+  return launch_gemm_f32_splitk(p, (float*)workspace, workspace_bytes, (hipStream_t)stream, counters, splits);
+}
+int m3_linear_splitk_dual(const m3_linear_desc* a, void* workspace_a, int32_t* counters_a, const m3_linear_desc* b, void* workspace_b,
+                          int32_t* counters_b, size_t workspace_bytes_each, int splits, m3_stream stream) {
+  GemmParams pa, pb;
+  if (int rc = linear_params(a, &pa)) return rc;
+  if (int rc = linear_pointers(a)) return rc;
+  if (int rc = linear_params(b, &pb)) return rc;
+  if (int rc = linear_pointers(b)) return rc;
+  return launch_gemm_f32_splitk_dual(pa, (float*)workspace_a, counters_a, pb, (float*)workspace_b, counters_b, workspace_bytes_each,
+                                     (hipStream_t)stream, splits);
+}
+static int conv2_params(const float* in, const float* w, const float* bias, int B, int T1, int F1, int C, int act, float* out, GemmParams* q) {
+  M3_REQUIRE(B > 0 && T1 >= 3 && F1 >= 3 && C > 0, "conv2d: input (%d,%d,%d,%d) smaller than the kernel", B, T1, F1, C);
+  M3_REQUIRE(act == M3_ACT_NONE || act == M3_ACT_RELU || act == M3_ACT_SILU, "conv2d: act %d", act);
+  GemmParams p;
+  p.mode = GEMM_A_CONV3X3S2;
+  p.A = in; p.lda = 4;
+  p.conv_T1 = T1; p.conv_F1 = F1; p.conv_T2 = (T1 - 3) / 2 + 1; p.conv_F2 = (F1 - 3) / 2 + 1; p.conv_C = C;
+  p.W = w; p.bias = bias; p.Y = out; p.ldy = C;
+  p.M = B * p.conv_T2 * p.conv_F2; p.N = C; p.K = 9 * C;
+  p.act = act;
+  *q = p;
+  return 0;
+}
+size_t m3_conv2d_3x3s2_splitk_workspace_size(int B, int T1, int F1, int C, int splits) {
+  GemmParams p;
+  size_t need = 0;
+  if (B > 0 && T1 >= 3 && F1 >= 3 && C > 0 && conv2_params(nullptr, nullptr, nullptr, B, T1, F1, C, M3_ACT_NONE, nullptr, &p) == 0)
+    gemm_f32_splitk_splits(p, splits, &need);
+  return need;
+}
+int m3_conv2d_3x3s2_splitk(const float* in, const float* w, const float* bias, int B, int T1, int F1, int C, int act, float* out,
+                           int splits, void* workspace, size_t workspace_bytes, int32_t* counters, m3_stream stream) {
+  M3_REQUIRE(in && w && out && aligned16(in) && aligned16(out), "conv2d: null / unaligned in, w or out");
+  GemmParams p;
+  if (int rc = conv2_params(in, w, bias, B, T1, F1, C, act, out, &p)) return rc;
+  return launch_gemm_f32_splitk(p, (float*)workspace, workspace_bytes, (hipStream_t)stream, counters, splits);
+}
+
 int m3_layer_norm(const float* x, const float* gamma, const float* beta, float eps, float* y, int rows, int dim,
                   m3_stream stream) {
   return launch_layernorm(x, gamma, beta, eps, y, rows, dim, (hipStream_t)stream);
diff --git a/3m-asr-inference_amd/csrc/conv.hip b/3m-asr-inference_amd/csrc/conv.hip
--- a/3m-asr-inference_amd/csrc/conv.hip
+++ b/3m-asr-inference_amd/csrc/conv.hip
@@ -229,12 +229,11 @@
                             slot_max_chunks >= 0);
 }
 
-__global__ __launch_bounds__(256) void conv1_relu_kernel(const float* __restrict__ feat, const float* __restrict__ w9c,
-                                                         const float* __restrict__ bias,
-                                                         const float* __restrict__ cmvn_mean,
-                                                         const float* __restrict__ cmvn_istd, int T, int idim, int T1,
-                                                         int F1, int C, float* __restrict__ out, int relu, int out_bf16,
-                                                         const int32_t* __restrict__ feat_len, int32_t* __restrict__ lens_out, int B) {
+__device__ __forceinline__ void conv1_relu_body(const float* __restrict__ feat, const float* __restrict__ w9c,
+                                                const float* __restrict__ bias, const float* __restrict__ cmvn_mean,
+                                                const float* __restrict__ cmvn_istd, int T, int idim, int T1, int F1, int C,
+                                                float* __restrict__ out, int relu, int out_bf16,
+                                                const int32_t* __restrict__ feat_len, int32_t* __restrict__ lens_out, int B) {
   extern __shared__ float xs[];
   const int row = blockIdx.x;
   if (feat_len != nullptr && blockIdx.x == 0 && blockIdx.y == 0)
@@ -285,6 +284,27 @@
   }
 }
 
+__global__ __launch_bounds__(256) void conv1_relu_kernel(const float* __restrict__ feat, const float* __restrict__ w9c,
+                                                         const float* __restrict__ bias,
+                                                         const float* __restrict__ cmvn_mean,
+                                                         const float* __restrict__ cmvn_istd, int T, int idim, int T1,
+                                                         int F1, int C, float* __restrict__ out, int relu, int out_bf16,
+                                                         const int32_t* __restrict__ feat_len, int32_t* __restrict__ lens_out, int B) {
+  conv1_relu_body(feat, w9c, bias, cmvn_mean, cmvn_istd, T, idim, T1, F1, C, out, relu, out_bf16, feat_len, lens_out, B);
+}
+struct Conv1Half {
+  const float *feat, *w9c, *bias, *cmvn_mean, *cmvn_istd; float* out; int relu, out_bf16;
+  const int32_t* feat_len; int32_t* lens_out;
+};
+__global__ __launch_bounds__(256) void conv1_relu_dual_kernel(const Conv1Half h0, const Conv1Half h1, int T, int idim, int T1, int F1,
+                                                              int C, int B) {
+  const Conv1Half& h = blockIdx.z == 0 ? h0 : h1;
+  conv1_relu_body(h.feat, h.w9c, h.bias, h.cmvn_mean, h.cmvn_istd, T, idim, T1, F1, C, h.out, h.relu, h.out_bf16, h.feat_len,
+                  h.lens_out, B);
+}
+
+static int conv1_fsplit(int rows) { return rows >= 2048 ? 1 : (rows >= 512 ? 2 : 5); }
+
 int launch_conv1_relu(const float* feat, const float* w9c, const float* bias, const float* cmvn_mean,
                       const float* cmvn_istd, int B, int T, int idim, int C, float* out, hipStream_t stream, int relu, int out_bf16,
                       const int32_t* feat_len, int32_t* lens_out) {
@@ -293,9 +313,29 @@
   const int T1 = (T - 3) / 2 + 1, F1 = (idim - 3) / 2 + 1;
   if (B * T1 == 0) return 0;
   const int threads = (int)align_up(C / 4, 64);
-  const int fsplit = B * T1 >= 2048 ? 1 : (B * T1 >= 512 ? 2 : 5);
+  const int fsplit = conv1_fsplit(B * T1);
   hipLaunchKernelGGL(conv1_relu_kernel, dim3(B * T1, fsplit), dim3(threads), 3 * idim * sizeof(float), stream,
                      feat, w9c, bias, cmvn_mean, cmvn_istd, T, idim, T1, F1, C, out, relu, out_bf16, feat_len, lens_out, B);
+  M3_LAUNCH_CHECK();
+  return 0;
+}
+
+int launch_conv1_relu_args(const Conv1Args& a, hipStream_t stream) {
+  return launch_conv1_relu(a.feat, a.w9c, a.bias, a.cmvn_mean, a.cmvn_istd, a.B, a.T, a.idim, a.C, a.out, stream, a.relu, a.out_bf16,
+                           a.feat_len, a.lens_out);
+}
+bool conv1_dual_fusable(const Conv1Args& a, const Conv1Args& b) {
+  return a.B == b.B && a.T == b.T && a.idim == b.idim && a.C == b.C && a.B > 0 && a.T >= 3 && a.idim >= 3 && (a.C & 3) == 0 &&
+         a.C <= 1024 && a.out != b.out;
+}
+int launch_conv1_relu_dual(const Conv1Args& a, const Conv1Args& b, hipStream_t stream) {
+  M3_REQUIRE(conv1_dual_fusable(a, b), "subsampling (dual): the two problems do not share a shape");
+  const int T1 = (a.T - 3) / 2 + 1, F1 = (a.idim - 3) / 2 + 1;
+  const int threads = (int)align_up(a.C / 4, 64);
+  const Conv1Half h0{a.feat, a.w9c, a.bias, a.cmvn_mean, a.cmvn_istd, a.out, a.relu, a.out_bf16, a.feat_len, a.lens_out};
+  const Conv1Half h1{b.feat, b.w9c, b.bias, b.cmvn_mean, b.cmvn_istd, b.out, b.relu, b.out_bf16, b.feat_len, b.lens_out};
+  hipLaunchKernelGGL(conv1_relu_dual_kernel, dim3(a.B * T1, conv1_fsplit(a.B * T1), 2), dim3(threads), 3 * a.idim * sizeof(float), stream,
+                     h0, h1, a.T, a.idim, T1, F1, a.C, a.B);
   M3_LAUNCH_CHECK();
   return 0;
 }
diff --git a/3m-asr-inference_amd/csrc/engine.hip b/3m-asr-inference_amd/csrc/engine.hip
--- a/3m-asr-inference_amd/csrc/engine.hip
+++ b/3m-asr-inference_amd/csrc/engine.hip
@@ -42,7 +42,8 @@
 
 struct SubW { const float* c1w; const float* c1b; const float* c2w; const float* c2b; Lin out; };
 
-enum class FuseKind { None, Gemm, Dwconv, Attention };
+enum class FuseKind { None, Gemm, Dwconv, Attention, Conv1, SplitK };
+struct SplitkArgs { float* ws = nullptr; size_t ws_bytes = 0; int32_t* counters = nullptr; };
 
 struct Stage {
   std::string name;
@@ -53,6 +54,8 @@
   GemmParams gemm;
   DwArgs dw;
   AttArgs att;
+  Conv1Args conv1;
+  SplitkArgs sk;
 };
 
 m3_stage_info stage_info(const char* kernel, int launches, double bytes, double flops, bool per_row = true) {
@@ -127,6 +130,7 @@
   int gate_index_max_rows;
   bool self_route;
   bool hfuse;
+  bool splitk_tail;
   int router_min_rows;
   bool router_xq;
   bool router_skip_xn;
@@ -139,6 +143,7 @@
     w.gate_index_max_rows = num("M3_GATE_INDEX_MAX_ROWS", 512);
     w.self_route = num("M3_SELF_ROUTE", 1) != 0;
     w.hfuse = num("M3_HFUSE", 1) != 0;
+    w.splitk_tail = num("M3_SPLITK_TAIL", 1) != 0;
     w.router_min_rows = num("M3_ROUTER_MIN_ROWS", 2048);
     w.router_xq = num("M3_ROUTER_XQ", 1) != 0;
     w.router_skip_xn = num("M3_ROUTER_SKIP_XN", 0) != 0;
@@ -271,6 +276,7 @@
 };
 
 struct Plan {
+  int32_t* splitk_cnt;
   int32_t* lens;
   float *c1, *c2, *x, *emb, *h1, *qkv, *pbuf, *ctx, *glu, *dw, *xn, *rl, *eall;
   void* xb;
@@ -310,6 +316,7 @@
   const int F = c.hidden_units > c.embed_linear_units ? c.hidden_units : c.embed_linear_units;
   const int world = c.ep_world_size > 0 ? c.ep_world_size : 1;
   const int Etot = c.num_experts * world;
+  p.splitk_cnt = cv.take<int32_t>(2 * kSplitkCounters);
   p.lens = cv.take<int32_t>(B);
   p.c1 = cv.take<float>((size_t)B * T1 * F1 * D);
   p.c2 = cv.take<float>((size_t)S * F2 * D);
@@ -494,6 +501,7 @@
   bool lens_in_conv1 = false;
   const float *tail_ln_g = nullptr, *tail_ln_b = nullptr; float tail_ln_eps = 0.f; float* tail_ln_out = nullptr;
   float* splitk_ws = nullptr; size_t splitk_bytes = 0;
+  int32_t* splitk_cnt = nullptr;
 };
 
 }
@@ -524,7 +532,14 @@
   size_t need = 0;
   if (gemm_f32_splitk_plan(p, &need) >= 2 && sb.splitk_ws != nullptr && need <= sb.splitk_bytes) {
     float* ws = sb.splitk_ws; const size_t wsb = sb.splitk_bytes;
-    add_stage(sb, name, 2, [p, ws, wsb](hipStream_t s) { return launch_gemm_f32_splitk(p, ws, wsb, s); }, gemm_info(p, true));
+    int32_t* cnt = sb.splitk_cnt;
+    add_stage(sb, name, cnt ? 1 : 2, [p, ws, wsb, cnt](hipStream_t s) { return launch_gemm_f32_splitk(p, ws, wsb, s, cnt); }, gemm_info(p, true));
+    if (cnt) {
+      Stage& st = sb.bd.stages.back();
+      st.fuse_kind = FuseKind::SplitK;
+      st.gemm = p;
+      st.sk = SplitkArgs{ws, wsb, cnt};
+    }
     return;
   }
   add_stage(sb, name, 1, [p](hipStream_t s) { return launch_gemm_f32(p, s); }, gemm_info(p, false));
@@ -537,6 +552,9 @@
   if (a.fuse_kind == FuseKind::Gemm) return gemm_f32_dual_fusable(a.gemm, b.gemm);
   if (a.fuse_kind == FuseKind::Dwconv) return dwconv_dual_fusable(a.dw, b.dw);
   if (a.fuse_kind == FuseKind::Attention) return relpos_attention_dual_fusable(a.att, b.att);
+  if (a.fuse_kind == FuseKind::Conv1) return conv1_dual_fusable(a.conv1, b.conv1);
+  if (a.fuse_kind == FuseKind::SplitK)
+    return gemm_f32_splitk_dual_fusable(a.gemm, b.gemm) && a.sk.ws != b.sk.ws && a.sk.counters != b.sk.counters;
   return false;
 }
 static Stage fused_stage(const Stage& a, const Stage& b) {
@@ -551,12 +569,23 @@
     const DwArgs pa = a.dw, pb = b.dw;
     d.run = [pa, pb](hipStream_t s) { return launch_dwconv_ln_silu_dual(pa, pb, s); };
     label = "dwconv_ln_silu_dual_kernel";
-  } else {
+  } else if (a.fuse_kind == FuseKind::Attention) {
     const AttArgs pa = a.att, pb = b.att;
     d.run = [pa, pb](hipStream_t s) { return launch_relpos_attention_dual(pa, pb, s); };
     label = "relpos_attention_dual_kernel";
-  }
-  d.info = stage_info(label, 1, a.info.alg_bytes + b.info.alg_bytes, a.info.flops + b.info.flops);
+  } else if (a.fuse_kind == FuseKind::Conv1) {
+    const Conv1Args pa = a.conv1, pb = b.conv1;
+    d.run = [pa, pb](hipStream_t s) { return launch_conv1_relu_dual(pa, pb, s); };
+    label = "conv1_relu_dual_kernel";
+  } else {
+    const GemmParams pa = a.gemm, pb = b.gemm;
+    const SplitkArgs ka = a.sk, kb = b.sk;
+    d.run = [pa, pb, ka, kb](hipStream_t s) {
+      return launch_gemm_f32_splitk_dual(pa, ka.ws, ka.counters, pb, kb.ws, kb.counters, std::min(ka.ws_bytes, kb.ws_bytes), s);
+    };
+    label = "gemm_f32_splitk_dual_kernel";
+  }
+  d.info = stage_info(label, 1, a.info.alg_bytes + b.info.alg_bytes, a.info.flops + b.info.flops, a.info.per_row != 0);
   return d;
 }
 static void fuse_independent_pairs(StageBuilder& sb, int first, int mid, int join) {
@@ -569,7 +598,7 @@
     assert(!st[m].reads_embed);
     int partner = -1;
     if (st[m].fuse_kind != FuseKind::None)
-      for (int k = std::max(i, first + 1); k < mid; ++k)
+      for (int k = st[m].fuse_kind == FuseKind::Conv1 ? i : std::max(i, first + 1); k < mid; ++k)
         if (stages_fusable(st[k], st[m])) { partner = k; break; }
     if (partner < 0) { pending.push_back(st[m]); continue; }
     for (; i < partner; ++i) out.push_back(st[i]);
@@ -604,8 +633,12 @@
   const int32_t* flen = sb.lens_in_conv1 ? sb.bd.key.feat_len : nullptr;
   int32_t* lens_out = pl.lens;
   sb.lens_in_conv1 = false;
-  add_stage(sb, pfx + "conv1", 1, [=](hipStream_t s) { return launch_conv1_relu(feat, w.c1w, w.c1b, cm, ci, B, T, idim, D, c1, s, 1, a16, flen, lens_out); },
+  Conv1Args ca;
+  ca.feat = feat; ca.w9c = w.c1w; ca.bias = w.c1b; ca.cmvn_mean = cm; ca.cmvn_istd = ci; ca.B = B; ca.T = T; ca.idim = idim; ca.C = D;
+  ca.out = c1; ca.relu = 1; ca.out_bf16 = a16; ca.feat_len = flen; ca.lens_out = lens_out;
+  add_stage(sb, pfx + "conv1", 1, [ca](hipStream_t s) { return launch_conv1_relu_args(ca, s); },
             stage_info("conv1_relu_kernel", 1, (double)B * T * idim * 4 + (double)B * T1 * F1 * D * (a16 ? 2 : 4), 18.0 * B * T1 * F1 * D, false));
+  const size_t conv1_at = sb.bd.stages.size() - 1;
   GemmParams g;
   g.a_bf16 = a16; g.y_bf16 = a16;
   g.mode = GEMM_A_CONV3X3S2; g.A = c1; g.lda = 4;
@@ -613,6 +646,10 @@
   g.W = w.c2w; g.bias = w.c2b; g.Y = c2; g.ldy = D; g.M = B * T2 * F2; g.N = D; g.K = 9 * D; g.act = ACT_RELU;
   if (sb.bd.packed) g.conv_len = pl.lens;
   add_gemm(sb, pfx + "conv2", g);
+  if (sb.bd.stages.back().fuse_kind == FuseKind::SplitK) {
+    sb.bd.stages[conv1_at].fuse_kind = FuseKind::Conv1;
+    sb.bd.stages[conv1_at].conv1 = ca;
+  }
   const bool packed = sb.bd.packed;
   GemmParams l;
   l.A = c2; l.lda = F2 * D; l.W = w.out.w; l.bias = w.out.b; l.Y = packed ? pl.xpad : xout; l.ldy = D;
@@ -1095,6 +1132,13 @@
   const int32_t* feat_len = k.feat_len; float* logits = k.logits;
   bd.key = k; bd.Tp = Tp; bd.S = B * Tp;
   sb.splitk_ws = pl.splitk; sb.splitk_bytes = pl.splitk_bytes;
+  int32_t* const cnt_main = pl.splitk_bytes && switches().splitk_tail ? pl.splitk_cnt : nullptr;
+  int32_t* const cnt_embed = cnt_main ? cnt_main + kSplitkCounters : nullptr;
+  if (cnt_main) {
+    M3_CHECK_HIP(hipMemsetAsync(cnt_main, 0, 2 * kSplitkCounters * sizeof(int32_t), nullptr));
+    M3_CHECK_HIP(hipStreamSynchronize(nullptr));
+  }
+  sb.splitk_cnt = cnt_main;
   {
     GemmParams t;
     t.M = B * Tp; t.N = c.attention_dim; t.K = c.attention_dim; t.w_bf16 = 1;
@@ -1161,7 +1205,7 @@
   }
   const Plan ple = embed_view(pl);
   const int embed_start = (int)bd.stages.size();
-  sb.splitk_ws = ple.splitk;
+  sb.splitk_ws = ple.splitk; sb.splitk_cnt = cnt_embed;
   build_subsample(sb, "embed.subsample.", e->sub_e, De, ple, ple.x);
   for (int i = 0; i < c.embed_blocks; ++i) {
     if (i + 1 == c.embed_blocks) {
@@ -1170,7 +1214,7 @@
     build_block(sb, "embed.blocks." + std::to_string(i) + ".", e->eblocks[i], De, c.embed_linear_units, c.embed_heads,
                 c.cnn_module_kernel, c.embed_cnn_layer_norm, false, i, i, ple, c.embed_causal > 0);
   }
-  sb.splitk_ws = pl.splitk;
+  sb.splitk_ws = pl.splitk; sb.splitk_cnt = cnt_main;
   if (c.embed_blocks == 0) {
     float* x = ple.x; float* emb = pl.emb;
     const float* g = e->e_after.g; const float* b = e->e_after.b;
diff --git a/3m-asr-inference_amd/csrc/gemm_f32_splitk.hip b/3m-asr-inference_amd/csrc/gemm_f32_splitk.hip
--- a/3m-asr-inference_amd/csrc/gemm_f32_splitk.hip
+++ b/3m-asr-inference_amd/csrc/gemm_f32_splitk.hip
@@ -10,9 +10,37 @@
 constexpr int kSplitLdsBytes = 2 * (SBM + SBN) * S_LD * 4;
 }
 
+__device__ __forceinline__ f32x4 splitk_sum_epilogue(const float* part, int splits, int M, int N, int m, int n, const float* bias,
+                                                     int act, float alpha) {
+  f32x4 v = bias ? ldg4(bias + n) : f32x4{0.f, 0.f, 0.f, 0.f};
+  for (int s0 = 0; s0 < splits; s0 += 4) {
+    f32x4 t[4];
+#pragma unroll
+    for (int j = 0; j < 4; ++j)
+      t[j] = (s0 + j < splits) ? ldg4(part + ((size_t)(s0 + j) * M + m) * N + n) : f32x4{0.f, 0.f, 0.f, 0.f};
+#pragma unroll
+    for (int j = 0; j < 4; ++j) v += t[j];
+  }
+#pragma unroll
+  for (int e = 0; e < 4; ++e) {
+    float t = v[e];
+    if (act == ACT_RELU) t = fmaxf(t, 0.f);
+    if (act == ACT_SILU) t = silu(t);
+    v[e] = t * alpha;
+  }
+  return v;
+}
+
+struct SplitkJob {
+  GemmParams p;
+  float* part;
+  int32_t* counters;
+  int splits, ksteps_per_split;
+};
+
 template <bool CONV>
-__global__ __launch_bounds__(256, 2) void gemm_f32_splitk_kernel(const GemmParams p, float* __restrict__ part,
-                                                                 int ksteps_per_split) {
+__device__ __forceinline__ void splitk_body(const GemmParams& p, float* part, int32_t* counters, const int splits,
+                                            const int ksteps_per_split, const int tile, const int split) {
   constexpr int MT = SBM / 32, NT = SBN / 32;
   constexpr int CA = SBK / 4, RA = 256 / CA, JA = SBM / RA, JB = SBN / RA;
   extern __shared__ __attribute__((aligned(16))) unsigned char splitk_lds[];
@@ -23,7 +51,7 @@
   const int tid = threadIdx.x, lane = tid & 63, wave = tid >> 6;
   const int col = lane & 15, kq = lane >> 4;
   const int wm = wave >> 1, wn = wave & 1;
-  const int n_tile = blockIdx.x % p.n_tiles, m_tile = blockIdx.x / p.n_tiles, split = blockIdx.y;
+  const int n_tile = tile % p.n_tiles, m_tile = tile / p.n_tiles;
   const int m0 = m_tile * SBM, n0 = n_tile * SBN;
   const int nsteps_total = p.K / SBK;
   const int s_lo = split * ksteps_per_split, s_hi = min(s_lo + ksteps_per_split, nsteps_total);
@@ -119,6 +147,40 @@
     const int m = m0 + row;
     if (m < p.M && n < p.N) stg4(part + ((size_t)split * p.M + m) * p.N + n, *reinterpret_cast<const f32x4*>(Cs + row * SC_LD + c4));
   }
+  if (counters == nullptr) return;
+  __builtin_amdgcn_fence(__ATOMIC_RELEASE, "agent");
+  __syncthreads();
+  int* last_flag = reinterpret_cast<int*>(splitk_lds);
+  if (tid == 0) {
+    __builtin_amdgcn_fence(__ATOMIC_RELEASE, "agent");
+    const int arrived = __hip_atomic_fetch_add(counters + tile, 1, __ATOMIC_RELAXED, __HIP_MEMORY_SCOPE_AGENT);
+    *last_flag = arrived == splits - 1;
+  }
+  __syncthreads();
+  if (*last_flag == 0) return;
+  __builtin_amdgcn_fence(__ATOMIC_ACQUIRE, "agent");
+  for (int it = 0; it < SBM / 16; ++it) {
+    const int row = (4 * it + wave) * 4 + (lane >> 4);
+    const int m = m0 + row;
+    if (m < p.M && n < p.N)
+      stg4(p.Y + (size_t)m * p.ldy + n, splitk_sum_epilogue(part, splits, p.M, p.N, m, n, p.bias, p.act, p.alpha));
+  }
+  if (tid == 0) __hip_atomic_store(counters + tile, 0, __ATOMIC_RELAXED, __HIP_MEMORY_SCOPE_AGENT);
+}
+
+template <bool CONV>
+__global__ __launch_bounds__(256, 2) void gemm_f32_splitk_kernel(const SplitkJob j) {
+  splitk_body<CONV>(j.p, j.part, j.counters, j.splits, j.ksteps_per_split, (int)blockIdx.x, (int)blockIdx.y);
+}
+template <bool CONV>
+__global__ __launch_bounds__(256, 2) void gemm_f32_splitk_dual_kernel(const SplitkJob j0, const SplitkJob j1, const int n0) {
+  const int id = (int)blockIdx.x, split = (int)blockIdx.y;
+  if (id < n0) {
+    if (id < j0.p.n_tiles * j0.p.m_tiles && split < j0.splits)
+      splitk_body<CONV>(j0.p, j0.part, j0.counters, j0.splits, j0.ksteps_per_split, id, split);
+  } else if (split < j1.splits) {
+    splitk_body<CONV>(j1.p, j1.part, j1.counters, j1.splits, j1.ksteps_per_split, id - n0, split);
+  }
 }
 
 __global__ __launch_bounds__(256) void splitk_reduce_kernel(const float* __restrict__ part, int splits, int M, int N,
@@ -127,23 +189,7 @@
   const size_t quads = (size_t)M * (N / 4);
   for (size_t q = (size_t)blockIdx.x * 256 + threadIdx.x; q < quads; q += (size_t)gridDim.x * 256) {
     const int m = (int)(q / (N / 4)), n = 4 * (int)(q % (N / 4));
-    f32x4 v = bias ? ldg4(bias + n) : f32x4{0.f, 0.f, 0.f, 0.f};
-    for (int s0 = 0; s0 < splits; s0 += 4) {
-      f32x4 t[4];
-#pragma unroll
-      for (int j = 0; j < 4; ++j)
-        t[j] = (s0 + j < splits) ? ldg4(part + ((size_t)(s0 + j) * M + m) * N + n) : f32x4{0.f, 0.f, 0.f, 0.f};
-#pragma unroll
-      for (int j = 0; j < 4; ++j) v += t[j];
-    }
-#pragma unroll
-    for (int e = 0; e < 4; ++e) {
-      float t = v[e];
-      if (act == ACT_RELU) t = fmaxf(t, 0.f);
-      if (act == ACT_SILU) t = silu(t);
-      v[e] = t * alpha;
-    }
-    stg4(y + (size_t)m * ldy + n, v);
+    stg4(y + (size_t)m * ldy + n, splitk_sum_epilogue(part, splits, M, N, m, n, bias, act, alpha));
   }
 }
 
@@ -152,15 +198,23 @@
   if (once.done()) return 0;
   M3_CHECK_HIP(hipFuncSetAttribute((const void*)gemm_f32_splitk_kernel<true>, hipFuncAttributeMaxDynamicSharedMemorySize, kSplitLdsBytes));
   M3_CHECK_HIP(hipFuncSetAttribute((const void*)gemm_f32_splitk_kernel<false>, hipFuncAttributeMaxDynamicSharedMemorySize, kSplitLdsBytes));
+  M3_CHECK_HIP(hipFuncSetAttribute((const void*)gemm_f32_splitk_dual_kernel<true>, hipFuncAttributeMaxDynamicSharedMemorySize, kSplitLdsBytes));
+  M3_CHECK_HIP(hipFuncSetAttribute((const void*)gemm_f32_splitk_dual_kernel<false>, hipFuncAttributeMaxDynamicSharedMemorySize, kSplitLdsBytes));
   once.mark();
   return 0;
+}
+
+static bool splitk_computable(const GemmParams& p) {
+  if (p.M <= 0 || p.N <= 0 || p.K < SBK) return false;
+  if (p.w_bf16 || p.a_bf16 || p.y_bf16 || p.Yb || (p.K & 63) || (p.N & 3) || (p.lda & 3) || (p.ldy & 3)) return false;
+  if (p.mode == GEMM_A_CONCAT2 || p.ln_wsum || p.ln_gamma || p.mask_in || p.mask_out || p.resid || p.act == ACT_GLU) return false;
+  if (p.mode == GEMM_A_CONV3X3S2 && (p.conv_C & 63)) return false;
+  return true;
 }
 
 int gemm_f32_splitk_plan(const GemmParams& p, size_t* ws_bytes) {
   if (ws_bytes) *ws_bytes = 0;
-  if (p.w_bf16 || p.K < 4096 || (p.K & 63) || (p.N & 3) || (p.lda & 3) || (p.ldy & 3)) return 0;
-  if (p.mode == GEMM_A_CONCAT2 || p.ln_wsum || p.ln_gamma || p.mask_in || p.mask_out || p.resid || p.act == ACT_GLU) return 0;
-  if (p.mode == GEMM_A_CONV3X3S2 && (p.conv_C & 63)) return 0;
+  if (!splitk_computable(p) || p.K < 4096) return 0;
   const long tiles = (long)cdiv(p.M, SBM) * cdiv(p.N, SBN);
   if (tiles > 160) return 0;
   const int nsteps = p.K / SBK;
@@ -173,25 +227,71 @@
   return splits;
 }
 
-int launch_gemm_f32_splitk(const GemmParams& pin, float* ws, size_t ws_bytes, hipStream_t stream) {
-  GemmParams p = pin;
+int gemm_f32_splitk_splits(const GemmParams& p, int forced, size_t* ws_bytes) {
+  if (forced <= 0) return gemm_f32_splitk_plan(p, ws_bytes);
+  if (ws_bytes) *ws_bytes = 0;
+  if (!splitk_computable(p) || (long)cdiv(p.M, SBM) * cdiv(p.N, SBN) > kSplitkCounters) return 0;
+  const int nsteps = p.K / SBK;
+  int splits = forced < nsteps ? forced : nsteps;
+  splits = cdiv(nsteps, cdiv(nsteps, splits));
+  if (ws_bytes) *ws_bytes = (size_t)splits * p.M * p.N * sizeof(float);
+  return splits;
+}
+
+static int splitk_job(const GemmParams& pin, float* ws, size_t ws_bytes, int32_t* counters, int forced, SplitkJob* j) {
   size_t need = 0;
-  const int splits = gemm_f32_splitk_plan(p, &need);
-  M3_REQUIRE(splits >= 2 && ws != nullptr && ws_bytes >= need, "gemm split-K: not applicable / workspace %zu < %zu", ws_bytes, need);
+  const int splits = gemm_f32_splitk_splits(pin, forced, &need);
+  M3_REQUIRE(splits >= 1 && splitk_computable(pin) && ws != nullptr && ws_bytes >= need,
+             "gemm split-K: not applicable / workspace %zu < %zu", ws_bytes, need);
+  j->p = pin;
+  j->p.m_tiles = cdiv(pin.M, SBM);
+  j->p.n_tiles = cdiv(pin.N, SBN);
+  M3_REQUIRE(j->p.m_tiles * j->p.n_tiles <= kSplitkCounters, "gemm split-K: %d tiles, %d arrival counters", j->p.m_tiles * j->p.n_tiles,
+             kSplitkCounters);
+  j->part = ws; j->counters = counters; j->splits = splits; j->ksteps_per_split = cdiv(pin.K / SBK, splits);
+  return 0;
+}
+
+int launch_gemm_f32_splitk(const GemmParams& pin, float* ws, size_t ws_bytes, hipStream_t stream, int32_t* counters, int forced_splits) {
+  SplitkJob j;
+  if (int rc = splitk_job(pin, ws, ws_bytes, counters, forced_splits, &j)) return rc;
   if (int rc = init_gemm_f32_splitk_kernels()) return rc;
-  p.m_tiles = cdiv(p.M, SBM);
-  p.n_tiles = cdiv(p.N, SBN);
-  const int per = cdiv(p.K / SBK, splits);
-  dim3 grid(p.m_tiles * p.n_tiles, splits);
+  const GemmParams& p = j.p;
+  dim3 grid(p.m_tiles * p.n_tiles, j.splits);
   if (p.mode == GEMM_A_CONV3X3S2)
-    hipLaunchKernelGGL((gemm_f32_splitk_kernel<true>), grid, dim3(256), kSplitLdsBytes, stream, p, ws, per);
+    hipLaunchKernelGGL((gemm_f32_splitk_kernel<true>), grid, dim3(256), kSplitLdsBytes, stream, j);
   else
-    hipLaunchKernelGGL((gemm_f32_splitk_kernel<false>), grid, dim3(256), kSplitLdsBytes, stream, p, ws, per);
-  const size_t quads = (size_t)p.M * (p.N / 4);
-  hipLaunchKernelGGL(splitk_reduce_kernel, dim3(grid1d(quads, 1024)), dim3(256), 0, stream, ws, splits, p.M, p.N, p.bias, p.act,
-                     p.alpha, p.Y, p.ldy);
+    hipLaunchKernelGGL((gemm_f32_splitk_kernel<false>), grid, dim3(256), kSplitLdsBytes, stream, j);
+  if (counters == nullptr) {
+    const size_t quads = (size_t)p.M * (p.N / 4);
+    hipLaunchKernelGGL(splitk_reduce_kernel, dim3(grid1d(quads, 1024)), dim3(256), 0, stream, ws, j.splits, p.M, p.N, p.bias, p.act,
+                       p.alpha, p.Y, p.ldy);
+  }
   M3_LAUNCH_CHECK();
   return 0;
 }
 
-}
+bool gemm_f32_splitk_dual_fusable(const GemmParams& a, const GemmParams& b) {
+  return splitk_computable(a) && splitk_computable(b) && a.mode == b.mode && a.N == b.N && a.K == b.K && a.conv_C == b.conv_C &&
+         a.conv_F1 == b.conv_F1 && a.conv_F2 == b.conv_F2;
+}
+int launch_gemm_f32_splitk_dual(const GemmParams& a, float* ws_a, int32_t* counters_a, const GemmParams& b, float* ws_b,
+                                int32_t* counters_b, size_t ws_bytes_each, hipStream_t stream, int forced_splits) {
+  M3_REQUIRE(gemm_f32_splitk_dual_fusable(a, b), "gemm split-K dual: the two problems do not share a kernel form");
+  M3_REQUIRE(counters_a != nullptr && counters_b != nullptr && counters_a != counters_b && ws_a != ws_b,
+             "gemm split-K dual: each problem needs its own partials and arrival counters");
+  SplitkJob j0, j1;
+  if (int rc = splitk_job(a, ws_a, ws_bytes_each, counters_a, forced_splits, &j0)) return rc;
+  if (int rc = splitk_job(b, ws_b, ws_bytes_each, counters_b, forced_splits, &j1)) return rc;
+  if (int rc = init_gemm_f32_splitk_kernels()) return rc;
+  const int n0 = (int)align_up((size_t)j0.p.m_tiles * j0.p.n_tiles, 8);
+  dim3 grid(n0 + j1.p.m_tiles * j1.p.n_tiles, j0.splits > j1.splits ? j0.splits : j1.splits);
+  if (a.mode == GEMM_A_CONV3X3S2)
+    hipLaunchKernelGGL((gemm_f32_splitk_dual_kernel<true>), grid, dim3(256), kSplitLdsBytes, stream, j0, j1, n0);
+  else
+    hipLaunchKernelGGL((gemm_f32_splitk_dual_kernel<false>), grid, dim3(256), kSplitLdsBytes, stream, j0, j1, n0);
+  M3_LAUNCH_CHECK();
+  return 0;
+}
+
+}
diff --git a/3m-asr-inference_amd/csrc/kernels.h b/3m-asr-inference_amd/csrc/kernels.h
--- a/3m-asr-inference_amd/csrc/kernels.h
+++ b/3m-asr-inference_amd/csrc/kernels.h
@@ -44,7 +44,13 @@
 const char* gemm_kernel_label(const GemmParams& p, bool splitk);
 bool gemm_bf16w_uses_tiled(const GemmParams& p);
 int gemm_f32_splitk_plan(const GemmParams& p, size_t* ws_bytes);
-int launch_gemm_f32_splitk(const GemmParams& p, float* ws, size_t ws_bytes, hipStream_t stream);
+constexpr int kSplitkCounters = 256;
+int gemm_f32_splitk_splits(const GemmParams& p, int forced, size_t* ws_bytes);
+int launch_gemm_f32_splitk(const GemmParams& p, float* ws, size_t ws_bytes, hipStream_t stream, int32_t* counters = nullptr,
+                           int forced_splits = 0);
+bool gemm_f32_splitk_dual_fusable(const GemmParams& a, const GemmParams& b);
+int launch_gemm_f32_splitk_dual(const GemmParams& a, float* ws_a, int32_t* counters_a, const GemmParams& b, float* ws_b,
+                                int32_t* counters_b, size_t ws_bytes_each, hipStream_t stream, int forced_splits = 0);
 int init_gemm_f32_splitk_kernels();
 int init_gemm_bf16_tiled_kernels();
 constexpr int kXbStatParts = 4;
@@ -235,6 +241,14 @@
 int launch_conv1_relu(const float* feat, const float* w9c, const float* bias, const float* cmvn_mean,
                       const float* cmvn_istd, int B, int T, int idim, int C, float* out, hipStream_t stream, int relu = 1,
                       int out_bf16 = 0, const int32_t* feat_len = nullptr, int32_t* lens_out = nullptr);
+struct Conv1Args {
+  const float *feat = nullptr, *w9c = nullptr, *bias = nullptr, *cmvn_mean = nullptr, *cmvn_istd = nullptr;
+  int B = 0, T = 0, idim = 0, C = 0; float* out = nullptr; int relu = 1, out_bf16 = 0;
+  const int32_t* feat_len = nullptr; int32_t* lens_out = nullptr;
+};
+int launch_conv1_relu_args(const Conv1Args& a, hipStream_t stream);
+bool conv1_dual_fusable(const Conv1Args& a, const Conv1Args& b);
+int launch_conv1_relu_dual(const Conv1Args& a, const Conv1Args& b, hipStream_t stream);
 int launch_cmvn(const float* x, const int32_t* len, const float* mean, const float* istd, int B, int T, int D,
                 float* y, hipStream_t stream);
 int launch_log_softmax_bias(const float* x, const float* bias, float* y, size_t rows, int n, hipStream_t stream);
diff --git a/3m-asr-inference_amd/m3asr/_lib.py b/3m-asr-inference_amd/m3asr/_lib.py
--- a/3m-asr-inference_amd/m3asr/_lib.py
+++ b/3m-asr-inference_amd/m3asr/_lib.py
@@ -118,6 +118,11 @@
     "m3_linear_workspace_size": (_sz, [_P(LinearDesc)]),
     "m3_linear_kernel": (C.c_char_p, [_P(LinearDesc), _i]),
     "m3_linear_ws": (_i, [_P(LinearDesc), _vp, _sz, _vp]),
+    "m3_linear_splitk_workspace_size": (_sz, [_P(LinearDesc), _i]),
+    "m3_linear_splitk": (_i, [_P(LinearDesc), _i, _vp, _sz, _vp, _vp]),
+    "m3_linear_splitk_dual": (_i, [_P(LinearDesc), _vp, _vp, _P(LinearDesc), _vp, _vp, _sz, _i, _vp]),
+    "m3_conv2d_3x3s2_splitk_workspace_size": (_sz, [_i, _i, _i, _i, _i]),
+    "m3_conv2d_3x3s2_splitk": (_i, [_vp, _vp, _vp, _i, _i, _i, _i, _i, _vp, _i, _vp, _sz, _vp, _vp]),
     "m3_conv2d_3x3s2_first": (_i, [_vp, _vp, _vp, _i, _i, _i, _i, _i, _vp, _vp]),
     "m3_conv2d_3x3s2": (_i, [_vp, _vp, _vp, _i, _i, _i, _i, _i, _vp, _vp]),
     "m3_layer_norm": (_i, [_vp, _vp, _vp, _f, _vp, _i, _i, _vp]),
diff --git a/include/m3asr.h b/include/m3asr.h
--- a/include/m3asr.h
+++ b/include/m3asr.h
@@ -144,6 +144,15 @@
 size_t m3_linear_workspace_size(const m3_linear_desc* desc);
 const char* m3_linear_kernel(const m3_linear_desc* desc, int with_workspace);
 int m3_linear_ws(const m3_linear_desc* desc, void* workspace, size_t workspace_bytes, m3_stream stream);
+#define M3_SPLITK_COUNTERS 256
+size_t m3_linear_splitk_workspace_size(const m3_linear_desc* desc, int splits);
+int m3_linear_splitk(const m3_linear_desc* desc, int splits, void* workspace, size_t workspace_bytes, int32_t* counters,
+                     m3_stream stream);
+int m3_linear_splitk_dual(const m3_linear_desc* a, void* workspace_a, int32_t* counters_a, const m3_linear_desc* b,
+                          void* workspace_b, int32_t* counters_b, size_t workspace_bytes_each, int splits, m3_stream stream);
+size_t m3_conv2d_3x3s2_splitk_workspace_size(int B, int T1, int F1, int C, int splits);
+int m3_conv2d_3x3s2_splitk(const float* in, const float* w, const float* bias, int B, int T1, int F1, int C, int act, float* out,
+                           int splits, void* workspace, size_t workspace_bytes, int32_t* counters, m3_stream stream);
 
 int m3_layer_norm(const float* x, const float* gamma, const float* beta, float eps, float* y, int rows, int dim,
                   m3_stream stream);
```

Result: slower. 134,200 frames/s (-9.7%).
